# PeihaoChen/RSPNet

Hardware: AMD Instinct MI355X
Metric: clips/sec pretext step (c3d 16x112x112, B=32/GPU) (higher is better)
Workload: dtype f32

## Files before the change

### include/rspnet_hip.h

```cpp
#ifndef RSPNET_HIP_H
#define RSPNET_HIP_H

#include <stddef.h>
#include <stdint.h>

#ifdef __cplusplus
extern "C" {
#endif

#define RSP_OK 0
#define RSP_EINVAL (-1)
#define RSP_EWORKSPACE (-2)
#define RSP_ELAUNCH (-3)
#define RSP_EUNSUPPORTED (-4)

const char* rsp_strerror(int code);
const char* rsp_last_error(void);
const char* rsp_last_conv_kernel(void);
int rsp_version(void);

typedef struct rsp_conv3d_desc {
  int32_t N, Di, Hi, Wi, Cin;
  int32_t Do, Ho, Wo, Cout;
  int32_t kT, kH, kW;
  int32_t sT, sH, sW;
  int32_t pT, pH, pW;
  int32_t in_ld;
  int32_t out_ld;
} rsp_conv3d_desc;

size_t rsp_conv3d_packed_fwd_elems(const rsp_conv3d_desc* d);
int rsp_conv3d_pack_fwd(const rsp_conv3d_desc* d, const float* w_ref, float* w_packed, void* stream);

int32_t rsp_conv3d_stat_tiles(const rsp_conv3d_desc* d);
size_t rsp_conv3d_fwd_workspace(const rsp_conv3d_desc* d);
int rsp_conv3d_fwd(const rsp_conv3d_desc* d, const float* x, const float* w_packed, const float* bias, float* y,
                   float* stat_partials, void* workspace, size_t workspace_bytes, void* stream);

size_t rsp_conv3d_dgrad_workspace(const rsp_conv3d_desc* d);
int rsp_conv3d_dgrad(const rsp_conv3d_desc* d, const float* dy, const float* w_ref, float* dx, void* workspace,
                     size_t workspace_bytes, void* stream);

size_t rsp_conv3d_packed_dgrad_elems(const rsp_conv3d_desc* d);
int rsp_conv3d_dgrad_packed(const rsp_conv3d_desc* d, const float* dy, const float* w_packed, float* dx, void* workspace,
                            size_t workspace_bytes, void* stream);

typedef struct rsp_pack_job {
  const void* src;
  void* dst;
  int64_t total;
  int32_t kind, Cout_src, Cin_src, kT, kH, kW;
  int32_t transpose, O, C, Kld, nTd, nTh, nTw, k0d, k0h, k0w, kstepd, ksteph, kstepw, ntaps;
  int32_t blocks, reserved;
} rsp_pack_job;
int32_t rsp_conv3d_pack_jobs(const rsp_conv3d_desc* d, int32_t which, int32_t Cout_src, int32_t Cin_src, const float* w_ref,
                             float* w_packed, rsp_pack_job* jobs, int32_t max_jobs);
int rsp_pack_run(const rsp_pack_job* jobs_device, int32_t n_jobs, int32_t max_blocks, void* stream);
void rsp_conv3d_pack_forget(const void* w_packed);

size_t rsp_conv3d_wgrad_workspace(const rsp_conv3d_desc* d);
size_t rsp_conv3d_rowgeom_bytes(const rsp_conv3d_desc* d);
int rsp_conv3d_rowgeom(const rsp_conv3d_desc* d, void* table, void* stream);
int rsp_conv3d_wgrad(const rsp_conv3d_desc* d, const float* x, const float* dy, float* dw_ref, float* dbias, int32_t cout_valid,
                     int32_t cin_valid, const void* rowgeom_table, void* workspace, size_t workspace_bytes, void* stream);

const char* rsp_conv3d_kernel_name(const rsp_conv3d_desc* d, int which);

double rsp_conv3d_executed_fraction(const rsp_conv3d_desc* d, int which);

int rsp_conv3d_set_option(const char* name, int32_t value);

int rsp_fastdiv_check(int d, int n);

typedef struct rsp_bn_ema_job {
  float* running_mean;
  float* running_var;
  const float* batch_stats;
  int32_t C;
  float momentum;
} rsp_bn_ema_job;
size_t rsp_bn_finalize_workspace(int32_t tiles, int32_t C);
int rsp_bn_finalize(const float* stat_partials, int32_t tiles, int32_t C, int32_t c_valid, int32_t stat_ld, int64_t count,
                    const float* conv_bias, const float* gamma, const float* beta, float eps, float momentum, float* running_mean,
                    float* running_var, float* batch_stats_out, float* mean_invstd , float* scale_shift ,
                    void* workspace, size_t workspace_bytes, void* stream);
int rsp_bn_running_update(const rsp_bn_ema_job* jobs_device, int32_t n_jobs, int32_t max_c, void* stream);

typedef struct rsp_pool3d_desc {
  int32_t N, Di, Hi, Wi, C;
  int32_t Do, Ho, Wo;
  int32_t kT, kH, kW, sT, sH, sW, pT, pH, pW;
  int32_t in_ld, out_ld, res_ld;
} rsp_pool3d_desc;

int rsp_bn_act_pool_fwd(const rsp_pool3d_desc* d, const float* y, const float* scale_shift, const float* residual,
                        int relu, const float* gate, float* out, void* stream);

int rsp_bn_act_maxpool_applicable(const rsp_pool3d_desc* d);
int rsp_bn_act_maxpool_fwd(const rsp_pool3d_desc* d, const float* y, const float* scale_shift, int relu, const float* gate, float* out,
                           int32_t* argmax, void* stream);

size_t rsp_bn_bwd_workspace(const rsp_pool3d_desc* d);
int rsp_bn_act_pool_bwd(const rsp_pool3d_desc* d, const float* y, const float* residual, const float* dout,
                        const float* gamma, const float* mean_invstd, const float* scale_shift, int relu, float* dy,
                        float* dres, float* dgamma, float* dbeta, int32_t c_valid, const float* gate, const float* dmean,
                        void* workspace, size_t workspace_bytes, void* stream);

size_t rsp_bn_eval_bwd_workspace(const rsp_pool3d_desc* d);
int rsp_bn_eval_act_pool_bwd(const rsp_pool3d_desc* d, const float* y, const float* residual, const float* dout,
                             const float* mean_invstd, const float* scale_shift, int relu, float* dy, float* dres,
                             float* dgamma, float* dbeta, int32_t c_valid, void* workspace, size_t workspace_bytes,
                             void* stream);

int rsp_maxpool3d_fwd(const rsp_pool3d_desc* d, const float* x, float* out, int32_t* argmax, void* stream);
int rsp_maxpool3d_bwd(const rsp_pool3d_desc* d, const float* dout, const int32_t* argmax, float* dx, void* stream);

size_t rsp_gate_fwd_workspace(int32_t N, int32_t P, int32_t C);
int rsp_gate_fwd(const float* x, int32_t N, int32_t P, int32_t C, int32_t in_ld, const float* w, const float* b,
                 float* out, int32_t out_ld, float* mean, float* gate, void* workspace, size_t workspace_bytes,
                 void* stream);
int rsp_bn_gate_sums(const float* y, int32_t N, int32_t P, int32_t C, int32_t y_ld, const float* scale_shift, int relu,
                     float* act, int32_t act_ld, const float* w, const float* b, float* mean, float* gate, void* workspace,
                     size_t workspace_bytes, void* stream);
int rsp_gate_apply(const float* x, int32_t N, int32_t P, int32_t C, int32_t in_ld, const float* gate, float* out, int32_t out_ld,
                   void* stream);
int rsp_gate_bwd_params(const float* y, const float* scale_shift, int relu, const float* dout, int32_t N, int32_t P, int32_t C,
                        int32_t y_ld, int32_t dout_ld, const float* w, const float* mean, const float* gate, float* dw, float* db,
                        float* dmean, void* workspace, size_t workspace_bytes, void* stream);
size_t rsp_gate_bwd_workspace(int32_t N, int32_t P, int32_t C);
int rsp_gate_bwd(const float* x, const float* dout, int32_t N, int32_t P, int32_t C, int32_t x_ld, int32_t dout_ld,
                 const float* w, const float* mean, const float* gate, float* dx, int32_t dx_ld, float* dw, float* db,
                 void* workspace, size_t workspace_bytes, void* stream);

int rsp_head_fwd(const float* feat, int32_t B, int32_t P, int32_t C, int32_t feat_ld, const float* w1,
                 const float* b1, const float* w2, const float* b2, int32_t dim, float* out1, float* out2,
                 float* pooled, float* raw, void* stream);
size_t rsp_head_bwd_workspace(int32_t B, int32_t dim);
int rsp_head_bwd(const float* dout1, const float* dout2, const float* pooled, const float* raw, const float* w1,
                 const float* w2, int32_t B, int32_t P, int32_t C, int32_t feat_ld, int32_t dim, float* dw1,
                 float* db1, float* dw2, float* db2, float* dfeat, void* workspace, size_t workspace_bytes,
                 void* stream);

int rsp_spatial_mean_fwd(const float* x, int32_t N, int32_t P, int32_t C, int32_t ld, float* mean, void* stream);
int rsp_spatial_mean_bwd(const float* dmean, int32_t N, int32_t P, int32_t C, int32_t ld, float* dx, void* stream);
int rsp_linear_fwd(const float* x, int32_t B, int32_t Cin, const float* w, const float* bias, int32_t Cout, int relu,
                   float* y, void* stream);
size_t rsp_linear_bwd_workspace(int32_t B, int32_t Cout);
int rsp_linear_bwd(const float* x, const float* y, const float* dy, const float* w, int32_t B, int32_t Cin, int32_t Cout,
                   int relu, float* dx, float* dw, float* db, void* workspace, size_t workspace_bytes, void* stream);
int rsp_l2norm_fwd(const float* x, int32_t B, int32_t dim, float* y, void* stream);
int rsp_l2norm_bwd(const float* x, const float* dy, int32_t B, int32_t dim, float* dx, void* stream);

int rsp_logits_fwd(const float* qA, const float* qM, const float* kA, const float* kM, const float* knegA,
                   const float* knegM, const float* queue, int32_t B, int32_t dim, int32_t dim_m, int32_t K, float inv_T,
                   float* logits1, float* logits2, float* lposM, float* lnegM, void* stream);
size_t rsp_logits_bwd_workspace(int32_t B, int32_t dim, int32_t K);
int rsp_logits_bwd(const float* dlogits1, const float* dlogits2, const float* dlposM, const float* dlnegM,
                   const float* kA, const float* kM, const float* knegA, const float* knegM, const float* queue,
                   int32_t B, int32_t dim, int32_t dim_m, int32_t K, float inv_T, float* dqA, float* dqM, void* workspace,
                   size_t workspace_bytes, void* stream);

int rsp_loss_fwd_bwd(const float* logits1, const float* logits2, const float* lposM, const float* lnegM, int32_t B,
                     int32_t K1 , float margin, float A, float M, float* losses, float* dlogits1,
                     float* dlogits2, float* dlposM, float* dlnegM, float* row_scratch , void* stream);

int rsp_queue_enqueue(float* queue, int32_t dim, int32_t K, int32_t ptr, const float* keys, int32_t n, void* stream);
int rsp_queue_enqueue_dev(float* queue, int32_t dim, int32_t K, int64_t* ptr_dev, const float* keys, int32_t n, void* stream);

int rsp_clip_gather(const float* im, int32_t B_in, int32_t C, int32_t T_in, int32_t H, int32_t W, const int32_t* src,
                    const int32_t* step, int32_t B_out, int32_t T_out, int32_t C_out, float* out, void* stream);
int rsp_clip_gather_multi(int32_t n_jobs, const float* const* ims, const int32_t* const* srcs, const int32_t* const* steps,
                          float* const* outs, int32_t B_in, int32_t C, int32_t T_in, int32_t H, int32_t W, int32_t B_out, int32_t T_out,
                          int32_t C_out, void* stream);

int rsp_momentum_update(float* k, const float* q, int64_t n, float m, void* stream);

int rsp_sgd_step(float* p, const float* g, float* buf, int64_t n, float lr, float mu, float wd, float gscale,
                 int first, void* stream);

#define RSP_ELT_RELU_FWD 0
#define RSP_ELT_RELU_BWD 1
#define RSP_ELT_SIGMOID_FWD 2
#define RSP_ELT_SIGMOID_BWD 3
#define RSP_ELT_ADD 4
int rsp_eltwise(int32_t op, const float* a, const float* b , float* y, int64_t n, void* stream);

int rsp_rows_gather(const float* in, const int32_t* idx, int32_t n, int32_t width, float* out, void* stream);

#define RSP_AUG_BRIGHTNESS 0
// ... 83 lines not shown
```

### rspnet_amd/_lib.py

```python
from __future__ import annotations

import ctypes as C
import os
from typing import Optional

_HERE = os.path.dirname(os.path.abspath(__file__))
LIB_PATH = os.environ.get("RSPNET_HIP_LIB") or os.path.join(_HERE, "librspnet_hip.so")

c_f32p = C.c_void_p
c_i32p = C.c_void_p
c_stream = C.c_void_p


class ConvDesc(C.Structure):
    _fields_ = [(n, C.c_int32) for n in (
        "N", "Di", "Hi", "Wi", "Cin", "Do", "Ho", "Wo", "Cout", "kT", "kH", "kW", "sT", "sH", "sW",
        "pT", "pH", "pW", "in_ld", "out_ld")]


class PoolDesc(C.Structure):
    _fields_ = [(n, C.c_int32) for n in (
        "N", "Di", "Hi", "Wi", "C", "Do", "Ho", "Wo", "kT", "kH", "kW", "sT", "sH", "sW", "pT", "pH", "pW",
        "in_ld", "out_ld", "res_ld")]


class PackJob(C.Structure):
    _fields_ = [("src", C.c_void_p), ("dst", C.c_void_p), ("total", C.c_int64)] + [(n, C.c_int32) for n in (
        "kind", "Cout_src", "Cin_src", "kT", "kH", "kW", "transpose", "O", "C", "Kld", "nTd", "nTh", "nTw", "k0d", "k0h", "k0w",
        "kstepd", "ksteph", "kstepw", "ntaps", "blocks", "reserved")]


class BnEmaJob(C.Structure):
    _fields_ = [("running_mean", C.c_void_p), ("running_var", C.c_void_p), ("batch_stats", C.c_void_p), ("C", C.c_int32),
                ("momentum", C.c_float)]


class AugmentClipDesc(C.Structure):
    _fields_ = [("src", C.c_void_p), ("frame_pitch", C.c_int64), ("row_pitch", C.c_int32), ("h", C.c_int32), ("w", C.c_int32),
                ("gray", C.c_int32), ("flip", C.c_int32), ("n_ops", C.c_int32), ("op", C.c_int32 * 4),
                ("factor", C.c_float * 4), ("one_minus", C.c_float * 4)]


class ClsMeters(C.Structure):
    _fields_ = [("val", C.c_float * 3), ("sum", C.c_float * 3), ("count", C.c_int32 * 3)]


class PretextMeters(C.Structure):
    _fields_ = [("val", C.c_float * 8), ("sum", C.c_float * 8), ("count", C.c_int32 * 8)]


class FingerprintJob(C.Structure):
    _fields_ = [("ptr", C.c_void_p), ("words", C.c_int64), ("chunk0", C.c_int64), ("kind", C.c_int32), ("reserved", C.c_int32)]


class FingerprintRec(C.Structure):
    _fields_ = [("hash", C.c_uint64), ("sumsq", C.c_double), ("sum_abs", C.c_double), ("max_abs", C.c_float),
                ("nonfinite", C.c_uint32)]


_PD = C.POINTER(ConvDesc)
_PP = C.POINTER(PoolDesc)
_sz = C.c_size_t
_i32 = C.c_int32
_i64 = C.c_int64
_f = C.c_float
_p = C.c_void_p

SIGNATURES = {
    "rsp_strerror": (C.c_char_p, [C.c_int]),
    "rsp_last_error": (C.c_char_p, []),
    "rsp_last_conv_kernel": (C.c_char_p, []),
    "rsp_version": (C.c_int, []),
    "rsp_conv3d_packed_fwd_elems": (_sz, [_PD]),
    "rsp_conv3d_pack_fwd": (C.c_int, [_PD, _p, _p, _p]),
    "rsp_conv3d_stat_tiles": (_i32, [_PD]),
    "rsp_conv3d_fwd_workspace": (_sz, [_PD]),
    "rsp_conv3d_fwd": (C.c_int, [_PD, _p, _p, _p, _p, _p, _p, _sz, _p]),
    "rsp_conv3d_dgrad_workspace": (_sz, [_PD]),
    "rsp_conv3d_dgrad": (C.c_int, [_PD, _p, _p, _p, _p, _sz, _p]),
    "rsp_conv3d_packed_dgrad_elems": (_sz, [_PD]),
    "rsp_conv3d_dgrad_packed": (C.c_int, [_PD, _p, _p, _p, _p, _sz, _p]),
    "rsp_conv3d_pack_jobs": (_i32, [_PD, _i32, _i32, _i32, _p, _p, _p, _i32]),
    "rsp_pack_run": (C.c_int, [_p, _i32, _i32, _p]),
    "rsp_conv3d_pack_forget": (None, [_p]),
    "rsp_conv3d_wgrad_workspace": (_sz, [_PD]),
    "rsp_conv3d_rowgeom_bytes": (_sz, [_PD]),
    "rsp_conv3d_rowgeom": (C.c_int, [_PD, _p, _p]),
    "rsp_conv3d_wgrad": (C.c_int, [_PD, _p, _p, _p, _p, _i32, _i32, _p, _p, _sz, _p]),
    "rsp_conv3d_kernel_name": (C.c_char_p, [_PD, C.c_int]),
    "rsp_conv3d_executed_fraction": (C.c_double, [_PD, C.c_int]),
    "rsp_conv3d_set_option": (C.c_int, [C.c_char_p, _i32]),
    "rsp_fastdiv_check": (C.c_int, [C.c_int, C.c_int]),
    "rsp_bn_finalize_workspace": (_sz, [_i32, _i32]),
    "rsp_bn_finalize": (C.c_int, [_p, _i32, _i32, _i32, _i32, _i64, _p, _p, _p, _f, _f, _p, _p, _p, _p, _p, _p, _sz, _p]),
    "rsp_bn_running_update": (C.c_int, [_p, _i32, _i32, _p]),
    "rsp_bn_act_pool_fwd": (C.c_int, [_PP, _p, _p, _p, C.c_int, _p, _p, _p]),
    "rsp_bn_act_maxpool_applicable": (C.c_int, [_PP]),
    "rsp_bn_act_maxpool_fwd": (C.c_int, [_PP, _p, _p, C.c_int, _p, _p, _p, _p]),
    "rsp_bn_bwd_workspace": (_sz, [_PP]),
    "rsp_bn_act_pool_bwd": (C.c_int, [_PP, _p, _p, _p, _p, _p, _p, C.c_int, _p, _p, _p, _p, _i32, _p, _p, _p, _sz, _p]),
    "rsp_bn_eval_bwd_workspace": (_sz, [_PP]),
    "rsp_bn_eval_act_pool_bwd": (C.c_int, [_PP, _p, _p, _p, _p, _p, C.c_int, _p, _p, _p, _p, _i32, _p, _sz, _p]),
    "rsp_maxpool3d_fwd": (C.c_int, [_PP, _p, _p, _p, _p]),
    "rsp_maxpool3d_bwd": (C.c_int, [_PP, _p, _p, _p, _p]),
    "rsp_gate_fwd_workspace": (_sz, [_i32, _i32, _i32]),
    "rsp_gate_fwd": (C.c_int, [_p, _i32, _i32, _i32, _i32, _p, _p, _p, _i32, _p, _p, _p, _sz, _p]),
    "rsp_bn_gate_sums": (C.c_int, [_p, _i32, _i32, _i32, _i32, _p, C.c_int, _p, _i32, _p, _p, _p, _p, _p, _sz, _p]),
    "rsp_gate_apply": (C.c_int, [_p, _i32, _i32, _i32, _i32, _p, _p, _i32, _p]),
    "rsp_gate_bwd_params": (C.c_int, [_p, _p, C.c_int, _p, _i32, _i32, _i32, _i32, _i32, _p, _p, _p, _p, _p, _p, _p, _sz, _p]),
    "rsp_gate_bwd_workspace": (_sz, [_i32, _i32, _i32]),
    "rsp_gate_bwd": (C.c_int, [_p, _p, _i32, _i32, _i32, _i32, _i32, _p, _p, _p, _p, _i32, _p, _p, _p, _sz, _p]),
    "rsp_head_fwd": (C.c_int, [_p, _i32, _i32, _i32, _i32, _p, _p, _p, _p, _i32, _p, _p, _p, _p, _p]),
    "rsp_head_bwd_workspace": (_sz, [_i32, _i32]),
    "rsp_head_bwd": (C.c_int, [_p, _p, _p, _p, _p, _p, _i32, _i32, _i32, _i32, _i32, _p, _p, _p, _p, _p, _p, _sz, _p]),
    "rsp_spatial_mean_fwd": (C.c_int, [_p, _i32, _i32, _i32, _i32, _p, _p]),
    "rsp_spatial_mean_bwd": (C.c_int, [_p, _i32, _i32, _i32, _i32, _p, _p]),
    "rsp_linear_fwd": (C.c_int, [_p, _i32, _i32, _p, _p, _i32, C.c_int, _p, _p]),
    "rsp_linear_bwd_workspace": (_sz, [_i32, _i32]),
    "rsp_linear_bwd": (C.c_int, [_p, _p, _p, _p, _i32, _i32, _i32, C.c_int, _p, _p, _p, _p, _sz, _p]),
    "rsp_l2norm_fwd": (C.c_int, [_p, _i32, _i32, _p, _p]),
    "rsp_l2norm_bwd": (C.c_int, [_p, _p, _i32, _i32, _p, _p]),
    "rsp_logits_fwd": (C.c_int, [_p, _p, _p, _p, _p, _p, _p, _i32, _i32, _i32, _i32, _f, _p, _p, _p, _p, _p]),
    "rsp_logits_bwd_workspace": (_sz, [_i32, _i32, _i32]),
    "rsp_logits_bwd": (C.c_int, [_p, _p, _p, _p, _p, _p, _p, _p, _p, _i32, _i32, _i32, _i32, _f, _p, _p, _p, _sz, _p]),
    "rsp_loss_fwd_bwd": (C.c_int, [_p, _p, _p, _p, _i32, _i32, _f, _f, _f, _p, _p, _p, _p, _p, _p, _p]),
    "rsp_queue_enqueue": (C.c_int, [_p, _i32, _i32, _i32, _p, _i32, _p]),
    "rsp_queue_enqueue_dev": (C.c_int, [_p, _i32, _i32, _p, _p, _i32, _p]),
    "rsp_clip_gather": (C.c_int, [_p, _i32, _i32, _i32, _i32, _i32, _p, _p, _i32, _i32, _i32, _p, _p]),
    "rsp_clip_gather_multi": (C.c_int, [_i32, _p, _p, _p, _p, _i32, _i32, _i32, _i32, _i32, _i32, _i32, _i32, _p]),
    "rsp_momentum_update": (C.c_int, [_p, _p, _i64, _f, _p]),
    "rsp_sgd_step": (C.c_int, [_p, _p, _p, _i64, _f, _f, _f, _f, C.c_int, _p]),
    "rsp_rows_gather": (C.c_int, [_p, _p, _i32, _i32, _p, _p]),
    "rsp_eltwise": (C.c_int, [_i32, _p, _p, _p, _i64, _p]),
    "rsp_augment_workspace": (_sz, [_i32, _i32, _i32]),
    "rsp_augment_batch": (C.c_int, [_p, _i32, _i32, _i32, C.POINTER(C.c_float), C.POINTER(C.c_float), C.POINTER(C.c_float), _p, _i64,
                                    _p, _sz, _p]),
    "rsp_cosine_topk_splits": (_i32, [_i32, _i32, _i32]),
    "rsp_cosine_topk_workspace": (_sz, [_i32, _i32, _i32, _i32, _i32]),
    "rsp_cosine_topk": (C.c_int, [_p, _i32, _i32, _p, _i32, _i32, _i32, _i32, _i32, _p, _p, _p, _sz, _p]),
    "rsp_topk_hits": (C.c_int, [_p, _i32, _i32, _p, _p, _i32, C.POINTER(C.c_int32), _i32, _p, _p]),
    "rsp_knn_classify_workspace": (_sz, [_i32, _i32, _i32, _i32, _i32, _i32]),
    "rsp_knn_classify": (C.c_int, [_p, _i32, _i32, _p, _p, _i32, _i32, _p, _i32, _i32, _f, _i32, _i32, _i32, _p, _p, _p, _p, _p, _p,
                                   _p, _sz, _p]),
    "rsp_xent_metrics_workspace": (_sz, [_i32, _i32]),
    "rsp_xent_metrics": (C.c_int, [_p, _i32, _i32, _i32, _i32, _p, _i32, _p, _p, _p, _p, _p, _p, _sz, _p]),
    "rsp_pretext_metrics_workspace": (_sz, [_i32]),
    "rsp_pretext_metrics": (C.c_int, [_p, _p, _p, _p, _i32, _i32, _p, _p, _p, _p, _sz, _p]),
    "rsp_cam_maps_workspace": (_sz, [_i32, _i32]),
    "rsp_cam_maps": (C.c_int, [_p, _i32, _p, _i32, _p, _i32, _i32, _i32, _p, _p, _p, _p, _i32, _i32, _p, _p, _sz, _p]),
    "rsp_cam_overlay": (C.c_int, [_p, _i32, _i32, _i32, _i32, _p, _p, _i32, _i32, _i32, _i32, _p, _p]),
    "rsp_fingerprint_workspace": (_sz, [_i64]),
    "rsp_fingerprint": (C.c_int, [_p, _i32, _i64, _p, _p, _sz, _p]),
}

_lib: Optional[C.CDLL] = None


class RspError(RuntimeError):
    pass


def load(init_gpu: bool = False) -> C.CDLL:
    global _lib
    if init_gpu:
        _init_gpu()
    if _lib is not None:
        return _lib
    if not os.path.exists(LIB_PATH):
        raise RspError(
            f"{LIB_PATH} not found: build it with rspnet_amd/csrc/build.sh (or __graft_entry__.build()). "
            "rspnet_amd has no CPU or eager fallback.")
    try:
        import torch
    except ImportError:
        pass
    lib = C.CDLL(LIB_PATH)
    for name, (res, args) in SIGNATURES.items():
        fn = getattr(lib, name)
        fn.restype = res
        fn.argtypes = args
    _lib = lib
    return lib

# ... 33 lines not shown
```

### rspnet_amd/csrc/bn_pool.hip

```cpp
#include "common.h"

namespace {

__global__ __launch_bounds__(256) void bn_finalize_stage1(const float* __restrict__ part, int tiles, int C, int ld, int S,
                                                          double* __restrict__ out) {
  __shared__ double red[4][64][2];
  const int c = blockIdx.x * 64 + (threadIdx.x & 63);
  const int rl = threadIdx.x >> 6;
  const int per = (tiles + S - 1) / S;
  const int t0 = blockIdx.y * per, t1 = min(tiles, t0 + per);
  double s = 0.0, ss = 0.0;
  if (c < C)
    for (int t = t0 + rl; t < t1; t += 4) {
      const float2 v = *reinterpret_cast<const float2*>(part + ((long long)t * ld + c) * 2);
      s += (double)v.x;
      ss += (double)v.y;
    }
  red[rl][threadIdx.x & 63][0] = s;
  red[rl][threadIdx.x & 63][1] = ss;
  __syncthreads();
  if (rl == 0 && c < C) {
    const int l = threadIdx.x;
    out[((long long)blockIdx.y * C + c) * 2 + 0] = red[0][l][0] + red[1][l][0] + red[2][l][0] + red[3][l][0];
    out[((long long)blockIdx.y * C + c) * 2 + 1] = red[0][l][1] + red[1][l][1] + red[2][l][1] + red[3][l][1];
// ... 256 lines not shown
        const long long base = (((long long)n * d.Di + od * d.sT) * d.Hi + oh * d.sH) * d.Wi + ow * d.sW;
        float v[NW][VEC], r[NW][VEC], g[VEC], best[VEC];
#pragma unroll
        for (int w = 0; w < NW; ++w) {
          load_vec<VEC>(p.y + (base + off[w]) * d.in_ld + c, v[w]);
          if (p.res) load_vec<VEC>(p.res + (base + off[w]) * d.res_ld + c, r[w]);
        }
        if (p.gate) load_vec<VEC>(p.gate + (long long)n * d.C + c, g);
#pragma unroll
        for (int e = 0; e < VEC; ++e) best[e] = -INFINITY;
#pragma unroll
        for (int w = 0; w < NW; ++w)
#pragma unroll
          for (int e = 0; e < VEC; ++e) {
            float z = fmaf(v[w][e], sc[e], sh[e]);
            if (p.res) z += r[w][e];
            if (p.relu) z = rsp_relu(z);
            if (p.gate) z *= g[e];
            best[e] = rsp_max_nan(best[e], z);
          }
        store_vec<VEC>(p.out + o * d.out_ld + c, best);
      }
    }
    return;
  }
  for (long long o = (long long)blockIdx.x * p.ppi + pl; o < p.npos; o += (long long)gridDim.x * p.ppi) {
    float best[VEC];
    if (unit) {
      float v[VEC], r[VEC];
      load_vec<VEC>(p.y + o * d.in_ld + c, v);
      if (p.res) load_vec<VEC>(p.res + o * d.res_ld + c, r);
#pragma unroll
      for (int e = 0; e < VEC; ++e) {
        float z = fmaf(v[e], sc[e], sh[e]);
        if (p.res) z += r[e];
        best[e] = p.relu ? rsp_relu(z) : z;
      }
      if (p.gate) {
        const int n = fastdiv(fastdiv(fastdiv((int)o, p.dWo), p.dHo), p.dDo);
        float g[VEC];
        load_vec<VEC>(p.gate + (long long)n * d.C + c, g);
#pragma unroll
        for (int e = 0; e < VEC; ++e) best[e] *= g[e];
      }
    } else {
      const int op = (int)o;
      const int q1 = fastdiv(op, p.dWo), ow = op - q1 * d.Wo;
      const int q2 = fastdiv(q1, p.dHo), oh = q1 - q2 * d.Ho;
      const int n = fastdiv(q2, p.dDo), od = q2 - n * d.Do;
      float g[VEC];
      if (p.gate) load_vec<VEC>(p.gate + (long long)n * d.C + c, g);
#pragma unroll
      for (int e = 0; e < VEC; ++e) best[e] = -INFINITY;
      for (int kt = 0; kt < d.kT; ++kt) {
        const int id = od * d.sT - d.pT + kt;
        if ((unsigned)id >= (unsigned)d.Di) continue;
        for (int kh = 0; kh < d.kH; ++kh) {
          const int ih = oh * d.sH - d.pH + kh;
          if ((unsigned)ih >= (unsigned)d.Hi) continue;
          for (int kw = 0; kw < d.kW; ++kw) {
            const int iw = ow * d.sW - d.pW + kw;
            if ((unsigned)iw >= (unsigned)d.Wi) continue;
            const long long pos = (((long long)n * d.Di + id) * d.Hi + ih) * d.Wi + iw;
            float v[VEC];
            load_vec<VEC>(p.y + pos * d.in_ld + c, v);
            float r[VEC];
            if (p.res) load_vec<VEC>(p.res + pos * d.res_ld + c, r);
#pragma unroll
            for (int e = 0; e < VEC; ++e) {
              float z = fmaf(v[e], sc[e], sh[e]);
              if (p.res) z += r[e];
              if (p.relu) z = rsp_relu(z);
              if (p.gate) z *= g[e];
              best[e] = rsp_max_nan(best[e], z);
            }
          }
        }
      }
    }
    store_vec<VEC>(p.out + o * d.out_ld + c, best);
  }
}

struct BwdParams {
  rsp_pool3d_desc d;
  const float* __restrict__ y;
  const float* __restrict__ res;
  const float* __restrict__ dout;
  const float* __restrict__ gamma;
  const float* __restrict__ mi;
  const float* __restrict__ ss;
  const double* __restrict__ sums;
  float* __restrict__ partial;
  float* __restrict__ dy;
  float* __restrict__ dres;
  int relu;
  int cg;
  int nblocks;
  long long count;
  int cgc, ppi;
  long long npos;
  FastDiv dcgc, dWo, dHo, dDo;
  int Cv;
  const float* __restrict__ gate;
  const float* __restrict__ dmean;
  float invP;
};

template <int VEC>
__device__ __forceinline__ void gated_grad(const BwdParams& p, int n, int c, float (&g)[VEC]) {
  float gt[VEC], dm[VEC];
  load_vec<VEC>(p.gate + (long long)n * p.d.C + c, gt);
  load_vec<VEC>(p.dmean + (long long)n * p.d.C + c, dm);
#pragma unroll
  for (int e = 0; e < VEC; ++e) g[e] = fmaf(g[e], gt[e], dm[e] * p.invP);
}

template <int VEC>
__device__ __forceinline__ void load_gamma(const BwdParams& p, int c, float (&gam)[VEC]) {
  if (p.gamma && p.Cv == p.d.C) {
    load_vec<VEC>(p.gamma + c, gam);
  } else {
#pragma unroll
    for (int e = 0; e < VEC; ++e) gam[e] = c + e < p.Cv ? (p.gamma ? p.gamma[c + e] : 1.f) : 0.f;
  }
}

template <int VEC>
__device__ __forceinline__ void zval(const BwdParams& p, long long pos, int c, const float (&sc)[VEC],
                                     const float (&sh)[VEC], float (&yv)[VEC], float (&z)[VEC]) {
  load_vec<VEC>(p.y + pos * p.d.in_ld + c, yv);
  float r[VEC];
  if (p.res) load_vec<VEC>(p.res + pos * p.d.res_ld + c, r);
#pragma unroll
  for (int e = 0; e < VEC; ++e) {
    z[e] = fmaf(yv[e], sc[e], sh[e]);
    if (p.res) z[e] += r[e];
  }
}

template <int VEC, int MODE>
__global__ __launch_bounds__(256) void bn_bwd_reduce_kernel(const BwdParams p) {
  const rsp_pool3d_desc& d = p.d;
  __shared__ float red[256][2 * VEC];
  const int cg0 = blockIdx.y * 256;
  const int cgc = min(p.cg - cg0, 256);
  const int ppi = p.ppi;
  const int t = threadIdx.x;
  const int pl = fastdiv(t, p.dcgc);
  const int cgi = cg0 + (t - pl * p.cgc);
  const bool active = pl < ppi && (t - pl * p.cgc) < cgc;
  const int c = cgi * VEC;
  float s1[VEC], s2[VEC];
#pragma unroll
  for (int e = 0; e < VEC; ++e) s1[e] = s2[e] = 0.f;
  if (active) {
    float sc[VEC], sh[VEC], mean[VEC], invstd[VEC];
    load_vec<VEC>(p.ss + c, sc);
    load_vec<VEC>(p.ss + d.C + c, sh);
    load_vec<VEC>(p.mi + c, mean);
    load_vec<VEC>(p.mi + d.C + c, invstd);
    const long long npos = (long long)d.N * d.Do * d.Ho * d.Wo;
    long long op = (long long)blockIdx.x * ppi + pl;
    long long stride = (long long)gridDim.x * ppi;
    if constexpr (MODE == 1) {
      const long long step = ppi;
      stride *= 4;
      op = (long long)blockIdx.x * ppi * 4 + pl;
      for (; op + 3 * step < npos; op += stride) {
        float yv[4][VEC], r[4][VEC], g[4][VEC];
#pragma unroll
        for (int u = 0; u < 4; ++u) {
          load_vec<VEC>(p.y + (op + u * step) * d.in_ld + c, yv[u]);
          if (p.res) load_vec<VEC>(p.res + (op + u * step) * d.res_ld + c, r[u]);
          load_vec<VEC>(p.dout + (op + u * step) * d.out_ld + c, g[u]);
        }
#pragma unroll
        for (int u = 0; u < 4; ++u)
#pragma unroll
          for (int e = 0; e < VEC; ++e) {
            float z = fmaf(yv[u][e], sc[e], sh[e]);
            if (p.res) z += r[u][e];
            const float zz = p.relu ? rsp_relu(z) : z;
            const float dz = (p.relu && rsp_relu_blocks(zz)) ? 0.f : g[u][e];
            s1[e] += dz;
            s2[e] = fmaf(dz, (yv[u][e] - mean[e]) * invstd[e], s2[e]);
          }
      }
      stride = step;
    }
    long long op_end = MODE == 1 ? min(npos, op + 4 * (long long)ppi) : npos;
    if constexpr (MODE == 2 || MODE == 3) {
      {
        constexpr int NW = MODE == 2 ? 4 : 8;
        long long off[NW];
        window_offsets<NW>(d, off);
        for (; op < npos; op += stride) {
          const int q1 = fastdiv((int)op, p.dWo), ow = (int)op - q1 * d.Wo;
          const int q2 = fastdiv(q1, p.dHo), oh = q1 - q2 * d.Ho;
          const int n = fastdiv(q2, p.dDo), od = q2 - n * d.Do;
          const long long base = (((long long)n * d.Di + od * d.sT) * d.Hi + oh * d.sH) * d.Wi + ow * d.sW;
          float yv[NW][VEC], r[NW][VEC], g[VEC], best[VEC], by[VEC];
#pragma unroll
          for (int w = 0; w < NW; ++w) {
            load_vec<VEC>(p.y + (base + off[w]) * d.in_ld + c, yv[w]);
            if (p.res) load_vec<VEC>(p.res + (base + off[w]) * d.res_ld + c, r[w]);
          }
          load_vec<VEC>(p.dout + op * d.out_ld + c, g);
#pragma unroll
          for (int e = 0; e < VEC; ++e) { best[e] = -INFINITY; by[e] = 0.f; }
#pragma unroll
          for (int w = 0; w < NW; ++w)
#pragma unroll
            for (int e = 0; e < VEC; ++e) {
              float z = fmaf(yv[w][e], sc[e], sh[e]);
              if (p.res) z += r[w][e];
              const float zz = p.relu ? rsp_relu(z) : z;
              if (rsp_max_takes(zz, best[e])) { best[e] = zz; by[e] = yv[w][e]; }
            }
#pragma unroll
          for (int e = 0; e < VEC; ++e) {
            const float dz = (p.relu && rsp_relu_blocks(best[e])) ? 0.f : g[e];
            s1[e] += dz;
            s2[e] = fmaf(dz, (by[e] - mean[e]) * invstd[e], s2[e]);
          }
        }
      }
      op_end = 0;
    }
    for (; op < op_end; op += stride) {
      const int q1 = fastdiv((int)op, p.dWo), ow = (int)op - q1 * d.Wo;
      const int q2 = fastdiv(q1, p.dHo), oh = q1 - q2 * d.Ho;
      const int n = fastdiv(q2, p.dDo), od = q2 - n * d.Do;
      float best[VEC], by[VEC];
#pragma unroll
      for (int e = 0; e < VEC; ++e) { best[e] = -INFINITY; by[e] = 0.f; }
      for (int kt = 0; kt < d.kT; ++kt) {
        const int id = od * d.sT - d.pT + kt;
        if ((unsigned)id >= (unsigned)d.Di) continue;
        for (int kh = 0; kh < d.kH; ++kh) {
          const int ih = oh * d.sH - d.pH + kh;
          if ((unsigned)ih >= (unsigned)d.Hi) continue;
          for (int kw = 0; kw < d.kW; ++kw) {
            const int iw = ow * d.sW - d.pW + kw;
            if ((unsigned)iw >= (unsigned)d.Wi) continue;
            const long long pos = (((long long)n * d.Di + id) * d.Hi + ih) * d.Wi + iw;
            float yv[VEC], z[VEC];
            zval<VEC>(p, pos, c, sc, sh, yv, z);
#pragma unroll
            for (int e = 0; e < VEC; ++e) {
              const float zz = p.relu ? rsp_relu(z[e]) : z[e];
              if (rsp_max_takes(zz, best[e])) { best[e] = zz; by[e] = yv[e]; }
            }
          }
        }
      }
      float g[VEC];
      load_vec<VEC>(p.dout + op * d.out_ld + c, g);
      if (p.gate) gated_grad<VEC>(p, n, c, g);
#pragma unroll
      for (int e = 0; e < VEC; ++e) {
        const float dz = (p.relu && rsp_relu_blocks(best[e])) ? 0.f : g[e];
        s1[e] += dz;
        s2[e] = fmaf(dz, (by[e] - mean[e]) * invstd[e], s2[e]);
      }
    }
  }
#pragma unroll
  for (int e = 0; e < VEC; ++e) { red[t][e] = s1[e]; red[t][VEC + e] = s2[e]; }
  __syncthreads();
  if (t < cgc) {
    float a1[VEC], a2[VEC];
#pragma unroll
    for (int e = 0; e < VEC; ++e) a1[e] = a2[e] = 0.f;
    for (int l = 0; l < ppi; ++l)
#pragma unroll
      for (int e = 0; e < VEC; ++e) { a1[e] += red[l * cgc + t][e]; a2[e] += red[l * cgc + t][VEC + e]; }
    float* o = p.partial + ((long long)blockIdx.x * d.C + (cg0 + t) * VEC) * 2;
#pragma unroll
    for (int e = 0; e < VEC; ++e) { o[2 * e] = a1[e]; o[2 * e + 1] = a2[e]; }
  }
}

__global__ __launch_bounds__(1024) void bn_bwd_finalize_kernel(const float* __restrict__ partial, int nblocks, int C, int Cv,
                                                               double* __restrict__ sums, float* __restrict__ dgamma,
                                                               float* __restrict__ dbeta) {
  const int c = blockIdx.x * FIN_CH + (threadIdx.x & (FIN_CH - 1));
  double a, b;
  if (!fin_sum_partials(partial, nblocks, C, C, a, b)) return;
  sums[2 * c] = a;
  sums[2 * c + 1] = b;
  if (dbeta && c < Cv) dbeta[c] = (float)a;
  if (dgamma && c < Cv) dgamma[c] = (float)b;
}

template <int VEC>
__global__ __launch_bounds__(256) void bn_bwd_apply_kernel(const BwdParams p) {
  const rsp_pool3d_desc& d = p.d;
  const long long total = (long long)d.N * d.Di * d.Hi * d.Wi * p.cg;
  const double invn = 1.0 / (double)p.count;
  for (long long idx = blockIdx.x * 256ll + threadIdx.x; idx < total; idx += 256ll * gridDim.x) {
    const int cgi = (int)(idx % p.cg);
    long long q = idx / p.cg;
    const long long pos = q;
    const int iw = (int)(q % d.Wi); q /= d.Wi;
    const int ih = (int)(q % d.Hi); q /= d.Hi;
    const int id = (int)(q % d.Di);
    const int n = (int)(q / d.Di);
    const int c = cgi * VEC;
    float sc[VEC], sh[VEC], mean[VEC], invstd[VEC], gam[VEC];
    load_vec<VEC>(p.ss + c, sc);
    load_vec<VEC>(p.ss + d.C + c, sh);
    load_vec<VEC>(p.mi + c, mean);
    load_vec<VEC>(p.mi + d.C + c, invstd);
    load_gamma<VEC>(p, c, gam);
    float yv[VEC], z[VEC], dz[VEC];
    zval<VEC>(p, pos, c, sc, sh, yv, z);
#pragma unroll
    for (int e = 0; e < VEC; ++e) dz[e] = 0.f;
    const int od = id / d.sT, oh = ih / d.sH, ow = iw / d.sW;
    if (od < d.Do && oh < d.Ho && ow < d.Wo) {
      bool win[VEC];
      float mine[VEC];
#pragma unroll
      for (int e = 0; e < VEC; ++e) { mine[e] = p.relu ? rsp_relu(z[e]) : z[e]; win[e] = true; }
      const int my = ((id - od * d.sT) * d.kH + (ih - oh * d.sH)) * d.kW + (iw - ow * d.sW);
      if (d.kT * d.kH * d.kW > 1) {
        for (int kt = 0; kt < d.kT; ++kt)
          for (int kh = 0; kh < d.kH; ++kh)
            for (int kw = 0; kw < d.kW; ++kw) {
              const int o = (kt * d.kH + kh) * d.kW + kw;
              if (o == my) continue;
              const long long pp = (((long long)n * d.Di + od * d.sT + kt) * d.Hi + oh * d.sH + kh) * d.Wi + ow * d.sW + kw;
              float y2[VEC], z2[VEC];
              zval<VEC>(p, pp, c, sc, sh, y2, z2);
#pragma unroll
              for (int e = 0; e < VEC; ++e) {
                const float v = p.relu ? rsp_relu(z2[e]) : z2[e];
                if (rsp_max_displaced(o < my, v, mine[e])) win[e] = false;
              }
            }
      }
      const long long op = (((long long)n * d.Do + od) * d.Ho + oh) * d.Wo + ow;
      float g[VEC];
      load_vec<VEC>(p.dout + op * d.out_ld + c, g);
#pragma unroll
      for (int e = 0; e < VEC; ++e) dz[e] = (win[e] && !(p.relu && rsp_relu_blocks(mine[e]))) ? g[e] : 0.f;
    }
// ... 420 lines not shown
  const bool tile = d->kT == d->sT && d->kH == d->sH && d->kW == d->sW && !(d->pT | d->pH | d->pW);
  return tile && nwin == 4 ? 2 : (tile && nwin == 8 ? 3 : 0);
}

#define RSP_BN_LAUNCH_V(K, V, mode, grid, stream, p)                                                   \
  do {                                                                                                 \
    switch (mode) {                                                                                    \
      case 1: hipLaunchKernelGGL((K<V, 1>), grid, dim3(256), 0, stream, p); break;                     \
      case 2: hipLaunchKernelGGL((K<V, 2>), grid, dim3(256), 0, stream, p); break;                     \
      case 3: hipLaunchKernelGGL((K<V, 3>), grid, dim3(256), 0, stream, p); break;                     \
      default: hipLaunchKernelGGL((K<V, 0>), grid, dim3(256), 0, stream, p); break;                    \
    }                                                                                                  \
  } while (0)
#define RSP_BN_LAUNCH(K, vec, mode, grid, stream, p)                                                   \
  do {                                                                                                 \
    if (vec) RSP_BN_LAUNCH_V(K, 4, mode, grid, stream, p);                                             \
    else RSP_BN_LAUNCH_V(K, 1, mode, grid, stream, p);                                                 \
  } while (0)

int grid_for(long long total) {
  long long b = (total + 255) / 256;
  return (int)(b > 8192 ? 8192 : (b < 1 ? 1 : b));
}

int reduce_blocks(const rsp_pool3d_desc* d, int cg) {
  const int cgc = cg < 256 ? cg : 256;
  const int ppi = 256 / cgc;
  const long long npos = (long long)d->N * d->Do * d->Ho * d->Wo;
  long long b = (npos + (long long)ppi * 8 - 1) / ((long long)ppi * 8);
  return (int)(b > 2048 ? 2048 : (b < 1 ? 1 : b));
}

}

extern "C" {

static int finalize_slices(int tiles) { return tiles >= 8192 ? 256 : (tiles >= 4096 ? 64 : (tiles >= 64 ? 16 : 1)); }

size_t rsp_bn_finalize_workspace(int32_t tiles, int32_t C) {
  const int S = finalize_slices(tiles);
  return (size_t)S * C * 2 * sizeof(double);
}

__global__ __launch_bounds__(256) void bn_ema_kernel(const rsp_bn_ema_job* __restrict__ jobs) {
  const rsp_bn_ema_job j = jobs[blockIdx.y];
  const int c = blockIdx.x * 256 + threadIdx.x;
  if (c >= j.C) return;
  j.running_mean[c] = (1.f - j.momentum) * j.running_mean[c] + j.momentum * j.batch_stats[c];
  j.running_var[c] = (1.f - j.momentum) * j.running_var[c] + j.momentum * j.batch_stats[j.C + c];
}

int rsp_bn_running_update(const rsp_bn_ema_job* jobs_device, int32_t n_jobs, int32_t max_c, void* stream) {
  RSP_REQUIRE(jobs_device && n_jobs > 0 && n_jobs <= 65535 && max_c > 0, "rsp_bn_running_update: bad argument");
  hipLaunchKernelGGL(bn_ema_kernel, dim3(rsp_cdiv(max_c, 256), n_jobs), dim3(256), 0, (hipStream_t)stream, jobs_device);
  return rsp_check_launch("bn_ema_kernel");
}

int rsp_bn_finalize(const float* stat_partials, int32_t tiles, int32_t C, int32_t c_valid, int32_t stat_ld, int64_t count,
                    const float* conv_bias, const float* gamma, const float* beta, float eps, float momentum, float* running_mean,
                    float* running_var, float* batch_stats_out, float* mean_invstd, float* scale_shift, void* workspace,
                    size_t workspace_bytes, void* stream) {
  RSP_REQUIRE(stat_partials && mean_invstd && scale_shift && workspace, "rsp_bn_finalize: null pointer");
  RSP_REQUIRE(tiles > 0 && C > 0 && count > 0 && stat_ld >= C && c_valid > 0 && c_valid <= C, "rsp_bn_finalize: bad size");
  const int S = finalize_slices(tiles);
  if (workspace_bytes < (size_t)S * C * 2 * sizeof(double)) {
    rsp_set_error("rsp_bn_finalize: workspace too small");
    return RSP_EWORKSPACE;
  }
  hipStream_t s = (hipStream_t)stream;
  if (tiles <= 2048) {
    hipLaunchKernelGGL(bn_finalize_one_kernel, dim3(rsp_cdiv(C, FIN_CH)), dim3(1024), 0, s, stat_partials, tiles, C, c_valid, stat_ld, (long long)count,
                       conv_bias, gamma, beta, eps, momentum, running_mean, running_var, mean_invstd, scale_shift, batch_stats_out);
    return rsp_check_launch("bn_finalize_one_kernel");
  }
  double* part = reinterpret_cast<double*>(workspace);
  hipLaunchKernelGGL(bn_finalize_stage1, dim3(rsp_cdiv(C, 64), S), dim3(256), 0, s, stat_partials, tiles, C, stat_ld, S, part);
  int rc = rsp_check_launch("bn_finalize_stage1");
  if (rc != RSP_OK) return rc;
  hipLaunchKernelGGL(bn_finalize_stage2, dim3(rsp_cdiv(C, 64)), dim3(1024), 0, s, part, S, C, c_valid, (long long)count, conv_bias,
                     gamma, beta, eps, momentum, running_mean, running_var, mean_invstd, scale_shift, batch_stats_out);
  return rsp_check_launch("bn_finalize_stage2");
}

int rsp_bn_act_pool_fwd(const rsp_pool3d_desc* d, const float* y, const float* scale_shift, const float* residual,
                        int relu, const float* gate, float* out, void* stream) {
  RSP_REQUIRE(pool_ok(d, false), "rsp_bn_act_pool_fwd: bad descriptor");
  RSP_REQUIRE(y && scale_shift && out, "rsp_bn_act_pool_fwd: null pointer");
  if (!residual && (d->kT != d->sT || d->kH != d->sH || d->kW != d->sW || d->pT || d->pH || d->pW) &&
      rsp_bn_act_maxpool_applicable(d) && rsp_aligned16(y) && rsp_aligned16(out) && rsp_aligned16(scale_shift) &&
      (!gate || rsp_aligned16(gate)))
    return rsp_bn_act_maxpool_fwd(d, y, scale_shift, relu, gate, out, nullptr, stream);
  PoolParams p;
  p.d = *d; p.y = y; p.ss = scale_shift; p.res = residual; p.gate = gate; p.out = out; p.relu = relu;
  const bool vec = d->C % 4 == 0 && d->in_ld % 4 == 0 && d->out_ld % 4 == 0 && rsp_aligned16(y) && rsp_aligned16(out) &&
                   rsp_aligned16(scale_shift) && (!residual || (d->res_ld % 4 == 0 && rsp_aligned16(residual))) &&
                   (!gate || rsp_aligned16(gate));
  p.cg = vec ? d->C / 4 : d->C;
  const Layout L = make_layout(d, p.cg, 4);
  RSP_REQUIRE(L.npos < (1ll << 31), "rsp_bn_act_pool_fwd: more than 2^31 - 1 output positions");
  set_layout(p, L);
  RSP_BN_LAUNCH(bn_act_pool_fwd_kernel, vec, bn_mode(d, gate != nullptr), L.grid, (hipStream_t)stream, p);
  return rsp_check_launch("bn_act_pool_fwd_kernel");
}

size_t rsp_bn_bwd_workspace(const rsp_pool3d_desc* d) {
  if (!pool_ok(d, true)) return 0;
  return rsp_align_up((size_t)2048 * d->C * 2 * sizeof(float), 256) + (size_t)d->C * 2 * sizeof(double);
}

int rsp_bn_act_pool_bwd(const rsp_pool3d_desc* d, const float* y, const float* residual, const float* dout,
                        const float* gamma, const float* mean_invstd, const float* scale_shift, int relu, float* dy,
                        float* dres, float* dgamma, float* dbeta, int32_t c_valid, const float* gate, const float* dmean,
                        void* workspace, size_t workspace_bytes, void* stream) {
  RSP_REQUIRE(pool_ok(d, true), "rsp_bn_act_pool_bwd: needs disjoint windows (kernel == stride, no padding)");
  RSP_REQUIRE(!gate || (dmean && d->kT * d->kH * d->kW == 1 && d->sT * d->sH * d->sW == 1 && !residual),
              "rsp_bn_act_pool_bwd: a gated unit has a unit window, no residual, and needs dmean");
  RSP_REQUIRE(c_valid > 0 && c_valid <= d->C, "rsp_bn_act_pool_bwd: bad valid channel count");
  RSP_REQUIRE(y && dout && mean_invstd && scale_shift && dy && workspace, "rsp_bn_act_pool_bwd: null pointer");
  if (workspace_bytes < rsp_bn_bwd_workspace(d)) {
    rsp_set_error("rsp_bn_act_pool_bwd: workspace too small");
    return RSP_EWORKSPACE;
  }
  hipStream_t s = (hipStream_t)stream;
  BwdParams p;
  memset(&p, 0, sizeof p);
  p.d = *d; p.y = y; p.res = residual; p.dout = dout; p.gamma = gamma; p.mi = mean_invstd; p.ss = scale_shift;
  p.dy = dy; p.dres = dres; p.relu = relu;
  p.Cv = c_valid;
  p.gate = gate; p.dmean = dmean;
  p.invP = 1.f / (float)((long long)d->Di * d->Hi * d->Wi);
  p.count = (long long)d->N * d->Di * d->Hi * d->Wi;
  const bool vec = d->C % 4 == 0 && d->in_ld % 4 == 0 && d->out_ld % 4 == 0 && rsp_aligned16(y) && rsp_aligned16(dout) &&
                   rsp_aligned16(dy) && rsp_aligned16(scale_shift) && rsp_aligned16(mean_invstd) &&
                   (!gamma || c_valid != d->C || rsp_aligned16(gamma)) &&
                   (!residual || (d->res_ld % 4 == 0 && rsp_aligned16(residual) && (!dres || rsp_aligned16(dres)))) &&
                   (!gate || (rsp_aligned16(gate) && rsp_aligned16(dmean)));
  p.cg = vec ? d->C / 4 : d->C;
  p.partial = reinterpret_cast<float*>(workspace);
  double* sums = reinterpret_cast<double*>(reinterpret_cast<unsigned char*>(workspace) +
                                           rsp_align_up((size_t)2048 * d->C * 2 * sizeof(float), 256));
  p.sums = sums;
  const Layout L = make_layout(d, p.cg, 4);
  RSP_REQUIRE(L.npos < (1ll << 31), "rsp_bn_act_pool_bwd: more than 2^31 - 1 output positions");
  set_layout(p, L);
  p.nblocks = reduce_blocks(d, p.cg);
  dim3 rgrid(p.nblocks, rsp_cdiv(p.cg, 256));
  const int mode = bn_mode(d, gate != nullptr);
  RSP_BN_LAUNCH(bn_bwd_reduce_kernel, vec, mode, rgrid, s, p);
  int rc = rsp_check_launch("bn_bwd_reduce_kernel");
  if (rc != RSP_OK) return rc;
  hipLaunchKernelGGL(bn_bwd_finalize_kernel, dim3(rsp_cdiv(d->C, FIN_CH)), dim3(1024), 0, s, p.partial, p.nblocks, d->C, c_valid, sums,
                     dgamma, dbeta);
  rc = rsp_check_launch("bn_bwd_finalize_kernel");
  if (rc != RSP_OK) return rc;
  const bool exact = d->Di % d->sT == 0 && d->Hi % d->sH == 0 && d->Wi % d->sW == 0 && d->kT * d->kH * d->kW <= 8;
  if (exact) {
    RSP_BN_LAUNCH(bn_bwd_apply_win_kernel, vec, mode, L.grid, s, p);
    return rsp_check_launch("bn_bwd_apply_win_kernel");
  }
  const long long total = (long long)d->N * d->Di * d->Hi * d->Wi * p.cg;
  if (vec) hipLaunchKernelGGL(bn_bwd_apply_kernel<4>, dim3(grid_for(total)), dim3(256), 0, s, p);
  else hipLaunchKernelGGL(bn_bwd_apply_kernel<1>, dim3(grid_for(total)), dim3(256), 0, s, p);
  return rsp_check_launch("bn_bwd_apply_kernel");
}

static int eval_bwd_mode(const rsp_pool3d_desc* d) {
  const int m = bn_mode(d, false);
  if (m == 1) return 1;
  const bool exact = d->Di % d->sT == 0 && d->Hi % d->sH == 0 && d->Wi % d->sW == 0;
  return exact ? m : 0;
}

static long long eval_bwd_npos(const rsp_pool3d_desc* d, int mode) {
  if (mode != 0) return (long long)d->N * d->Do * d->Ho * d->Wo;
  return (long long)d->N * rsp_cdiv(d->Di, d->sT) * rsp_cdiv(d->Hi, d->sH) * rsp_cdiv(d->Wi, d->sW);
}

size_t rsp_bn_eval_bwd_workspace(const rsp_pool3d_desc* d) {
  if (!pool_ok(d, true)) return 0;
  const long long npos = eval_bwd_npos(d, eval_bwd_mode(d));
  const long long rows = npos < EVAL_BWD_MAX_BLOCKS ? npos : EVAL_BWD_MAX_BLOCKS;
  return (size_t)rows * d->C * 2 * sizeof(float);
}

#define RSP_BN_EVAL_LAUNCH_S(V, M, grid, stream, p)                                                                       \
  do {                                                                                                                    \
    if (sums) hipLaunchKernelGGL((bn_eval_bwd_kernel<V, M, true>), grid, dim3(256), 0, stream, p);                        \
    else hipLaunchKernelGGL((bn_eval_bwd_kernel<V, M, false>), grid, dim3(256), 0, stream, p);                            \
  } while (0)
#define RSP_BN_EVAL_LAUNCH_V(V, mode, grid, stream, p)                                                                    \
  do {                                                                                                                    \
    switch (mode) {                                                                                                       \
      case 1: RSP_BN_EVAL_LAUNCH_S(V, 1, grid, stream, p); break;                                                         \
      case 2: RSP_BN_EVAL_LAUNCH_S(V, 2, grid, stream, p); break;                                                         \
      case 3: RSP_BN_EVAL_LAUNCH_S(V, 3, grid, stream, p); break;                                                         \
      default: RSP_BN_EVAL_LAUNCH_S(V, 0, grid, stream, p); break;                                                        \
    }                                                                                                                     \
  } while (0)

int rsp_bn_eval_act_pool_bwd(const rsp_pool3d_desc* d, const float* y, const float* residual, const float* dout,
                             const float* mean_invstd, const float* scale_shift, int relu, float* dy, float* dres,
                             float* dgamma, float* dbeta, int32_t c_valid, void* workspace, size_t workspace_bytes,
                             void* stream) {
  RSP_REQUIRE(pool_ok(d, true), "rsp_bn_eval_act_pool_bwd: needs disjoint windows (kernel == stride, no padding)");
  RSP_REQUIRE(c_valid > 0 && c_valid <= d->C, "rsp_bn_eval_act_pool_bwd: bad valid channel count");
  RSP_REQUIRE(y && dout && scale_shift && dy, "rsp_bn_eval_act_pool_bwd: null pointer");
  RSP_REQUIRE(!dres || residual, "rsp_bn_eval_act_pool_bwd: dres without a residual");
  RSP_REQUIRE(d->res_ld >= d->C || !residual, "rsp_bn_eval_act_pool_bwd: bad residual pitch");
  const bool sums = dgamma || dbeta;
  RSP_REQUIRE(!sums || (mean_invstd && workspace), "rsp_bn_eval_act_pool_bwd: parameter gradients need mean_invstd and a workspace");
  if (sums && workspace_bytes < rsp_bn_eval_bwd_workspace(d)) {
    rsp_set_error("rsp_bn_eval_act_pool_bwd: workspace too small");
    return RSP_EWORKSPACE;
  }
  hipStream_t s = (hipStream_t)stream;
  EvalBwdParams p;
  memset(&p, 0, sizeof p);
  p.d = *d; p.y = y; p.res = residual; p.dout = dout; p.mi = mean_invstd; p.ss = scale_shift;
  p.partial = sums ? reinterpret_cast<float*>(workspace) : nullptr;
  p.dy = dy; p.dres = dres; p.relu = relu; p.Cv = c_valid;
  const bool vec = d->C % 4 == 0 && d->in_ld % 4 == 0 && d->out_ld % 4 == 0 && rsp_aligned16(y) && rsp_aligned16(dout) &&
                   rsp_aligned16(dy) && rsp_aligned16(scale_shift) && (!sums || rsp_aligned16(mean_invstd)) &&
                   (!residual || (d->res_ld % 4 == 0 && rsp_aligned16(residual) && (!dres || rsp_aligned16(dres))));
  p.cg = vec ? d->C / 4 : d->C;
  const int mode = eval_bwd_mode(d);
  p.npos = eval_bwd_npos(d, mode);
  RSP_REQUIRE(p.npos < (1ll << 31), "rsp_bn_eval_act_pool_bwd: more than 2^31 - 1 positions");
  p.cgc = p.cg < 256 ? p.cg : 256;
  p.ppi = 256 / p.cgc;
  p.dcgc = fastdiv_make(p.cgc);
  p.De = rsp_cdiv(d->Di, d->sT); p.He = rsp_cdiv(d->Hi, d->sH); p.We = rsp_cdiv(d->Wi, d->sW);
  if (mode == 0) { p.dW = fastdiv_make(p.We); p.dH = fastdiv_make(p.He); p.dD = fastdiv_make(p.De); }
  else { p.dW = fastdiv_make(d->Wo); p.dH = fastdiv_make(d->Ho); p.dD = fastdiv_make(d->Do); }
  long long b = (p.npos + (long long)p.ppi * 16 - 1) / ((long long)p.ppi * 16);
  b = b > EVAL_BWD_MAX_BLOCKS ? EVAL_BWD_MAX_BLOCKS : (b < 1 ? 1 : b);
  const dim3 grid((unsigned)b, (unsigned)rsp_cdiv(p.cg, 256));
  if (vec) RSP_BN_EVAL_LAUNCH_V(4, mode, grid, s, p);
  else RSP_BN_EVAL_LAUNCH_V(1, mode, grid, s, p);
  int rc = rsp_check_launch("bn_eval_bwd_kernel");
  if (rc != RSP_OK || !sums) return rc;
  hipLaunchKernelGGL(bn_eval_bwd_finalize_kernel, dim3(rsp_cdiv(d->C, FIN_CH)), dim3(1024), 0, s, p.partial, (int)b, d->C, c_valid,
                     dgamma, dbeta);
  return rsp_check_launch("bn_eval_bwd_finalize_kernel");
}

}
// ... 1 lines not shown
```

### rspnet_amd/csrc/conv_igemm.hip

```cpp
#include "common.h"
#include <algorithm>
#include <type_traits>
#include "conv_stem.h"

namespace {

constexpr int BK = 32;
constexpr int LDK = BK + 4;
constexpr int MAX_TAPS = 343;

__device__ __attribute__((aligned(64))) float g_zero[16];

const float* igemm_zero_page() {
  static const float* cache[64] = {nullptr};
  int dev = 0;
  if (hipGetDevice(&dev) != hipSuccess || dev < 0 || dev >= 64) dev = 0;
  if (!cache[dev]) {
    void* z = nullptr;
    if (hipGetSymbolAddress(&z, HIP_SYMBOL(g_zero)) != hipSuccess || !z) return nullptr;
    cache[dev] = reinterpret_cast<const float*>(z);
  }
  return cache[dev];
}

// ... 2325 lines not shown
  if (mp.split) {
    mp.ms = plan_multi_split(nm, Ms, tl, nc, cols);
    if (mp.ms.bytes > ws_bytes) mp.split = false;
  }
  if (!((tiles_all >= 512 && tiles_all <= 4096) || mp.split)) return mp;
  mp.n = nm;
  const bool square = bn == 128 || bn == 64;
  mp.l.family = K_MULTI;
  mp.l.bm = 128; mp.l.bn = bn; mp.l.waves_m = square ? 2 : 4; mp.l.waves_n = square ? 2 : 1; mp.l.vec = 4; mp.l.minw = 2;
  mp.l.cols = cols;
  mp.l.partial_bytes = mp.split ? mp.ms.bytes : 0;
  return mp;
}

}

bool rsp_conv_desc_ok(const rsp_conv3d_desc* d) {
  if (!d) return false;
  if (d->N <= 0 || d->Cin <= 0 || d->Cout <= 0) return false;
  if (d->kT * d->kH * d->kW > MAX_TAPS || d->kT <= 0 || d->kH <= 0 || d->kW <= 0) return false;
  if (d->sT <= 0 || d->sH <= 0 || d->sW <= 0 || d->pT < 0 || d->pH < 0 || d->pW < 0) return false;
  if (d->Do != (d->Di + 2 * d->pT - d->kT) / d->sT + 1) return false;
  if (d->Ho != (d->Hi + 2 * d->pH - d->kH) / d->sH + 1) return false;
  if (d->Wo != (d->Wi + 2 * d->pW - d->kW) / d->sW + 1) return false;
  if (d->Do <= 0 || d->Ho <= 0 || d->Wo <= 0) return false;
  if (d->in_ld < d->Cin || d->out_ld < d->Cout) return false;
  return (long long)d->N * d->Do * d->Ho * d->Wo < (1ll << 31);
}

extern "C" {


size_t rsp_conv3d_packed_fwd_elems(const rsp_conv3d_desc* d) {
  if (!desc_ok(d)) return 0;
  if (rsp_stem_applicable(d)) return rsp_stem_packed_elems(d);
  const size_t K = (size_t)d->kT * d->kH * d->kW * d->Cin;
  return (size_t)d->Cout * rsp_align_up(K, 4);
}

int rsp_conv3d_pack_fwd(const rsp_conv3d_desc* d, const float* w_ref, float* w_packed, void* stream) {
  RSP_REQUIRE(desc_ok(d), "rsp_conv3d_pack_fwd: bad descriptor");
  RSP_REQUIRE(w_ref && w_packed, "rsp_conv3d_pack_fwd: null pointer");
  if (rsp_stem_applicable(d)) return rsp_stem_pack(d, w_ref, w_packed, (hipStream_t)stream);
  PackParams p;
  p.w = w_ref; p.out = w_packed;
  p.Cout = d->Cout; p.Cin = d->Cin; p.kT = d->kT; p.kH = d->kH; p.kW = d->kW;
  p.transpose = 0; p.O = d->Cout; p.C = d->Cin;
  p.Kld = (int)rsp_align_up((size_t)d->kT * d->kH * d->kW * d->Cin, 4);
  p.nTd = d->kT; p.nTh = d->kH; p.nTw = d->kW;
  p.k0d = p.k0h = p.k0w = 0;
  p.kstepd = p.ksteph = p.kstepw = 1;
  const long long total = (long long)p.O * p.Kld;
  const int blocks = (int)((total + 255) / 256 > 4096 ? 4096 : (total + 255) / 256);
  hipLaunchKernelGGL(pack_weight_kernel, dim3(blocks), dim3(256), 0, (hipStream_t)stream, p);
  return rsp_check_launch("pack_weight_kernel");
}

int32_t rsp_conv3d_stat_tiles(const rsp_conv3d_desc* d) {
  if (!desc_ok(d)) return 0;
  if (rsp_stem_applicable(d)) return rsp_stem_tiles(d);
  return rsp_cdiv((long long)d->N * d->Do * d->Ho * d->Wo, 128);
}

size_t rsp_conv3d_fwd_workspace(const rsp_conv3d_desc* d) {
  if (!desc_ok(d)) return 0;
  if (rsp_stem_applicable(d)) return 0;
  IgemmParams p;
  fill_fwd_params(d, ALIGNED, ALIGNED, nullptr, ALIGNED, nullptr, p);
  return igemm_partial_bytes(p);
}

int rsp_conv3d_fwd(const rsp_conv3d_desc* d, const float* x, const float* w_packed, const float* bias, float* y,
                   float* stat_partials, void* workspace, size_t workspace_bytes, void* stream) {
  RSP_REQUIRE(desc_ok(d), "rsp_conv3d_fwd: bad descriptor");
  RSP_REQUIRE(x && w_packed && y, "rsp_conv3d_fwd: null pointer");
  RSP_REQUIRE(rsp_aligned16(w_packed), "rsp_conv3d_fwd: packed weight must be 16-byte aligned");
  rsp_note_reset();
  if (rsp_stem_applicable(d)) return rsp_stem_fwd(d, x, w_packed, bias, y, stat_partials, (hipStream_t)stream);
  IgemmParams p;
  const bool vec4 = fill_fwd_params(d, x, w_packed, bias, y, stat_partials, p);
  return run_igemm(p, vec4, workspace, workspace_bytes, (hipStream_t)stream);
}

double rsp_conv3d_executed_fraction(const rsp_conv3d_desc* d, int which) {
  if (!desc_ok(d)) return 1.0;
  if (which == 2) return rsp_wgrad_executed_fraction(d);
  if (which == 0) {
    if (rsp_stem_applicable(d)) return 1.0;
    IgemmParams p;
    const bool vec4 = fill_fwd_params(d, ALIGNED, ALIGNED, nullptr, ALIGNED, nullptr, p);
    return igemm_live_fraction(p, vec4, plan_conv(p, vec4, 0, SIZE_MAX).l[0]);
  }
  IgemmParams cls[64];
  bool cvec[64], in_multi[64] = {false};
  const int ncls = dgrad_classes(d, ALIGNED, ALIGNED, ALIGNED, cls, cvec);
  const MultiPlan mp = plan_multi(cls, cvec, ncls, multi_split_ok(d, ALIGNED), SIZE_MAX);
  for (int j = 0; j < mp.n; ++j) in_multi[mp.cls[j]] = true;
  double live = 0.0, tot = 0.0;
  for (int i = 0; i < ncls; ++i) {
    const IgemmParams& p = cls[i];
    const double wgt = (double)p.M * p.K;
    live += wgt * igemm_live_fraction(p, cvec[i], in_multi[i] ? mp.l : plan_conv(p, cvec[i], 0, SIZE_MAX).l[0]);
    tot += wgt;
  }
  return tot > 0 ? live / tot : 1.0;
}

int rsp_fastdiv_check(int d, int n) {
  const FastDiv f = fastdiv_make(d);
  return f.mul ? (int)((unsigned)(((unsigned long long)(unsigned)n * f.mul) >> 32) >> f.shr) : n;
}

const char* rsp_conv3d_kernel_name(const rsp_conv3d_desc* d, int which) {
  if (!desc_ok(d)) return "invalid";
  if (which == 2) return rsp_wgrad_kernel_name(d);
  if (which == 0 && rsp_stem_applicable(d)) return rsp_stem_kernel_name(d);
  static thread_local char names[64][64];
  static thread_local int n_names = 0;
  LaunchPlan l;
  if (which == 0) {
    IgemmParams p;
    const bool vec4 = fill_fwd_params(d, ALIGNED, ALIGNED, nullptr, ALIGNED, nullptr, p);
    l = plan_conv(p, vec4, out_span_bytes(p), SIZE_MAX).l[0];
  } else {
    IgemmParams cls[64];
    bool cvec[64];
    const int ncls = dgrad_classes(d, ALIGNED, ALIGNED, ALIGNED, cls, cvec);
    const MultiPlan mp = plan_multi(cls, cvec, ncls, multi_split_ok(d, ALIGNED), SIZE_MAX);
    if (d->sT * d->sH * d->sW > 1) cls[0].nTd = cls[0].nTh = cls[0].nTw = 1;
    l = mp.n ? mp.l : plan_conv(cls[0], cvec[0], out_span_bytes(cls[0]), SIZE_MAX).l[0];
  }
  char name[64];
  if (l.family == K_PERSIST || l.family == K_PERSIST_FOLD)
    snprintf(name, sizeof name, kernel_format(l.family), l.bm, l.bn, l.waves_m, l.waves_n, l.ks ? "true" : "false", l.minw);
  else
    snprintf(name, sizeof name, kernel_format(l.family), l.bm, l.bn, l.waves_m, l.waves_n, l.vec, l.minw);
  for (int i = 0; i < n_names; ++i)
    if (!strcmp(names[i], name)) return names[i];
  if (n_names == 64) n_names = 0;
  return strcpy(names[n_names++], name);
}

size_t rsp_conv3d_dgrad_workspace(const rsp_conv3d_desc* d) {
  if (!desc_ok(d)) return 0;
  IgemmParams cls[64];
  bool cvec[64];
  const int ncls = dgrad_classes(d, ALIGNED, ALIGNED, ALIGNED, cls, cvec);
  for (int i = 0; i < ncls; ++i) cvec[i] = true;
  size_t part = plan_multi(cls, cvec, ncls, true, SIZE_MAX).l.partial_bytes;
  for (int i = 0; i < ncls; ++i) {
    const size_t b = igemm_partial_bytes(cls[i]);
    part = b > part ? b : part;
  }
  return dgrad_wpack_bytes(d) + part;
}


static void dgrad_pack_params(const rsp_conv3d_desc* d, const DgradClass& g, const float* w_ref, float* out, PackParams& pk) {
  pk.w = w_ref; pk.out = out;
  pk.Cout = d->Cout; pk.Cin = d->Cin; pk.kT = d->kT; pk.kH = d->kH; pk.kW = d->kW;
  pk.transpose = 1; pk.O = d->Cin; pk.C = d->Cout;
  pk.Kld = (int)rsp_align_up((size_t)g.nt * g.nh * g.nw * d->Cout, 4);
  pk.nTd = g.nt; pk.nTh = g.nh; pk.nTw = g.nw;
  pk.k0d = g.k0t; pk.k0h = g.k0h; pk.k0w = g.k0w;
  pk.kstepd = d->sT; pk.ksteph = d->sH; pk.kstepw = d->sW;
}
// ... 217 lines not shown
```

### rspnet_amd/csrc/conv_stem.h

```cpp
#pragma once
#include "common.h"

bool rsp_conv_desc_ok(const rsp_conv3d_desc* d);
bool rsp_stem_applicable(const rsp_conv3d_desc* d);
int rsp_stem_tiles(const rsp_conv3d_desc* d);
size_t rsp_stem_packed_elems(const rsp_conv3d_desc* d);
int rsp_stem_pack(const rsp_conv3d_desc* d, const float* w_ref, float* w_packed, hipStream_t s);
int rsp_stem_fwd(const rsp_conv3d_desc* d, const float* x, const float* w_packed, const float* bias, float* y,
                 float* stat_partials, hipStream_t s);
const char* rsp_stem_kernel_name(const rsp_conv3d_desc* d);
void rsp_stem_note_packed(const void* w_packed, bool three_channels);
void rsp_stem_forget_packed(const void* w_packed);
const char* rsp_wgrad_kernel_name(const rsp_conv3d_desc* d);
double rsp_wgrad_executed_fraction(const rsp_conv3d_desc* d);
```

### rspnet_amd/csrc/conv_stem.hip

```cpp
#include "conv_stem.h"

#include <mutex>
#include <unordered_map>

namespace {

struct StemParams {
  const float* __restrict__ x;
  const float* __restrict__ w;
  const float* __restrict__ bias;
  float* __restrict__ y;
  float* __restrict__ stat;
  int N, Di, Hi, Wi, Do, Ho, Wo;
  int kT, kH, kW, sT, sH, sW, pT, pH, pW;
  int Cout, out_ld;
  int tw_shift;
  int HT, WT, WTh, WTL;
  int npix, npix_r;
  int FR;
  int ntaps, nchunks;
  int tiles_h, tiles_w, tiles;
  unsigned x_bytes, w_bytes;
  int wide;
};

struct StemBias {
  floatx4 w[2];
  float n[2];
};

__device__ __forceinline__ StemBias stem_bias(const float* __restrict__ bias, int Cout, bool wide, int lane) {
  StemBias b;
#pragma unroll
  for (int j = 0; j < 2; ++j) {
    b.w[j] = floatx4{0.f, 0.f, 0.f, 0.f};
    b.n[j] = 0.f;
    const int cw = 32 * j + 4 * (lane & 7), cn = 32 * j + (lane & 31);
    if (bias && wide && cw < Cout) b.w[j] = *reinterpret_cast<const floatx4*>(bias + cw);
    if (bias && !wide && cn < Cout) b.n[j] = bias[cn];
  }
  asm volatile("" : "+v"(b.w[0]), "+v"(b.w[1]), "+v"(b.n[0]), "+v"(b.n[1]));
  return b;
}

__device__ __forceinline__ void stem_store_wide(const StemParams& p, const floatx16 (&acc)[2], float* stage ,
                                                const long long* rowaddr , int wave, int lane, const StemBias& b) {
  const int l32 = lane & 31, h = lane >> 5;
  const int q = lane & 7, rbase = lane >> 3;
#pragma unroll
  for (int j = 0; j < 2; ++j) {
    const int col = 32 * j + 4 * q;
#pragma unroll
    for (int r = 0; r < 2; ++r) {
#pragma unroll
      for (int e = 0; e < 8; ++e) stage[((e >> 2) * 8 + h * 4 + (e & 3)) * 32 + l32] = acc[j][8 * r + e];
#pragma unroll
      for (int i = 0; i < 2; ++i) {
        const int rl = rbase + 8 * i;
        const floatx4 v = *reinterpret_cast<const floatx4*>(stage + rl * 32 + 4 * q);
        const long long addr = rowaddr[wave * 32 + 16 * r + rl];
        if (addr >= 0 && col < p.Cout) *reinterpret_cast<floatx4*>(p.y + addr + col) = v + b.w[j];
      }
    }
  }
}

template <int G, int NS>
__global__ __launch_bounds__(256, 2) void stem_kernel(const StemParams p) {
  constexpr int TCH = 2 * G;
  constexpr int BU = TCH * 64;
  constexpr int BI = (BU + 255) / 256;
  typedef __attribute__((address_space(3))) void* lptr_t;
  extern __shared__ __attribute__((aligned(16))) unsigned char smem_raw[];
  float* halo = reinterpret_cast<float*>(smem_raw);
  float* Bs = halo + p.FR * p.npix_r * 4;
  int* taptab = reinterpret_cast<int*>(Bs + 2 * BU * 4);
  long long* rowaddr = reinterpret_cast<long long*>(taptab + p.nchunks * TCH);

  const int t = threadIdx.x;
  const int lane = t & 63;
  const int wave = __builtin_amdgcn_readfirstlane(t >> 6);
  const int l32 = lane & 31, h = lane >> 5;

  const int tile = rsp_xcd_remap(blockIdx.x, gridDim.x);
  const int wb = tile % p.tiles_w;
  int q0 = tile / p.tiles_w;
  const int hb = q0 % p.tiles_h;
  q0 /= p.tiles_h;
  const int to = q0 % p.Do;
  const int n = q0 / p.Do;
  const int TW = 1 << p.tw_shift, TH = 128 >> p.tw_shift;
  const int h0 = hb * TH, w0 = wb * TW;
  const StemBias bias = stem_bias(p.bias, p.Cout, p.wide != 0, lane);

  const int khw = p.kH * p.kW;
  for (int i = t; i < p.nchunks * TCH; i += 256) {
    int off = 0;
    if (i < p.ntaps) {
      const int kw = i % p.kW, r = i / p.kW;
      const int kh = r % p.kH, kt = r / p.kH;
      const int col = p.sW == 2 ? (kw & 1) * p.WTh + (kw >> 1) : kw;
      off = (((kt % p.FR) * p.npix_r) + kh * p.WTL + col) * 16;
    }
    taptab[i] = off;
  }

  unsigned hrel[4];
#pragma unroll
  for (int i = 0; i < 4; ++i) {
    const int q = i * 256 + t;
    unsigned r = 0xffffffffu;
    if (q < p.npix) {
      const int hyy = q / p.WTL, cc = q - hyy * p.WTL;
      const int wxp = p.sW == 2 ? (cc < p.WTh ? 2 * cc : 2 * (cc - p.WTh) + 1) : cc;
      const int hi = h0 * p.sH - p.pH + hyy, wi = w0 * p.sW - p.pW + wxp;
      if (wxp < p.WT && (unsigned)hi < (unsigned)p.Hi && (unsigned)wi < (unsigned)p.Wi) r = (unsigned)((hi * p.Wi + wi) * 16);
    }
    hrel[i] = r;
  }

  __amdgpu_buffer_rsrc_t rsrc_x = __builtin_amdgcn_make_buffer_rsrc(const_cast<float*>(p.x), 0, (int)p.x_bytes, 0x00020000);
  __amdgpu_buffer_rsrc_t rsrc_w = __builtin_amdgcn_make_buffer_rsrc(const_cast<float*>(p.w), 0, (int)p.w_bytes, 0x00020000);

  auto load_frame = [&](int f) {
    const int ti = to * p.sT - p.pT + f;
    const bool okf = (unsigned)ti < (unsigned)p.Di;
    const unsigned fbase = (unsigned)(((long long)(n * p.Di + (okf ? ti : 0)) * p.Hi * p.Wi) * 16);
    const int slot = f % p.FR;
#pragma unroll
    for (int i = 0; i < 4; ++i) {
      if (i * 256 + wave * 64 < p.npix_r) {
        const unsigned off = (okf & (hrel[i] != 0xffffffffu)) ? fbase + hrel[i] : 0xffffffffu;
        float* dst = halo + (slot * p.npix_r + i * 256 + wave * 64) * 4;
        __builtin_amdgcn_raw_ptr_buffer_load_lds(rsrc_x, (lptr_t)dst, 16, off, 0, 0, 0);
      }
    }
  };
  auto load_weights = [&](int c, int buf) {
#pragma unroll
    for (int i = 0; i < BI; ++i) {
      if (i * 256 + wave * 64 < BU) {
        const unsigned off = ((unsigned)c * BU + i * 256 + t) * 16u;
        float* dst = Bs + (buf * BU + i * 256 + wave * 64) * 4;
        __builtin_amdgcn_raw_ptr_buffer_load_lds(rsrc_w, (lptr_t)dst, 16, off, 0, 0, 0);
      }
// ... 15 lines not shown

  floatx16 acc[2];
#pragma unroll
  for (int j = 0; j < 2; ++j)
#pragma unroll
    for (int e = 0; e < 16; ++e) acc[j][e] = 0.f;

  int buf = 0;
  for (int c = 0; c < p.nchunks; ++c) {
    const bool more = c + 1 < p.nchunks;
    floatx4 af[G], bf[G][2];
#pragma unroll
    for (int g = 0; g < G; ++g) af[g] = *reinterpret_cast<const floatx4*>(arow + toff[g]);
    const float* bb = Bs + buf * BU * 4 + (h * 64 + l32) * 4;
#pragma unroll
    for (int g = 0; g < G; ++g)
#pragma unroll
      for (int j = 0; j < 2; ++j) bf[g][j] = *reinterpret_cast<const floatx4*>(bb + (2 * g * 64 + 32 * j) * 4);
    int toffn[G];
#pragma unroll
    for (int g = 0; g < G; ++g) toffn[g] = more ? taptab[(c + 1) * TCH + 2 * g + h] : 0;
    if (more) {
      load_weights(c + 1, buf ^ 1);
      const int fh = frame_hi(c + 1);
      while (loaded < fh) load_frame(++loaded);
    }
#pragma unroll
    for (int g = 0; g < G; ++g)
#pragma unroll
      for (int s = 0; s < NS; ++s)
#pragma unroll
        for (int j = 0; j < 2; ++j) acc[j] = __builtin_amdgcn_mfma_f32_32x32x2f32(af[g][s], bf[g][j][s], acc[j], 0, 0, 0);
    __builtin_amdgcn_sched_barrier(0);
    __syncthreads();
    buf ^= 1;
#pragma unroll
    for (int g = 0; g < G; ++g) toff[g] = toffn[g];
  }

  if (t < 128) {
    const int ry = t >> p.tw_shift, rx = t & (TW - 1);
    const int ho = h0 + ry, wo = w0 + rx;
    rowaddr[t] = (ho < p.Ho && wo < p.Wo) ? ((((long long)n * p.Do + to) * p.Ho + ho) * p.Wo + wo) * p.out_ld : -1;
  }
  __syncthreads();
  float* red = Bs;
  if (p.wide) stem_store_wide(p, acc, Bs + 512 + wave * 512, rowaddr, wave, lane, bias);
#pragma unroll
  for (int j = 0; j < 2; ++j) {
    const int col = 32 * j + l32;
    const float bv = bias.n[j];
    float s = 0.f, ss = 0.f;
#pragma unroll
    for (int e = 0; e < 16; ++e) {
      const long long addr = rowaddr[wave * 32 + (e >> 2) * 8 + h * 4 + (e & 3)];
      const float v = addr >= 0 ? acc[j][e] : 0.f;
      if (!p.wide && addr >= 0 && col < p.Cout) p.y[addr + col] = v + bv;
      s += v;
      ss = fmaf(v, v, ss);
    }
    s += __shfl_xor(s, 32);
    ss += __shfl_xor(ss, 32);
    if (h == 0) {
      red[(wave * 64 + col) * 2 + 0] = s;
      red[(wave * 64 + col) * 2 + 1] = ss;
    }
  }
  if (p.stat) {
    __syncthreads();
    if (t < 64 && t < p.Cout) {
      float s = 0.f, ss = 0.f;
#pragma unroll
      for (int w = 0; w < 4; ++w) {
        s += red[(w * 64 + t) * 2 + 0];
        ss += red[(w * 64 + t) * 2 + 1];
      }
      float* o = p.stat + ((long long)tile * p.Cout + t) * 2;
      o[0] = s;
      o[1] = ss;
    }
  }
}

template <int G, bool WIDE, int NS>
__global__ __launch_bounds__(256, 2) void stem_resident_kernel(const StemParams p) {
  constexpr int TCH = 2 * G;
  constexpr int BU = TCH * 64;
  constexpr int BI = (BU + 255) / 256;
  typedef __attribute__((address_space(3))) void* lptr_t;
  extern __shared__ __attribute__((aligned(16))) unsigned char smem_raw[];
  const int hsz = p.FR * p.npix_r * 4;
  float* halo = reinterpret_cast<float*>(smem_raw);
  float* Bs = halo + 2 * hsz;
  int* taptab = reinterpret_cast<int*>(Bs + p.nchunks * BU * 4);
  long long* rowaddr = reinterpret_cast<long long*>(taptab + p.nchunks * TCH);
  float* red = reinterpret_cast<float*>(rowaddr + 128);

  const int t = threadIdx.x;
  const int lane = t & 63;
  const int wave = __builtin_amdgcn_readfirstlane(t >> 6);
  const int l32 = lane & 31, h = lane >> 5;
  const int TW = 1 << p.tw_shift, TH = 128 >> p.tw_shift;

  for (int i = t; i < p.nchunks * TCH; i += 256) {
    int off = 0;
    if (i < p.ntaps) {
      const int kw = i % p.kW, r = i / p.kW;
      const int kh = r % p.kH, kt = r / p.kH;
      const int col = p.sW == 2 ? (kw & 1) * p.WTh + (kw >> 1) : kw;
      off = ((kt * p.npix_r) + kh * p.WTL + col) * 16;
    }
    taptab[i] = off;
  }
  __amdgpu_buffer_rsrc_t rsrc_x = __builtin_amdgcn_make_buffer_rsrc(const_cast<float*>(p.x), 0, (int)p.x_bytes, 0x00020000);
  __amdgpu_buffer_rsrc_t rsrc_w = __builtin_amdgcn_make_buffer_rsrc(const_cast<float*>(p.w), 0, (int)p.w_bytes, 0x00020000);
  for (int c = 0; c < p.nchunks; ++c) {
#pragma unroll
    for (int i = 0; i < BI; ++i) {
      if (i * 256 + wave * 64 < BU) {
        const unsigned off = ((unsigned)c * BU + i * 256 + t) * 16u;
        float* dst = Bs + (c * BU + i * 256 + wave * 64) * 4;
        __builtin_amdgcn_raw_ptr_buffer_load_lds(rsrc_w, (lptr_t)dst, 16, off, 0, 0, 0);
      }
    }
  }
  int hyy[4], wxp[4];
#pragma unroll
  for (int i = 0; i < 4; ++i) {
    const int q = i * 256 + t;
    hyy[i] = -(1 << 20);
    wxp[i] = 0;
    if (q < p.npix) {
      const int r = q / p.WTL, cc = q - r * p.WTL;
      const int wx_ = p.sW == 2 ? (cc < p.WTh ? 2 * cc : 2 * (cc - p.WTh) + 1) : cc;
      if (wx_ < p.WT) {
        hyy[i] = r;
        wxp[i] = wx_;
      }
    }
  }
  auto issue_halo = [&](int tile, int buf) {
    const int wb = tile % p.tiles_w;
    int q0 = tile / p.tiles_w;
    const int hb = q0 % p.tiles_h;
    q0 /= p.tiles_h;
    const int to = q0 % p.Do, n = q0 / p.Do;
    const int hi0 = hb * TH * p.sH - p.pH, wi0 = wb * TW * p.sW - p.pW;
    unsigned hrel[4];
#pragma unroll
    for (int i = 0; i < 4; ++i) {
      const int hi = hi0 + hyy[i], wi = wi0 + wxp[i];
      hrel[i] = ((unsigned)hi < (unsigned)p.Hi && (unsigned)wi < (unsigned)p.Wi) ? (unsigned)((hi * p.Wi + wi) * 16) : 0xffffffffu;
    }
    for (int f = 0; f < p.kT; ++f) {
      const int ti = to * p.sT - p.pT + f;
      const bool okf = (unsigned)ti < (unsigned)p.Di;
      const unsigned fbase = (unsigned)(((long long)(n * p.Di + (okf ? ti : 0)) * p.Hi * p.Wi) * 16);
#pragma unroll
      for (int i = 0; i < 4; ++i) {
        if (i * 256 + wave * 64 < p.npix_r) {
          const unsigned off = (okf & (hrel[i] != 0xffffffffu)) ? fbase + hrel[i] : 0xffffffffu;
          float* dst = halo + buf * hsz + (f * p.npix_r + i * 256 + wave * 64) * 4;
          __builtin_amdgcn_raw_ptr_buffer_load_lds(rsrc_x, (lptr_t)dst, 16, off, 0, 0, 0);
        }
      }
    }
  };

  const int m = wave * 32 + l32;
  const int rowoff = (((m >> p.tw_shift) * p.sH) * p.WTL + (m & (TW - 1))) * 16;
  const StemBias bias = stem_bias(p.bias, p.Cout, WIDE, lane);

  int cur = 0;
  if ((int)blockIdx.x < p.tiles) issue_halo(blockIdx.x, 0);
  for (int tile = blockIdx.x; tile < p.tiles; tile += gridDim.x) {
    __syncthreads();
    const int next = tile + gridDim.x;
    const char* arow = reinterpret_cast<const char*>(halo + cur * hsz) + rowoff;
    floatx16 acc[2];
#pragma unroll
    for (int j = 0; j < 2; ++j)
#pragma unroll
      for (int e = 0; e < 16; ++e) acc[j][e] = 0.f;
    for (int c = 0; c < p.nchunks; ++c) {
      floatx4 af[G], bf[G][2];
#pragma unroll
      for (int g = 0; g < G; ++g) af[g] = *reinterpret_cast<const floatx4*>(arow + taptab[c * TCH + 2 * g + h]);
      const float* bb = Bs + c * BU * 4 + (h * 64 + l32) * 4;
#pragma unroll
      for (int g = 0; g < G; ++g)
#pragma unroll
        for (int j = 0; j < 2; ++j) bf[g][j] = *reinterpret_cast<const floatx4*>(bb + (2 * g * 64 + 32 * j) * 4);
      if (c == p.nchunks - 1 && next < p.tiles) issue_halo(next, cur ^ 1);
#pragma unroll
      for (int g = 0; g < G; ++g)
#pragma unroll
        for (int s = 0; s < NS; ++s)
#pragma unroll
          for (int j = 0; j < 2; ++j) acc[j] = __builtin_amdgcn_mfma_f32_32x32x2f32(af[g][s], bf[g][j][s], acc[j], 0, 0, 0);
    }
    const int wb = tile % p.tiles_w;
    int q0 = tile / p.tiles_w;
    const int hb = q0 % p.tiles_h;
    q0 /= p.tiles_h;
    const int to = q0 % p.Do, n = q0 / p.Do;
    if (t < 128) {
      const int ho = hb * TH + (t >> p.tw_shift), wo = wb * TW + (t & (TW - 1));
      rowaddr[t] = (ho < p.Ho && wo < p.Wo) ? ((((long long)n * p.Do + to) * p.Ho + ho) * p.Wo + wo) * p.out_ld : -1;
    }
    __syncthreads();
    if (WIDE) stem_store_wide(p, acc, halo + cur * hsz + wave * 512, rowaddr, wave, lane, bias);
#pragma unroll
    for (int j = 0; j < 2; ++j) {
      const int col = 32 * j + l32;
      const float bv = bias.n[j];
      float s = 0.f, ss = 0.f;
#pragma unroll
      for (int e = 0; e < 16; ++e) {
        const long long addr = rowaddr[wave * 32 + (e >> 2) * 8 + h * 4 + (e & 3)];
        const float v = addr >= 0 ? acc[j][e] : 0.f;
        if (!WIDE && addr >= 0 && col < p.Cout) p.y[addr + col] = v + bv;
        s += v;
        ss = fmaf(v, v, ss);
      }
      s += __shfl_xor(s, 32);
      ss += __shfl_xor(ss, 32);
      if (h == 0) {
        red[(wave * 64 + col) * 2 + 0] = s;
        red[(wave * 64 + col) * 2 + 1] = ss;
      }
    }
    if (p.stat) {
      __syncthreads();
      if (t < 64 && t < p.Cout) {
        float s = 0.f, ss = 0.f;
#pragma unroll
        for (int w = 0; w < 4; ++w) {
          s += red[(w * 64 + t) * 2 + 0];
          ss += red[(w * 64 + t) * 2 + 1];
        }
        float* o = p.stat + ((long long)tile * p.Cout + t) * 2;
        o[0] = s;
        o[1] = ss;
      }
    }
    cur ^= 1;
  }
}

__global__ void stem_pack_kernel(const float* __restrict__ w, float* __restrict__ out, int Cout, int kT, int kH, int kW,
                                 int ntaps, long long total) {
  for (long long i = blockIdx.x * (long long)blockDim.x + threadIdx.x; i < total; i += (long long)gridDim.x * blockDim.x) {
    const int ci = (int)(i & 3), n = (int)((i >> 2) & 63), tap = (int)(i >> 8);
    float v = 0.f;
    if (tap < ntaps && n < Cout) {
      const int kw = tap % kW, r = tap / kW;
      const int kh = r % kH, kt = r / kH;
      v = w[((((long long)n * 4 + ci) * kT + kt) * kH + kh) * kW + kw];
    }
    out[i] = v;
  }
}

struct StemPlan {
  bool ok;
  int G, TCH, nchunks, tw_shift, HT, WT, WTh, WTL, npix, npix_r, FR, tiles_h, tiles_w;
  bool resident;
  bool wide_ok;
  long long tiles;
  size_t lds;
};

StemPlan stem_plan(const rsp_conv3d_desc* d) {
  StemPlan s;
  memset(&s, 0, sizeof s);
  if (d->Cin != 4 || d->in_ld != 4 || d->Cout > 64 || d->out_ld < d->Cout) return s;
  if (d->sW < 1 || d->sW > 2 || d->sH < 1 || d->sH > 2) return s;
  const int ntaps = d->kT * d->kH * d->kW;
  if (ntaps > 343) return s;
  if ((unsigned long long)d->N * d->Di * d->Hi * d->Wi * 16ull >= 0xF0000000ull) return s;
  const long long waste16 = (long long)rsp_cdiv(d->Ho, 8) * 8 * rsp_cdiv(d->Wo, 16) * 16;
  const long long waste8 = (long long)rsp_cdiv(d->Ho, 16) * 16 * rsp_cdiv(d->Wo, 8) * 8;
  s.tw_shift = waste8 < waste16 ? 3 : 4;
  const long long covered = waste8 < waste16 ? waste8 : waste16;
  if (ntaps > 64 && covered * 100 > (long long)d->Ho * d->Wo * 104) return s;
  const int TW = 1 << s.tw_shift, TH = 128 >> s.tw_shift;
  s.HT = (TH - 1) * d->sH + d->kH;
  s.WT = (TW - 1) * d->sW + d->kW;
  s.WTh = (s.WT + 1) / 2;
  s.WTL = d->sW == 2 ? 2 * s.WTh : s.WT;
  s.npix = s.HT * s.WTL;
  if (s.npix > 1024) return s;
  s.npix_r = (s.npix + 63) / 64 * 64;
  s.FR = d->kT < 3 ? d->kT : 3;
  int best = 0, best_pad = 1 << 30;
  const int cand[3] = {8, 7, 5};
  for (int i = 0; i < 3; ++i) {
    const int tch = 2 * cand[i];
    if (d->kT > 3 && d->kH * d->kW < 2 * tch) continue;
    const int pad = rsp_cdiv(ntaps, tch) * tch;
    if (pad < best_pad) {
      best_pad = pad;
      best = cand[i];
    }
// ... 17 lines not shown
  return s;
}

std::mutex g_three_mu;
std::unordered_map<const void*, bool> g_three;

bool stem_three_channels(const void* w_packed) {
  std::lock_guard<std::mutex> lk(g_three_mu);
  auto it = g_three.find(w_packed);
  return it != g_three.end() && it->second;
}

template <int G, int NS>
int launch_stem(const StemParams& p, const StemPlan& pl, hipStream_t s) {
  static bool attr_set = false;
  if (!attr_set) {
    (void)hipFuncSetAttribute(reinterpret_cast<const void*>(&stem_kernel<G, NS>), hipFuncAttributeMaxDynamicSharedMemorySize,
                              150 * 1024);
    attr_set = true;
  }
  if (pl.resident) {
    static bool attr_set_r = false;
    if (!attr_set_r) {
      (void)hipFuncSetAttribute(reinterpret_cast<const void*>(&stem_resident_kernel<G, true, NS>),
                                hipFuncAttributeMaxDynamicSharedMemorySize, 80 * 1024);
      (void)hipFuncSetAttribute(reinterpret_cast<const void*>(&stem_resident_kernel<G, false, NS>),
                                hipFuncAttributeMaxDynamicSharedMemorySize, 80 * 1024);
      attr_set_r = true;
    }
    long long per_cu = (160 * 1024) / (long long)pl.lds;
    per_cu = per_cu > 3 ? 3 : per_cu;
    const long long grid = pl.tiles < 256 * per_cu ? pl.tiles : 256 * per_cu;
    rsp_note_kernel(p.wide ? "stem_resident_kernel<%d, true, %d>" : "stem_resident_kernel<%d, false, %d>", G, NS);
    if (p.wide) hipLaunchKernelGGL((stem_resident_kernel<G, true, NS>), dim3((unsigned)grid), dim3(256), pl.lds, s, p);
    else hipLaunchKernelGGL((stem_resident_kernel<G, false, NS>), dim3((unsigned)grid), dim3(256), pl.lds, s, p);
    return rsp_check_launch("stem_resident_kernel");
  }
  rsp_note_kernel("stem_kernel<%d, %d>", G, NS);
  hipLaunchKernelGGL((stem_kernel<G, NS>), dim3((unsigned)pl.tiles), dim3(256), pl.lds, s, p);
  return rsp_check_launch("stem_kernel");
}

}

bool rsp_stem_applicable(const rsp_conv3d_desc* d) { return stem_plan(d).ok; }

int rsp_stem_tiles(const rsp_conv3d_desc* d) { return (int)stem_plan(d).tiles; }

const char* rsp_stem_kernel_name(const rsp_conv3d_desc* d) {
  const StemPlan pl = stem_plan(d);
  if (pl.resident && pl.wide_ok)
    return pl.G == 8 ? "stem_resident_kernel<8, true, 3>" : (pl.G == 7 ? "stem_resident_kernel<7, true, 3>" : "stem_resident_kernel<5, true, 3>");
  if (pl.resident)
    return pl.G == 8 ? "stem_resident_kernel<8, false, 3>" : (pl.G == 7 ? "stem_resident_kernel<7, false, 3>" : "stem_resident_kernel<5, false, 3>");
  return pl.G == 8 ? "stem_kernel<8, 3>" : (pl.G == 7 ? "stem_kernel<7, 3>" : "stem_kernel<5, 3>");
}

void rsp_stem_note_packed(const void* w_packed, bool three_channels) {
  std::lock_guard<std::mutex> lk(g_three_mu);
  if (three_channels) g_three[w_packed] = true;
  else g_three.erase(w_packed);
}

void rsp_stem_forget_packed(const void* w_packed) {
  std::lock_guard<std::mutex> lk(g_three_mu);
  g_three.erase(w_packed);
}

size_t rsp_stem_packed_elems(const rsp_conv3d_desc* d) {
  const StemPlan pl = stem_plan(d);
  return (size_t)pl.nchunks * pl.TCH * 256;
}

int rsp_stem_pack(const rsp_conv3d_desc* d, const float* w_ref, float* w_packed, hipStream_t s) {
  const StemPlan pl = stem_plan(d);
  const long long total = (long long)pl.nchunks * pl.TCH * 256;
  const int blocks = (int)((total + 255) / 256 > 2048 ? 2048 : (total + 255) / 256);
  rsp_stem_note_packed(w_packed, false);
  hipLaunchKernelGGL(stem_pack_kernel, dim3(blocks), dim3(256), 0, s, w_ref, w_packed, d->Cout, d->kT, d->kH, d->kW,
                     d->kT * d->kH * d->kW, total);
  return rsp_check_launch("stem_pack_kernel");
}

int rsp_stem_fwd(const rsp_conv3d_desc* d, const float* x, const float* w_packed, const float* bias, float* y,
                 float* stat_partials, hipStream_t s) {
  const StemPlan pl = stem_plan(d);
  RSP_REQUIRE(pl.ok, "rsp_stem_fwd: descriptor not on the stem path");
  RSP_REQUIRE(rsp_aligned16(x) && rsp_aligned16(w_packed), "rsp_conv3d_fwd: 4-channel input and packed weight must be 16-byte aligned");
  StemParams p;
  memset(&p, 0, sizeof p);
  p.x = x; p.w = w_packed; p.bias = bias; p.y = y; p.stat = stat_partials;
  p.N = d->N; p.Di = d->Di; p.Hi = d->Hi; p.Wi = d->Wi; p.Do = d->Do; p.Ho = d->Ho; p.Wo = d->Wo;
  p.kT = d->kT; p.kH = d->kH; p.kW = d->kW; p.sT = d->sT; p.sH = d->sH; p.sW = d->sW;
  p.pT = d->pT; p.pH = d->pH; p.pW = d->pW;
  p.Cout = d->Cout; p.out_ld = d->out_ld;
  p.tw_shift = pl.tw_shift;
  p.HT = pl.HT; p.WT = pl.WT; p.WTh = pl.WTh; p.WTL = pl.WTL;
  p.npix = pl.npix; p.npix_r = pl.npix_r; p.FR = pl.FR;
  p.ntaps = d->kT * d->kH * d->kW; p.nchunks = pl.nchunks;
  p.tiles_h = pl.tiles_h; p.tiles_w = pl.tiles_w; p.tiles = (int)pl.tiles;
  p.wide = pl.wide_ok && rsp_aligned16(y) && (!bias || rsp_aligned16(bias));
  p.x_bytes = (unsigned)((unsigned long long)d->N * d->Di * d->Hi * d->Wi * 16ull);
  p.w_bytes = (unsigned)((size_t)pl.nchunks * pl.TCH * 1024);
  if (stem_three_channels(w_packed)) {
    switch (pl.G) {
      case 8: return launch_stem<8, 3>(p, pl, s);
      case 7: return launch_stem<7, 3>(p, pl, s);
      default: return launch_stem<5, 3>(p, pl, s);
    }
  }
  switch (pl.G) {
    case 8: return launch_stem<8, 4>(p, pl, s);
    case 7: return launch_stem<7, 4>(p, pl, s);
    default: return launch_stem<5, 4>(p, pl, s);
  }
}
```

### rspnet_amd/engine.py

```python
from __future__ import annotations

import contextlib
import os
from dataclasses import dataclass, field
from typing import Dict, List, NamedTuple, Optional, Tuple, Union

import torch
from torch import nn

from . import ops as _ops
from .ops import ConvGeom, PoolGeom

Triple = Tuple[int, int, int]


@dataclass
class ConvBN:
    conv: nn.Module
    bn: nn.Module
    src: int
    dst: int
    k: Triple
    s: Triple = (1, 1, 1)
    p: Triple = (0, 0, 0)
    relu: bool = True
    pool: Optional[Tuple[Triple, Triple]] = None
    residual: Optional[int] = None
    into: Optional[Tuple[int, int, int]] = None
    branch: int = 0
    virtual_w: bool = False
    cout_pad: int = 0


@dataclass
class ConvBNGroup:
    members: List[ConvBN]
    cat: Optional["_CatConv"] = field(default=None, repr=False, compare=False)


@dataclass
class ConvBias:
    conv: nn.Module
    src: int
    dst: int
    k: Triple
    s: Triple = (1, 1, 1)
    p: Triple = (0, 0, 0)
    relu: bool = False


@dataclass
class Pool:
    src: int
    dst: int
    k: Triple
    s: Triple
    p: Triple = (0, 0, 0)
    branch: int = 0


@dataclass
class Gate:
    conv: nn.Module
    src: int
    dst: int
    into: Optional[Tuple[int, int, int]] = None
    branch: int = 0


@dataclass
class Plan:
    nodes: List[object]
    input_slot: int = 0
    output_slot: int = 0
    gate_fusion: Optional[dict] = field(default=None, repr=False, compare=False)
    pool_fusion: Optional[dict] = field(default=None, repr=False, compare=False)


@dataclass
class _Saved:
    x: torch.Tensor
    y: torch.Tensor
    mi: torch.Tensor
    ss: torch.Tensor
    cg: ConvGeom
    pg: PoolGeom
    res: Optional[torch.Tensor] = None
    eval_mode: bool = False
    gate: Optional["_SavedGate"] = None


_SavedVStem = NamedTuple("_SavedVStem", [("x_e", torch.Tensor), ("x_o", torch.Tensor), ("y", torch.Tensor), ("mi", torch.Tensor),
                                         ("ss", torch.Tensor), ("cg", ConvGeom), ("pg", PoolGeom), ("vs", "VirtualStem")])
_SavedMember = NamedTuple("_SavedMember", [("off", int), ("C", int), ("mi", torch.Tensor), ("ss", torch.Tensor), ("pg", PoolGeom)])
_SavedGroup = NamedTuple("_SavedGroup", [("x", torch.Tensor), ("y", torch.Tensor), ("cg", ConvGeom), ("per", List[_SavedMember])])
_SavedPool = NamedTuple("_SavedPool", [("pg", PoolGeom), ("idx", torch.Tensor)])
_SavedGate = NamedTuple("_SavedGate", [("at", int), ("x", Optional[torch.Tensor]), ("mean", torch.Tensor), ("gate", torch.Tensor)])
_SavedConvBias = NamedTuple("_SavedConvBias", [("x", torch.Tensor), ("y", torch.Tensor), ("cg", ConvGeom)])
SavedState = Union[_Saved, _SavedVStem, _SavedGroup, _SavedPool, _SavedGate, _SavedConvBias]


@dataclass
class ForwardCtx:
    saved: Dict[Union[int, Tuple[int, int]], SavedState] = field(default_factory=dict)
    feat_shape: Optional[Tuple[int, ...]] = None
    packed: Optional["PackedWeights"] = None
    head: object = None


class PackedWeights:

    def __init__(self):
        self._entries = []
        self._index = {}
        self._sets = []
        self._ptrs = []
        self._dirty = True
        self._virtual = {}

    def invalidate(self):
        self._dirty = True

    def refresh_now(self):
        if self._dirty and self._entries:
            self._refresh()

    def _refresh(self):
        be = _ops.backend()
        for vs in self._virtual.values():
            vs.refresh()
        ptrs = [c.weight.data_ptr() for _, _, c in self._entries]
        if len(self._sets) > 1 or ptrs != self._ptrs:
            self._sets = [be.pack_set([(g, which, c.weight.data) for g, which, c in self._entries])] if self._entries else []
            self._index = {(id(c), which, be.pack_signature(g, which, c.weight.data)): (0, i)
                           for i, (g, which, c) in enumerate(self._entries)}
            self._ptrs = ptrs
        for ps in self._sets:
            ps.run()
        self._dirty = False

    def _lookup(self, conv, cg: ConvGeom, which: int):
        if self._dirty:
            self._refresh()
        key = (id(conv), which, _ops.backend().pack_signature(cg, which, conv.weight.data))
        at = self._index.get(key)
        if at is None:
            ps = _ops.backend().pack_set([(cg, which, conv.weight.data)])
            ps.run()
            self._sets.append(ps)
            self._entries.append((cg, which, conv))
            self._ptrs.append(conv.weight.data_ptr())
            at = self._index[key] = (len(self._sets) - 1, 0)
        return self._sets[at[0]].packed[at[1]]

    def get(self, conv, cg: ConvGeom):
        return self._lookup(conv, cg, 0)

    def get_dgrad(self, conv, cg: ConvGeom):
        return self._lookup(conv, cg, 1)

    def virtual_stem(self, node) -> "VirtualStem":
        vs = self._virtual.get(id(node.conv))
        if vs is None or vs.device != node.conv.weight.device:
            vs = self._virtual[id(node.conv)] = VirtualStem(node)
        return vs


class _CatConv:
    weight: torch.Tensor = None


def _adjacent_cat(ts):
    t0 = ts[0]
    if not all(t.is_contiguous() and t.shape[1:] == t0.shape[1:] and t.dtype == t0.dtype for t in ts):
        return None
    end = t0.data_ptr() + t0.numel() * t0.element_size()
    for t in ts[1:]:
        if t.data_ptr() != end or t.untyped_storage().data_ptr() != t0.untyped_storage().data_ptr():
            return None
        end += t.numel() * t.element_size()
    shape = (sum(t.shape[0] for t in ts),) + tuple(t0.shape[1:])
    stride = tuple(t0.stride())
    return torch.as_strided(t0, shape, stride, t0.storage_offset())


INPUT_CHANNEL_PAD = 4
GATE_BWD_FUSED = not os.environ.get("RSP_NO_GATE_BWD_FUSION")


class VirtualStem:

    def __init__(self, node):
        self.conv = node.conv
        w = node.conv.weight
        Cout, cin, kT, kH, kW = w.shape
        assert cin == 3 and kW == 7 and node.s[2] == 2 and node.p[2] == 3
        self.holders, self.idx, self.src, self.dst = [], [], [], []
        co = torch.arange(Cout).view(Cout, 1, 1, 1, 1)
        c4 = torch.arange(4).view(1, 4, 1, 1, 1)
        kt = torch.arange(kT).view(1, 1, kT, 1, 1)
        kh = torch.arange(kH).view(1, 1, 1, kH, 1)
        j = torch.arange(6).view(1, 1, 1, 1, 6)
        for off in (3, 1):
            r = 4 * j + c4 - off
            valid = ((r >= 0) & (r < 21)).expand(Cout, 4, kT, kH, 6)
            real = ((((co * 3 + r % 3) * kT + kt) * kH + kh) * 7 + torch.div(r, 3, rounding_mode="floor")).expand(Cout, 4, kT, kH, 6)
            idx = torch.where(valid, real, torch.full_like(real, w.numel())).reshape(-1)
            flat_valid = valid.reshape(-1).nonzero().view(-1)
            self.idx.append(idx.to(w.device))
            self.src.append(flat_valid.to(w.device))
            self.dst.append(real.reshape(-1)[flat_valid].to(w.device))
            h = _CatConv()
            h.weight = torch.zeros((Cout, 4, kT, kH, 6), dtype=w.dtype, device=w.device)
            self.holders.append(h)
        self.device = w.device
        self.refresh()

    enabled = not os.environ.get("RSP_NO_VIRTUAL_STEM")

    @staticmethod
    def applies(node, xin) -> bool:
        w = node.conv.weight
        W = xin.shape[3]
        return (VirtualStem.enabled and node.virtual_w and w.shape[1] == 3 and xin.shape[4] == 4 and w.shape[4] == 7 and node.s[2] == 2 and node.p[2] == 3
                and (3 * W) % 4 == 0 and W % 2 == 0 and getattr(node.conv, "bias", None) is None and node.residual is None
                and node.into is None)

    def refresh(self):
        w = self.conv.weight
        ext = torch.cat([w.data.reshape(-1), w.data.new_zeros(1)])
        for h, idx in zip(self.holders, self.idx):
            torch.index_select(ext, 0, idx, out=h.weight.view(-1))

    def pack_rows(self, xin):
        N, D, H, W, _ = xin.shape
        Wp = 3 * W // 4 + 5
        flat = torch.zeros(N * D * H * Wp * 4 + 8, dtype=xin.dtype, device=xin.device)
        xv = flat[:N * D * H * Wp * 4].view(N, D, H, Wp, 4)
        xv.view(N, D, H, Wp * 4)[..., 12:12 + 3 * W].view(N, D, H, W, 3).copy_(xin[..., :3])
        return xv, torch.as_strided(flat, (N, D, H, Wp, 4), xv.stride(), 8)


class BranchStreams:
    _streams: Dict[Tuple, "torch.cuda.Stream"] = {}
    origin = None
    SMALL_WGRAD_FLOPS = float(os.environ.get("RSP_WGRAD_ASIDE_GFLOP", "50")) * 1e9

    MID_WGRAD_FLOPS = float(os.environ.get("RSP_WGRAD_MID_GFLOP", "400")) * 1e9
    MID_WGRAD_BYTES = float(os.environ.get("RSP_WGRAD_MID_MB", "450")) * 1e6
    EAGER_TASKS = not os.environ.get("RSP_NO_EAGER_OVERLAP")
    RUN_AHEAD = bool(int(os.environ.get("RSP_TASK_RUN_AHEAD", "1")))
    AHEAD_MAX_FLOPS = float(os.environ.get("RSP_TASK_AHEAD_MAX_GFLOP", "100")) * 1e9
    deferred = None

    def __init__(self, x: torch.Tensor):
        self.dev = x.device
        self.on = bool(x.is_cuda and _ops.backend().name == "hip" and BranchStreams.origin is not None
                       and torch.cuda.is_current_stream_capturing()
                       and torch.cuda.current_stream(self.dev).cuda_stream == BranchStreams.origin)
        self.origin_h = BranchStreams.origin
        self.fork_branches = self.on and bool(os.environ.get("RSP_BRANCH_FORKS"))
        if (not self.on and BranchStreams.EAGER_TASKS and x.is_cuda and _ops.backend().name == "hip"
                and not torch.cuda.is_current_stream_capturing()):
            self.on = True
            self.origin_h = torch.cuda.current_stream(self.dev).cuda_stream
        self.active: Dict[int, "torch.cuda.Stream"] = {}
        self.task = None

    def _get(self, key):
        key = (self.dev.index if self.dev.index is not None else torch.cuda.current_device(), key)
# ... 93 lines not shown
            if n.residual is not None or n.pool or n.into is not None or n.cout_pad or n.virtual_w or n.dst == plan.output_slot:
                continue
            if readers.get(n.dst) != [i + 1]:
                continue
            pi = None
            if i + 2 < len(plan.nodes):
                q = plan.nodes[i + 2]
                if (isinstance(q, Pool) and g.into is None and q.src == g.dst and q.branch == n.branch and readers.get(g.dst) == [i + 2]
                        and g.dst != plan.output_slot):
                    pi = i + 2
            table[i] = (i + 1, pi)
    plan.gate_fusion = table
    return table


GATE_POOL_APART = bool(os.environ.get("RSP_NO_GATE_POOL_KEEP"))


def _pool_fusion(plan: "Plan"):
    if plan.pool_fusion is not None:
        return plan.pool_fusion
    readers = _readers(plan)
    table = {}
    if not os.environ.get("RSP_NO_POOL_FUSION"):
        gated = _gate_fusion(plan)
        for i, n in enumerate(plan.nodes[:-1]):
            q = plan.nodes[i + 1]
            if not (isinstance(n, ConvBN) and isinstance(q, Pool) and q.src == n.dst and q.branch == n.branch) or i in gated:
                continue
            if n.pool or n.into is not None or n.cout_pad or n.dst == plan.output_slot or readers.get(n.dst) != [i + 1]:
                continue
            table[i] = i + 1
    plan.pool_fusion = table
    return table


def _view(t, into, C):
    return t if into is None else t[..., into[1]:into[1] + C]


def _out_view(slots, into, lead_shape, C, device):
    if into is None:
        return None
    slot, off, total = into
    if slot not in slots:
        slots[slot] = torch.empty(tuple(lead_shape) + (total,), dtype=torch.float32, device=device)
    return _view(slots[slot], into, C)


def _eval_scale_shift(bn, bias) -> torch.Tensor:
    scale = bn.weight.data * torch.rsqrt(bn.running_var + float(bn.eps))
    shift = bn.bias.data - bn.running_mean * scale
    if bias is not None:
        shift = shift + bias.data * scale
    return torch.stack([scale, shift]).contiguous()


def _eval_mean_invstd(bn, bias) -> torch.Tensor:
    mean = bn.running_mean if bias is None else bn.running_mean - bias.data
    return torch.stack([mean, torch.rsqrt(bn.running_var + float(bn.eps))]).contiguous()


EVAL_BACKWARD_MISSING = ("backward through an eval-mode backbone (BatchNorm on running statistics) is not implemented: "
                         "freeze the backbone (only_train_fc) or call model.train()")


def _handler(table, node):
    fn = table.get(type(node))
    if fn is None:
        raise NotImplementedError(f"plan node {type(node).__name__}")
    return fn


class _Forward:

    def __init__(self, plan, x, packed, keep, training, deferred):
        self.be = _ops.backend()
        self.plan, self.packed, self.keep, self.training, self.deferred = plan, packed, keep, training, deferred
        self.slots: Dict[int, torch.Tensor] = {plan.input_slot: x}
        self.ctx = ForwardCtx(packed=packed) if keep else None
        self.pool_fusion = _pool_fusion(plan)
        self.gate_fusion = _gate_fusion(plan) if training else {}
        self.skipped = set()

    def finalize(self, bn, stats, rows, bias_d):
        bso = self.deferred.get(id(bn)) if self.deferred is not None else None
        if bso is not None:
            return self.be.bn_finalize(stats, rows, bias_d, bn.weight.data, bn.bias.data, float(bn.eps), float(bn.momentum), None, None,
                                       batch_stats_out=bso)
        return self.be.bn_finalize(stats, rows, bias_d, bn.weight.data, bn.bias.data, float(bn.eps), float(bn.momentum),
                                   bn.running_mean, bn.running_var)

    def bn_apply(self, node, y, ss, C, dims, xin, key=None):
        be, slots = self.be, self.slots
        pk, ps = node.pool if node.pool else ((1, 1, 1), (1, 1, 1))
        pg = PoolGeom(*dims, C, pk, ps, (0, 0, 0))
        res = slots[node.residual] if node.residual is not None else None
        pi = self.pool_fusion.get(key) if key is not None else None
        if pi is not None:
            pnode = self.plan.nodes[pi]
            pgf = PoolGeom(*dims, C, pnode.k, pnode.s, pnode.p)
            if not self.keep:
                slots[pnode.dst] = be.bn_act_pool_fwd(pgf, y, ss, res, node.relu)
                self.skipped.add(pi)
                return pgf, res
            fused = be.bn_act_maxpool_fwd(pgf, y, ss, node.relu, True) if (res is None and hasattr(be, "bn_act_maxpool_fwd")) else None
            if fused is not None:
                slots[pnode.dst], idx = fused
                self.ctx.saved[pi] = _SavedPool(pgf, idx)
                self.skipped.add(pi)
                return pg, res
        out = _out_view(slots, node.into, (dims[0],) + pg.out_dims, C, xin.device)
        if out is not None:
            be.bn_act_pool_fwd(pg, y, ss, res, node.relu, out=out)
        else:
            slots[node.dst] = be.bn_act_pool_fwd(pg, y, ss, res, node.relu)
        return pg, res

    def convbn_virtual(self, node, key, xin):
        N, D, H, W, _ = xin.shape
        Cp = max(node.cout_pad, node.conv.weight.shape[0])
        vs = self.packed.virtual_stem(node)
        x_e, x_o = vs.pack_rows(xin)
        (kT, kH, _), (sT, sH, _), (pT, pH, _) = node.k, node.s, node.p
        cg = ConvGeom(N, D, H, x_e.shape[3], 4, Cp, (kT, kH, 6), (sT, sH, 3), (pT, pH, 0), Cin_alg=3 * 7 / 6)
        do, ho, g = cg.out_dims
        y = torch.empty((N, do, ho, 2 * g, Cp), dtype=torch.float32, device=xin.device)
        yv = y.view(N, do, ho, g, 2 * Cp)
        parts = []
        for c, xc in enumerate((x_e, x_o)):
            _, st = self.be.conv_fwd(cg, xc, self.packed.get(vs.holders[c], cg), None, True, out=yv[..., c * Cp:(c + 1) * Cp], out_ld=2 * Cp)
            parts.append(st)
        rows = N * do * ho * 2 * g
        mi, ss = self.finalize(node.bn, torch.cat(parts), rows, None)
        pg, _ = self.bn_apply(node, y, ss, Cp, (N, do, ho, 2 * g), xin, key)
        if self.keep:
            self.ctx.saved[key] = _SavedVStem(x_e, x_o, y, mi, ss, cg, pg, vs)

    def convbn(self, node, key):
        be, keep = self.be, self.keep
        xin = self.slots[node.src]
        if self.training and node.virtual_w and VirtualStem.applies(node, xin):
            return self.convbn_virtual(node, key, xin)
        N, D, H, W, Cin = xin.shape
        w = node.conv.weight
        Cout = w.shape[0]
        Cp = max(node.cout_pad, Cout)
        cg = ConvGeom(N, D, H, W, Cin, Cp, node.k, node.s, node.p, Cin_alg=w.shape[1])
        bias = getattr(node.conv, "bias", None)
        bn = node.bn
        bias_d = None if bias is None else bias.data
        if self.training:
            bias_conv = bias_d if (bias_d is None or Cp == Cout) else torch.cat([bias_d, bias_d.new_zeros(Cp - Cout)])
            y, stats = be.conv_fwd(cg, xin, self.packed.get(node.conv, cg), bias_conv, True)
            mi, ss = self.finalize(bn, stats, cg.rows, bias_d)
        else:
            y, _ = be.conv_fwd(cg, xin, self.packed.get(node.conv, cg), None, False)
            ss = _eval_scale_shift(bn, bias)
            mi = _eval_mean_invstd(bn, bias) if keep else None
            if Cp != Cout:
                pad = torch.zeros((2, Cp - Cout), dtype=ss.dtype, device=ss.device)
                ss, mi = (None if v is None else torch.cat([v, pad], dim=1).contiguous() for v in (ss, mi))
        dims = (N,) + cg.out_dims
        gated = self.gate_fusion.get(key)
        if gated is not None:
            return self.bn_gate(node, key, gated, xin, y, mi, ss, cg, dims)
        pg, res = self.bn_apply(node, y, ss, cg.Cout, dims, xin, key)
        if keep:
            self.ctx.saved[key] = _Saved(xin, y, mi, ss, cg, pg, res, eval_mode=not self.training)

    def bn_gate(self, node, key, gated, xin, y, mi, ss, cg, dims):
        be, keep, slots = self.be, self.keep, self.slots
        gi, pi = gated
        gnode = self.plan.nodes[gi]
        pnode = self.plan.nodes[pi] if pi is not None else None
        pg = PoolGeom(*dims, cg.Cout)
        pool = PoolGeom(*dims, cg.Cout, pnode.k, pnode.s, pnode.p) if pnode is not None else None
        keep_act = keep and not GATE_BWD_FUSED
        with_idx = (keep and pool is not None and not keep_act and getattr(be, "gate_pool_keep", False) and not GATE_POOL_APART
                    and be.bn_act_gate_pool_idx_ok(pool, y, ss))
        if keep and not with_idx:
            pnode = pool = None
        out = _out_view(slots, gnode.into, dims, cg.Cout, xin.device)
        gw, gb = gnode.conv.weight.data, gnode.conv.bias.data
        if with_idx:
            o, a, mean, gate, idx = be.bn_act_gate_fwd(pg, y, ss, node.relu, gw, gb, False, pool=pool, out=out, pool_idx=True)
            self.ctx.saved[pi] = _SavedPool(pool, idx)
        else:
            o, a, mean, gate = be.bn_act_gate_fwd(pg, y, ss, node.relu, gw, gb, keep_act, pool=pool, out=out)
        if pnode is not None:
            slots[pnode.dst] = o
            self.skipped.add(pi)
        elif gnode.into is None:
            slots[gnode.dst] = o
        self.skipped.add(gi)
        if keep:
            sg = self.ctx.saved[gi] = _SavedGate(gi, a if keep_act else None, mean, gate)
            self.ctx.saved[key] = _Saved(xin, y, mi, ss, cg, pg, None, gate=None if keep_act else sg)

    def group(self, node, ni):
        ms = node.members
        wcat = _adjacent_cat([m.conv.weight.data for m in ms]) if self.training else None
        if wcat is None:
            for j, m in enumerate(ms):
                self.convbn(m, (ni, j))
            return
        xin = self.slots[ms[0].src]
        N, D, H, W, Cin = xin.shape
        if node.cat is None:
            node.cat = _CatConv()
        node.cat.weight = wcat
        cg = ConvGeom(N, D, H, W, Cin, wcat.shape[0], ms[0].k, ms[0].s, ms[0].p)
        y, stats = self.be.conv_fwd(cg, xin, self.packed.get(node.cat, cg), None, True)
        off, per = 0, []
        for m in ms:
            C = m.conv.weight.shape[0]
            mi, ss = self.finalize(m.bn, stats[:, off:off + C], cg.rows, None)
            pg, _ = self.bn_apply(m, y[..., off:off + C], ss, C, (N,) + cg.out_dims, xin)
            per.append(_SavedMember(off, C, mi, ss, pg))
            off += C
        if self.keep:
            self.ctx.saved[ni] = _SavedGroup(xin, y, cg, per)

    def convbias(self, node, ni):
        xin = self.slots[node.src]
        N, D, H, W, Cin = xin.shape
        cg = ConvGeom(N, D, H, W, Cin, node.conv.weight.shape[0], node.k, node.s, node.p)
        y, _ = self.be.conv_fwd(cg, xin, self.packed.get(node.conv, cg), node.conv.bias.data, False)
        if node.relu:
            y = self.be.eltwise("relu_fwd", y, out=y)
        self.slots[node.dst] = y
        if self.keep:
            self.ctx.saved[ni] = _SavedConvBias(xin, y, cg)

    def pool(self, node, ni):
        xin = self.slots[node.src]
        N, D, H, W, Cc = xin.shape
        pg = PoolGeom(N, D, H, W, Cc, node.k, node.s, node.p)
        self.slots[node.dst], idx = self.be.maxpool_fwd(pg, xin, self.keep)
        if self.keep:
            self.ctx.saved[ni] = _SavedPool(pg, idx)

    def gate(self, node, ni):
        xin = self.slots[node.src]
        out = _out_view(self.slots, node.into, tuple(xin.shape[:4]), xin.shape[4], xin.device)
        o, mean, gate = self.be.gate_fwd(xin, node.conv.weight.data, node.conv.bias.data, out=out)
        if node.into is None:
            self.slots[node.dst] = o
        if self.keep:
            self.ctx.saved[ni] = _SavedGate(ni, xin, mean, gate)

    HANDLERS = {ConvBN: convbn, ConvBNGroup: group, ConvBias: convbias, Pool: pool, Gate: gate}

    def run_node(self, ni, node):
        if ni not in self.skipped:
            _handler(self.HANDLERS, node)(self, node, ni)


def run_forward(plan: Plan, x: torch.Tensor, packed: PackedWeights, keep: bool, training: bool = True,
                deferred: Optional[Dict[int, torch.Tensor]] = None) -> Tuple[torch.Tensor, Optional[ForwardCtx]]:
    fw = _Forward(plan, x, packed, keep, training, deferred)
    branches = BranchStreams(x)
    for ni, node in enumerate(plan.nodes):
        branches.run(node, lambda: fw.run_node(ni, node))
    branches.finish()
    out = fw.slots[plan.output_slot]
    if keep:
        fw.ctx.feat_shape = tuple(out.shape)
    return out, fw.ctx


def run_backward(plan: Plan, ctx: ForwardCtx, dfeat: torch.Tensor, grad_of, after_param_grads=None,
                 want_input_grad: bool = False, packed: Optional[PackedWeights] = None):
    it = run_backward_iter(plan, ctx, dfeat, grad_of, after_param_grads, want_input_grad, packed)
    try:
        while True:
            next(it)
    except StopIteration as done:
        return done.value


class _Backward:

    def __init__(self, plan, ctx, dfeat, grad_of, after_param_grads, want_input_grad, packed):
        self.be = _ops.backend()
        self.plan, self.ctx, self.grad_of, self.hook, self.want_input_grad = plan, ctx, grad_of, after_param_grads, want_input_grad
        self.packed = packed if packed is not None else ctx.packed
        self.dslots: Dict[int, torch.Tensor] = {plan.output_slot: dfeat}
        self.branches = BranchStreams(dfeat)

    def add_grad(self, slot, g):
        if g is None:
            return
        if slot in self.dslots:
            self.dslots[slot] = self.be.eltwise("add", self.dslots[slot].contiguous(), g, out=g)
        else:
            self.dslots[slot] = g

    def take_grad(self, node, C):
        return _view(self.dslots[node.into[0]], node.into, C) if node.into is not None else self.dslots.pop(node.dst)

    def issued(self, ni):
        if self.hook is not None:
            self.hook(ni, self.branches.grads_ready)

    def input_grad(self, src, cg, dy, conv):
        if src != self.plan.input_slot or self.want_input_grad:
            self.add_grad(src, self.be.conv_dgrad_packed(cg, dy, self.packed.get_dgrad(conv, cg)))

    def convbn(self, node, ni, key=None):
        key = ni if key is None else key
        sv = self.ctx.saved.pop(key)
        if isinstance(sv, _SavedVStem):
            return self.convbn_virtual(node, sv, ni)
        if sv.gate is not None:
            return self.convbn_gated(node, sv, ni)
        if sv.eval_mode:
            return self.convbn_eval(node, sv, ni)
        bn, grad_of = node.bn, self.grad_of
        dout = self.take_grad(node, sv.cg.Cout)
        dy, dres = self.be.bn_act_pool_bwd(sv.pg, sv.y, sv.res, dout, bn.weight.data, sv.mi, sv.ss, node.relu,
                                           node.residual is not None, grad_of(bn.weight), grad_of(bn.bias))
        self.convbn_tail(node, sv, ni, dy, dres, True)

    def convbn_virtual(self, node, sv, ni):
        be, grad_of, vs, cg = self.be, self.grad_of, sv.vs, sv.cg
        assert node.src == self.plan.input_slot and not self.want_input_grad, "a virtual-pixel stem reads the clip: no input gradient"
        dout = self.dslots.pop(node.dst)
        bn = node.bn
        dy, _ = be.bn_act_pool_bwd(sv.pg, sv.y, None, dout, bn.weight.data, sv.mi, sv.ss, node.relu, False, grad_of(bn.weight), grad_of(bn.bias))
        gw = grad_of(node.conv.weight)
        if gw is not None:
            N, do, ho, Wo, Cp = dy.shape
            dyv = dy.view(N, do, ho, Wo // 2, 2 * Cp)
            gflat = gw.view(-1)
            gflat.zero_()
            for c, xc in enumerate((sv.x_e, sv.x_o)):
                gv = torch.empty_like(vs.holders[c].weight)
                be.conv_wgrad(cg, xc, dyv[..., c * Cp:(c + 1) * Cp], gv)
                gflat.index_add_(0, vs.dst[c], gv.view(-1).index_select(0, vs.src[c]))
        self.issued(ni)

    def convbn_gated(self, node, sv, ni):
        bn, grad_of, sg = node.bn, self.grad_of, sv.gate
        gnode = self.plan.nodes[sg.at]
        dout = self.take_grad(gnode, sv.cg.Cout)
        dy = self.be.bn_act_gate_bwd(sv.pg, sv.y, dout, bn.weight.data, sv.mi, sv.ss, node.relu, gnode.conv.weight.data, sg.mean, sg.gate,
                                     grad_of(bn.weight), grad_of(bn.bias), grad_of(gnode.conv.weight), grad_of(gnode.conv.bias))
        self.issued(sg.at)
        self.convbn_tail(node, sv, ni, dy, None, True)

    def convbn_eval(self, node, sv, ni):
        be, grad_of = self.be, self.grad_of
        if not hasattr(be, "bn_eval_act_pool_bwd"):
            raise RuntimeError(EVAL_BACKWARD_MISSING)
        bn = node.bn
        dout = self.take_grad(node, sv.cg.Cout)
        bias = getattr(node.conv, "bias", None)
        gbias = grad_of(bias) if bias is not None else None
        dgamma, dbeta = grad_of(bn.weight), grad_of(bn.bias)
        sums = dbeta if (dbeta is not None or gbias is None) else torch.empty_like(bn.bias.data)
        dy, dres = be.bn_eval_act_pool_bwd(sv.pg, sv.y, sv.res, dout, sv.mi, sv.ss, node.relu, node.residual is not None, dgamma, sums)
        if gbias is not None:
            torch.mul(sv.ss[0][:gbias.shape[0]], sums, out=gbias)
        self.convbn_tail(node, sv, ni, dy, dres, False)

    def convbn_tail(self, node, sv, ni, dy, dres, zero_bias):
        be, grad_of = self.be, self.grad_of
        if node.residual is not None:
            self.add_grad(node.residual, dres)
        bias = getattr(node.conv, "bias", None)
        if bias is not None and zero_bias:
            gb = grad_of(bias)
            if gb is not None:
                gb.zero_()
        gw = grad_of(node.conv.weight)
        if (sv.cg.flops < BranchStreams.SMALL_WGRAD_FLOPS or
                (sv.cg.flops < BranchStreams.MID_WGRAD_FLOPS and sv.cg.bytes < BranchStreams.MID_WGRAD_BYTES)):
            self.branches.side_task(lambda: be.conv_wgrad(sv.cg, sv.x, dy, gw), (sv.x, dy), cost=float(sv.cg.flops))
        else:
            be.conv_wgrad(sv.cg, sv.x, dy, gw)
        self.issued(ni)
        self.input_grad(node.src, sv.cg, dy, node.conv)

    def group(self, node, ni):
        sv = self.ctx.saved.pop(ni, None)
        ms = node.members
        if sv is None:
            for j in range(len(ms) - 1, -1, -1):
                self.convbn(ms[j], ni, (ni, j))
            return
        be, grad_of = self.be, self.grad_of
        dy_cat = torch.empty_like(sv.y)
        for m, p in zip(ms, sv.per):
            be.bn_act_pool_bwd(p.pg, sv.y[..., p.off:p.off + p.C], None, self.take_grad(m, p.C), m.bn.weight.data, p.mi, p.ss, m.relu, False,
                               grad_of(m.bn.weight), grad_of(m.bn.bias), dy_out=dy_cat[..., p.off:p.off + p.C])
        gws = [grad_of(m.conv.weight) for m in ms]
        gcat = _adjacent_cat(gws) if all(g is not None for g in gws) else None
        if gcat is not None:
            be.conv_wgrad(sv.cg, sv.x, dy_cat, gcat)
        else:
            tmp = torch.empty_like(node.cat.weight)
            be.conv_wgrad(sv.cg, sv.x, dy_cat, tmp)
            off = 0
            for m, g in zip(ms, gws):
# ... 40 lines not shown
```

### rspnet_amd/ops.py

```python
from __future__ import annotations

import collections
import contextlib
import ctypes as C
import functools
from dataclasses import dataclass
from typing import Optional, Tuple

import torch

from . import _lib


@dataclass(frozen=True)
class ConvGeom:
    N: int
    Di: int
    Hi: int
    Wi: int
    Cin: int
    Cout: int
    k: Tuple[int, int, int]
    s: Tuple[int, int, int]
    p: Tuple[int, int, int]
    Cin_alg: float = 0

    @property
    def out_dims(self):
        return tuple((i + 2 * p - k) // s + 1 for i, k, s, p in zip((self.Di, self.Hi, self.Wi), self.k, self.s, self.p))

    @property
    def rows(self):
        d, h, w = self.out_dims
        return self.N * d * h * w

    @property
    def flops(self):
        return int(2 * self.rows * self.Cout * (self.Cin_alg or self.Cin) * self.k[0] * self.k[1] * self.k[2])

    @property
    def bytes(self):
        taps = self.k[0] * self.k[1] * self.k[2]
        cin = self.Cin_alg or self.Cin
        return int(4 * (self.N * self.Di * self.Hi * self.Wi * cin + self.rows * self.Cout + self.Cout * cin * taps))

    def desc(self, in_ld=None, out_ld=None) -> _lib.ConvDesc:
        do, ho, wo = self.out_dims
        return _lib.ConvDesc(self.N, self.Di, self.Hi, self.Wi, self.Cin, do, ho, wo, self.Cout, *self.k, *self.s, *self.p,
                             in_ld or self.Cin, out_ld or self.Cout)


@dataclass(frozen=True)
class PoolGeom:
    N: int
    Di: int
    Hi: int
    Wi: int
    C: int
    k: Tuple[int, int, int] = (1, 1, 1)
    s: Tuple[int, int, int] = (1, 1, 1)
    p: Tuple[int, int, int] = (0, 0, 0)

    @property
    def out_dims(self):
        return tuple((i + 2 * p - k) // s + 1 for i, k, s, p in zip((self.Di, self.Hi, self.Wi), self.k, self.s, self.p))

    def desc(self, in_ld=None, out_ld=None, res_ld=None) -> _lib.PoolDesc:
        do, ho, wo = self.out_dims
        return _lib.PoolDesc(self.N, self.Di, self.Hi, self.Wi, self.C, do, ho, wo, *self.k, *self.s, *self.p,
                             in_ld or self.C, out_ld or self.C, res_ld or self.C)


@functools.lru_cache(maxsize=4096)
def _conv_plan(g: "ConvGeom", in_ld, out_ld):
    lib = _lib.load()
    d = g.desc(in_ld=in_ld, out_ld=out_ld)
    ref = C.byref(d)
    names = tuple(lib.rsp_conv3d_kernel_name(ref, which).decode() for which in (0, 1, 2))
    return (d, ref, lib.rsp_conv3d_stat_tiles(ref), lib.rsp_conv3d_fwd_workspace(ref), lib.rsp_conv3d_dgrad_workspace(ref),
            lib.rsp_conv3d_wgrad_workspace(ref), g.out_dims, names)


@functools.lru_cache(maxsize=4096)
def executed_fraction(g: "ConvGeom", which: int) -> float:
    d = g.desc()
    return float(_lib.load().rsp_conv3d_executed_fraction(C.byref(d), which))


@functools.lru_cache(maxsize=8192)
def _pack_signature(g: "ConvGeom", which: int, cout_src: int, cin_src: int):
    lib = _lib.load()
    d = g.desc()
    buf = (_lib.PackJob * 64)()
    cnt = lib.rsp_conv3d_pack_jobs(C.byref(d), which, cout_src, cin_src, C.c_void_p(1 << 20), C.c_void_p(1 << 30), buf, 64)
    lib.rsp_conv3d_pack_forget(C.c_void_p(1 << 30))
    if cnt < 0:
        _lib.check(cnt, "rsp_conv3d_pack_jobs")
    n = (lib.rsp_conv3d_packed_dgrad_elems if which else lib.rsp_conv3d_packed_fwd_elems)(C.byref(d))
    return (int(n), bytes(buf)[:cnt * C.sizeof(_lib.PackJob)])


@functools.lru_cache(maxsize=4096)
def _pool_plan(pg: "PoolGeom", in_ld, out_ld, res_ld):
    lib = _lib.load()
    d = pg.desc(in_ld=in_ld, out_ld=out_ld, res_ld=res_ld)
    ref = C.byref(d)
    return d, ref, lib.rsp_bn_bwd_workspace(ref), pg.out_dims


def _ptr(t: Optional[torch.Tensor]):
    return None if t is None else C.c_void_p(t.data_ptr())


_raw_stream = getattr(torch._C, "_cuda_getCurrentRawStream", None)
_get_device = getattr(torch._C, "_cuda_getDevice", None)


def _stream():
    if _raw_stream is not None and _get_device is not None:
        return C.c_void_p(_raw_stream(_get_device()))
    return C.c_void_p(torch.cuda.current_stream().cuda_stream)


def _chk(t: torch.Tensor, name: str, dtype=torch.float32):
    if not t.is_cuda:
        raise _lib.RspError(f"{name}: expected a HIP device tensor (rspnet_amd has no CPU path)")
    if t.dtype != dtype:
        raise _lib.RspError(f"{name}: expected {dtype}, got {t.dtype}")
    if not t.is_contiguous():
        raise _lib.RspError(f"{name}: expected a contiguous tensor")
    return t


def _rows_ld(t: torch.Tensor, name: str) -> int:
    if not t.is_cuda or t.dtype != torch.float32:
        raise _lib.RspError(f"{name}: expected a float32 HIP device tensor (rspnet_amd has no CPU path)")
    if t.is_contiguous():
        return t.shape[-1]
    ld = t.stride(-2)
    exp, ok = ld, t.stride(-1) == 1
    for dim in range(t.dim() - 2, -1, -1):
        ok = ok and (t.stride(dim) == exp or t.shape[dim] == 1)
        exp *= t.shape[dim]
    if not ok:
        raise _lib.RspError(f"{name}: expected a dense NDHWC tensor or a channel slice of one")
    return ld


def _dy_target(y, in_ld: int, dy_out):
    if dy_out is not None:
        if _rows_ld(dy_out, "dy_out") != in_ld or dy_out.shape != y.shape:
            raise _lib.RspError("dy_out: expected the shape and channel pitch of y")
        return dy_out
    if not y.is_contiguous():
        raise _lib.RspError("y is a channel slice: pass dy_out with the same pitch")
    return torch.empty_like(y)


KnnResult = collections.namedtuple("KnnResult", "pred rank hits votes idx dist")


class HipOps:

    name = "hip"

    def __init__(self):
        self.lib = _lib.load(init_gpu=True)
        self._ws = {}
        self._rowgeom = collections.OrderedDict()
        self._rowgeom_bytes = 0
        self._rowgeom_streams = {}
        self.event_log = None
        self.hbm_log = None

    def _ev(self):
        if self.event_log is None:
            return None
        e = torch.cuda.Event(enable_timing=True)
        e.record()
        return e

    def _log(self, kind, g, e0, kernel=""):
        if e0 is not None:
            e1 = torch.cuda.Event(enable_timing=True)
            e1.record()
            which = {"conv_fwd": 0, "conv_dgrad": 1, "conv_wgrad": 2}[kind]
            self.event_log.append((kind, g.flops, e0, e1, kernel, g.bytes, g, g.flops * executed_fraction(g, which)))

    def _log_hbm(self, kind, nbytes, e0):
        if e0 is not None and self.hbm_log is not None:
            e1 = torch.cuda.Event(enable_timing=True)
            e1.record()
            self.hbm_log.append((kind, int(nbytes), e0, e1))

    def _workspace(self, dev, nbytes: int) -> torch.Tensor:
        if torch.cuda.is_current_stream_capturing():
            return torch.empty(max(int(nbytes), 256), dtype=torch.uint8, device=dev)
        key = (dev, _stream().value)
        buf = self._ws.get(key)
        if buf is None or buf.numel() < nbytes:
            if buf is not None:
                buf.record_stream(torch.cuda.current_stream(dev))
            buf = torch.empty(max(int(nbytes), 1 << 20), dtype=torch.uint8, device=dev)
            self._ws[key] = buf
        return buf

    def set_option(self, name: str, value: int) -> int:
        prev = self.lib.rsp_conv3d_set_option(name.encode(), int(value))
        if prev < 0:
            _lib.check(prev, "rsp_conv3d_set_option")
        _conv_plan.cache_clear()
        executed_fraction.cache_clear()
        return prev

    @contextlib.contextmanager
    def options(self, **kw):
        before = {}
        try:
            for name, value in kw.items():
                prev = self.set_option(name, value)
                self.set_option(name, -1)
                unset = self.set_option(name, value)
                before[name] = -1 if prev == unset else prev
            yield self
        finally:
            for name, value in before.items():
                self.set_option(name, value)

    def conv_pack_fwd(self, g: ConvGeom, w_ref: torch.Tensor) -> torch.Tensor:
        _chk(w_ref, "w_ref")
        d = g.desc()
        n = self.lib.rsp_conv3d_packed_fwd_elems(C.byref(d))
        out = torch.empty(n, dtype=torch.float32, device=w_ref.device)
        _lib.check(self.lib.rsp_conv3d_pack_fwd(C.byref(d), _ptr(w_ref), _ptr(out), _stream()), "rsp_conv3d_pack_fwd")
        return out

    def conv_fwd(self, g: ConvGeom, x, w_packed, bias, want_stats: bool, out: Optional[torch.Tensor] = None,
                 out_ld: Optional[int] = None, in_ld: Optional[int] = None):
        _chk(x, "x")
        d, dref, tiles, wsb, _, _, (do, ho, wo), names = _conv_plan(g, in_ld, out_ld)
        if out is None:
            out = torch.empty((g.N, do, ho, wo, g.Cout), dtype=torch.float32, device=x.device)
        stats = None
        if want_stats:
            stats = torch.empty((tiles, g.Cout, 2), dtype=torch.float32, device=x.device)
        ws = self._workspace(x.device, wsb) if wsb else None
        e0 = self._ev()
        _lib.check(self.lib.rsp_conv3d_fwd(dref, _ptr(x), _ptr(w_packed), _ptr(bias), _ptr(out), _ptr(stats),
                                           _ptr(ws), wsb, _stream()), "rsp_conv3d_fwd")
        self._log("conv_fwd", g, e0, names[0])
        return out, stats

    def conv_dgrad(self, g: ConvGeom, dy, w_ref):
        _chk(dy, "dy")
        _chk(w_ref, "w_ref")
        d, dref, _, _, wsb, _, _, names = _conv_plan(g, None, None)
        dx = torch.empty((g.N, g.Di, g.Hi, g.Wi, g.Cin), dtype=torch.float32, device=dy.device)
        ws = self._workspace(dy.device, wsb)
        e0 = self._ev()
        _lib.check(self.lib.rsp_conv3d_dgrad(dref, _ptr(dy), _ptr(w_ref), _ptr(dx), _ptr(ws), wsb, _stream()),
                   "rsp_conv3d_dgrad")
        self._log("conv_dgrad", g, e0, names[1])
        return dx

    def conv_dgrad_packed(self, g: ConvGeom, dy, w_packed):
        _chk(dy, "dy")
        d, dref, _, _, wsb, _, _, names = _conv_plan(g, None, None)
        dx = torch.empty((g.N, g.Di, g.Hi, g.Wi, g.Cin), dtype=torch.float32, device=dy.device)
        ws = self._workspace(dy.device, wsb)
        e0 = self._ev()
        _lib.check(self.lib.rsp_conv3d_dgrad_packed(dref, _ptr(dy), _ptr(_chk(w_packed, "w_packed")), _ptr(dx), _ptr(ws), wsb,
                                                    _stream()), "rsp_conv3d_dgrad_packed")
        self._log("conv_dgrad", g, e0, names[1])
        return dx

    def pack_signature(self, g: ConvGeom, which: int, w_ref):
        return _pack_signature(g, which, int(w_ref.shape[0]), int(w_ref.shape[1]))

    def pack_set(self, entries):
        return PackSet(self, entries)

    def conv_wgrad(self, g: ConvGeom, x, dy, dw_out: torch.Tensor, dbias_out: Optional[torch.Tensor] = None):
        _chk(x, "x")
        _chk(dw_out, "dw_out")
        dy_ld = _rows_ld(dy, "dy")
        d, dref, _, _, _, wsb, _, names = _conv_plan(g, None, None if dy_ld == g.Cout else dy_ld)
        ws = self._workspace(x.device, wsb)
        if dw_out.shape[0] > g.Cout or dw_out.shape[1] > g.Cin or (dbias_out is not None and tuple(dw_out.shape[:2]) != (g.Cout, g.Cin)):
            raise _lib.RspError("conv_wgrad: dw_out has more channels than the geometry, or a bias gradient with padded channels")
        table = self._rowgeom_table(g, d, dref, x.device)
        e0 = self._ev()
        _lib.check(self.lib.rsp_conv3d_wgrad(dref, _ptr(x), _ptr(dy), _ptr(dw_out), _ptr(dbias_out), dw_out.shape[0], dw_out.shape[1],
                                             _ptr(table), _ptr(ws), wsb, _stream()), "rsp_conv3d_wgrad")
        self._log("conv_wgrad", g, e0, names[2])

    ROWGEOM_MAX_TABLES = 128
    ROWGEOM_MAX_BYTES = 2 << 30

    def _rowgeom_table(self, g: ConvGeom, d, dref, dev):
        if max(g.k) > 8:
            return None
        key = (dev, g.N, g.Di, g.Hi, g.Wi, g.k, g.s, g.p, d.in_ld)
        ent = self._rowgeom.get(key)
        capturing = torch.cuda.is_current_stream_capturing()
        here = _stream().value
        if ent is None:
            if capturing:
                return None
            nbytes = int(self.lib.rsp_conv3d_rowgeom_bytes(dref))
            t = torch.empty(nbytes, dtype=torch.uint8, device=dev)
            _lib.check(self.lib.rsp_conv3d_rowgeom(dref, _ptr(t), _stream()), "rsp_conv3d_rowgeom")
            ev = torch.cuda.Event()
            ev.record()
            ent = self._rowgeom[key] = [t, ev, here, False]
            self._rowgeom_bytes += nbytes
            self._rowgeom_evict(dev)
        else:
            self._rowgeom.move_to_end(key)
            if ent[1] is not None and not capturing:
                if ent[1].query():
                    ent[1] = None
                elif here != ent[2]:
                    torch.cuda.current_stream(dev).wait_event(ent[1])
            if capturing:
                ent[3] = True
        if here not in self._rowgeom_streams and not capturing:
            self._rowgeom_streams[here] = torch.cuda.current_stream(dev)
        return ent[0]

    def _rowgeom_evict(self, dev):
        if len(self._rowgeom) <= self.ROWGEOM_MAX_TABLES and self._rowgeom_bytes <= self.ROWGEOM_MAX_BYTES:
            return
        for key in list(self._rowgeom)[:-1]:
            if len(self._rowgeom) <= self.ROWGEOM_MAX_TABLES and self._rowgeom_bytes <= self.ROWGEOM_MAX_BYTES:
                break
            t, _, _, pinned = self._rowgeom[key]
            if pinned:
                continue
            for st in self._rowgeom_streams.values():
                t.record_stream(st)
            self._rowgeom_bytes -= t.numel()
            del self._rowgeom[key]

    def bn_finalize(self, stats, count: int, conv_bias, gamma, beta, eps: float, momentum: float, running_mean,
                    running_var, batch_stats_out=None):
        tiles, Cc, _ = stats.shape
        if stats.is_contiguous():
            _chk(stats, "stats")
            stat_ld = Cc
        else:
            if not stats.is_cuda or stats.dtype != torch.float32 or stats.stride(2) != 1 or stats.stride(1) != 2 or stats.stride(0) % 2:
                raise _lib.RspError("stats: expected [tiles][C][2] float32 partials or a channel slice of them")
            stat_ld = stats.stride(0) // 2
        mi = torch.empty((2, Cc), dtype=torch.float32, device=stats.device)
        ss = torch.empty((2, Cc), dtype=torch.float32, device=stats.device)
        wsb = int(self.lib.rsp_bn_finalize_workspace(tiles, Cc))
        ws = self._workspace(stats.device, wsb)
        c_valid = Cc if gamma is None else int(gamma.shape[0])
        _lib.check(self.lib.rsp_bn_finalize(_ptr(stats), tiles, Cc, c_valid, stat_ld, count, _ptr(conv_bias), _ptr(gamma), _ptr(beta),
                                            eps, momentum, _ptr(running_mean), _ptr(running_var), _ptr(batch_stats_out), _ptr(mi),
                                            _ptr(ss), _ptr(ws), wsb, _stream()), "rsp_bn_finalize")
        return mi, ss

    def bn_ema_set(self, entries):
        return BnEmaSet(self, entries)

    def bn_act_pool_fwd(self, pg: PoolGeom, y, scale_shift, residual, relu: bool, out=None):
        in_ld = _rows_ld(y, "y")
        if out is None:
            do, ho, wo = pg.out_dims
            out = torch.empty((pg.N, do, ho, wo, pg.C), dtype=torch.float32, device=y.device)
        d, dref, _, _ = _pool_plan(pg, in_ld, _rows_ld(out, "out"), None if residual is None else _rows_ld(residual, "residual"))
        e0 = self._ev()
        _lib.check(self.lib.rsp_bn_act_pool_fwd(dref, _ptr(y), _ptr(scale_shift), _ptr(residual), int(relu), None, _ptr(out),
                                                _stream()), "rsp_bn_act_pool_fwd")
        n_in = pg.N * pg.Di * pg.Hi * pg.Wi * pg.C
        self._log_hbm("bn_act_pool_fwd", 4 * (n_in * (1 if residual is None else 2) + out.numel()), e0)
        return out

    def bn_act_maxpool_fwd(self, pg: PoolGeom, y, scale_shift, relu: bool, keep: bool):
        in_ld = _rows_ld(y, "y")
        do, ho, wo = pg.out_dims
        d = pg.desc(in_ld=in_ld)
        if not self.lib.rsp_bn_act_maxpool_applicable(C.byref(d)) or y.data_ptr() % 16 or scale_shift.data_ptr() % 16:
            return None
        out = torch.empty((pg.N, do, ho, wo, pg.C), dtype=torch.float32, device=y.device)
        idx = torch.empty((pg.N, do, ho, wo, pg.C), dtype=torch.int32, device=y.device) if keep else None
        e0 = self._ev()
        _lib.check(self.lib.rsp_bn_act_maxpool_fwd(C.byref(d), _ptr(y), _ptr(scale_shift), int(relu), None, _ptr(out), _ptr(idx),
                                                   _stream()), "rsp_bn_act_maxpool_fwd")
        self._log_hbm("bn_act_pool_fwd", 4 * (pg.N * pg.Di * pg.Hi * pg.Wi * pg.C + out.numel() * (2 if keep else 1)), e0)
        return out, idx

    def bn_act_pool_bwd(self, pg: PoolGeom, y, residual, dout, gamma, mean_invstd, scale_shift, relu: bool,
                        want_dres: bool, dgamma_out, dbeta_out, dy_out=None):
        in_ld = _rows_ld(y, "y")
        d, dref, wsb, _ = _pool_plan(pg, in_ld, _rows_ld(dout, "dout"), None if residual is None else _rows_ld(residual, "residual"))
        dy = _dy_target(y, in_ld, dy_out)
        dres = torch.empty_like(y) if want_dres else None
        ws = self._workspace(y.device, wsb)
        c_valid = pg.C if gamma is None else int(gamma.shape[0])
        e0 = self._ev()
        _lib.check(self.lib.rsp_bn_act_pool_bwd(dref, _ptr(y), _ptr(residual), _ptr(dout), _ptr(gamma),
                                                _ptr(mean_invstd), _ptr(scale_shift), int(relu), _ptr(dy), _ptr(dres),
                                                _ptr(dgamma_out), _ptr(dbeta_out), c_valid, None, None, _ptr(ws), wsb, _stream()),
                   "rsp_bn_act_pool_bwd")
        n_in = y.numel()
        self._log_hbm("bn_bwd(reduce+apply)", 4 * (2 * (n_in * (1 if residual is None else 2) + dout.numel()) + n_in * (2 if want_dres else 1)), e0)
        return dy, dres

    def bn_eval_act_pool_bwd(self, pg: PoolGeom, y, residual, dout, mean_invstd, scale_shift, relu: bool, want_dres: bool,
                             dgamma_out, dbeta_out, dy_out=None):
        in_ld = _rows_ld(y, "y")
        d, dref, _, _ = _pool_plan(pg, in_ld, _rows_ld(dout, "dout"), None if residual is None else _rows_ld(residual, "residual"))
        dy = _dy_target(y, in_ld, dy_out)
        if want_dres and residual is None:
            raise _lib.RspError("want_dres without a residual")
        dres = torch.empty(y.shape, dtype=torch.float32, device=y.device) if want_dres else None
        if want_dres and d.res_ld != pg.C:
            raise _lib.RspError("residual: a residual whose gradient is wanted must be contiguous")
        sums = dgamma_out is not None or dbeta_out is not None
        c_valid = pg.C
        for v in (dgamma_out, dbeta_out):
            if v is not None:
                c_valid = int(v.shape[0])
        wsb = int(self.lib.rsp_bn_eval_bwd_workspace(dref)) if sums else 0
        ws = self._workspace(y.device, wsb) if sums else None
        e0 = self._ev()
        _lib.check(self.lib.rsp_bn_eval_act_pool_bwd(dref, _ptr(y), _ptr(residual), _ptr(dout), _ptr(mean_invstd), _ptr(scale_shift),
                                                     int(relu), _ptr(dy), _ptr(dres), _ptr(dgamma_out), _ptr(dbeta_out), c_valid,
                                                     _ptr(ws), wsb, _stream()), "rsp_bn_eval_act_pool_bwd")
        n_in = y.numel()
        self._log_hbm("bn_eval_bwd(one pass)", 4 * (n_in * (1 if residual is None else 2) + dout.numel() + n_in * (2 if want_dres else 1)), e0)
        return dy, dres

    def maxpool_fwd(self, pg: PoolGeom, x, keep: bool):
        do, ho, wo = pg.out_dims
        out = torch.empty((pg.N, do, ho, wo, pg.C), dtype=torch.float32, device=x.device)
        idx = torch.empty((pg.N, do, ho, wo, pg.C), dtype=torch.int32, device=x.device) if keep else None
        d = pg.desc(in_ld=_rows_ld(x, "x"))
        _lib.check(self.lib.rsp_maxpool3d_fwd(C.byref(d), _ptr(x), _ptr(out), _ptr(idx), _stream()), "rsp_maxpool3d_fwd")
        return out, idx

    def maxpool_bwd(self, pg: PoolGeom, dout, idx):
        dx = torch.empty((pg.N, pg.Di, pg.Hi, pg.Wi, pg.C), dtype=torch.float32, device=dout.device)
        d = pg.desc(out_ld=_rows_ld(dout, "dout"))
        _lib.check(self.lib.rsp_maxpool3d_bwd(C.byref(d), _ptr(dout), _ptr(idx), _ptr(dx), _stream()), "rsp_maxpool3d_bwd")
        return dx

    def gate_fwd(self, x, w, b, out=None):
        _chk(x, "x")
        N, D, H, W, Cc = x.shape
        P = D * H * W
        if out is None:
            out = torch.empty_like(x)
        mean = torch.empty((N, Cc), dtype=torch.float32, device=x.device)
        gate = torch.empty((N, Cc), dtype=torch.float32, device=x.device)
        wsb = self.lib.rsp_gate_fwd_workspace(N, P, Cc)
        ws = self._workspace(x.device, wsb)
        _lib.check(self.lib.rsp_gate_fwd(_ptr(x), N, P, Cc, Cc, _ptr(_chk(w, "w")), _ptr(_chk(b, "b")), _ptr(out),
                                         _rows_ld(out, "out"), _ptr(mean), _ptr(gate), _ptr(ws), wsb, _stream()),
                   "rsp_gate_fwd")
        return out, mean, gate

    gate_pool_keep = True

    def bn_act_gate_fwd(self, pg: PoolGeom, y, scale_shift, relu: bool, w, b, keep_act: bool, pool: Optional[PoolGeom] = None,
                        out=None, pool_idx: bool = False):
        N, P, Cc = pg.N, pg.Di * pg.Hi * pg.Wi, pg.C
        y_ld = _rows_ld(y, "y")
        if keep_act and pool is not None:
            raise _lib.RspError("bn_act_gate_fwd: the pooled form keeps no activation")
        a = torch.empty((N, pg.Di, pg.Hi, pg.Wi, Cc), dtype=torch.float32, device=y.device) if keep_act else None
        mean = torch.empty((N, Cc), dtype=torch.float32, device=y.device)
        gate = torch.empty((N, Cc), dtype=torch.float32, device=y.device)
        wsb = self.lib.rsp_gate_fwd_workspace(N, P, Cc)
        ws = self._workspace(y.device, wsb)
        _lib.check(self.lib.rsp_bn_gate_sums(_ptr(y), N, P, Cc, y_ld, _ptr(scale_shift), int(relu), _ptr(a), Cc, _ptr(_chk(w, "w")),
                                             _ptr(_chk(b, "b")), _ptr(mean), _ptr(gate), _ptr(ws), wsb, _stream()), "rsp_bn_gate_sums")
        og = pool if pool is not None else pg
        if out is None:
            do, ho, wo = og.out_dims
            out = torch.empty((N, do, ho, wo, Cc), dtype=torch.float32, device=y.device)
        if keep_act:
            _lib.check(self.lib.rsp_gate_apply(_ptr(a), N, P, Cc, Cc, _ptr(gate), _ptr(out), _rows_ld(out, "out"), _stream()),
                       "rsp_gate_apply")
        elif pool_idx:
            d, dref, _, _ = _pool_plan(og, y_ld, _rows_ld(out, "out"), None)
            idx = torch.empty(tuple(out.shape), dtype=torch.int32, device=y.device)
            _lib.check(self.lib.rsp_bn_act_maxpool_fwd(dref, _ptr(y), _ptr(scale_shift), int(relu), _ptr(gate), _ptr(out), _ptr(idx),
# ... 488 lines not shown
```

Baseline: 352.1.

## Fuse stem conv with 2x2 pooling via max/min outputs and save pool-selected inputs

Adds a stem conv kernel that writes only the per-window max and min of the pre-BN conv output, plus statistics. A min/max BN+ReLU kernel then produces the pooled activation, choosing max or min by the sign of the BN scale. This avoids writing and rereading the full-resolution stem activation when no backward save is needed. Separately, the fused BN-act-pool forward now stores the selected pre-BN value per pooled position, so the backward reduction reads a pooled-size tensor instead of rescanning full windows. The cost is extra buffers and more special-cased code paths.

```diff
diff --git a/include/rspnet_hip.h b/include/rspnet_hip.h
--- a/include/rspnet_hip.h
+++ b/include/rspnet_hip.h
@@ -36,6 +36,10 @@
 size_t rsp_conv3d_fwd_workspace(const rsp_conv3d_desc* d);
 int rsp_conv3d_fwd(const rsp_conv3d_desc* d, const float* x, const float* w_packed, const float* bias, float* y,
                    float* stat_partials, void* workspace, size_t workspace_bytes, void* stream);
+
+int rsp_conv3d_stem_pooled_applicable(const rsp_conv3d_desc* d);
+int rsp_conv3d_stem_pooled_fwd(const rsp_conv3d_desc* d, const float* x, const float* w_packed, const float* bias, float* y_max,
+                               float* y_min, float* stat_partials, void* stream);
 
 size_t rsp_conv3d_dgrad_workspace(const rsp_conv3d_desc* d);
 int rsp_conv3d_dgrad(const rsp_conv3d_desc* d, const float* dy, const float* w_ref, float* dx, void* workspace,
@@ -105,6 +109,16 @@
                         const float* gamma, const float* mean_invstd, const float* scale_shift, int relu, float* dy,
                         float* dres, float* dgamma, float* dbeta, int32_t c_valid, const float* gate, const float* dmean,
                         void* workspace, size_t workspace_bytes, void* stream);
+
+int rsp_bn_act_pool_sel_applicable(const rsp_pool3d_desc* d);
+int rsp_bn_act_pool_sel_fwd(const rsp_pool3d_desc* d, const float* y, const float* scale_shift, int relu, float* out, float* y_sel,
+                            void* stream);
+int rsp_bn_act_pool_sel_bwd(const rsp_pool3d_desc* d, const float* y, const float* y_sel, const float* dout, const float* gamma,
+                            const float* mean_invstd, const float* scale_shift, int relu, float* dy, float* dgamma, float* dbeta,
+                            int32_t c_valid, void* workspace, size_t workspace_bytes, void* stream);
+
+int rsp_bn_act_minmax_fwd(const float* y_max, const float* y_min, int64_t positions, int32_t C, int32_t out_ld,
+                          const float* scale_shift, int relu, float* out, void* stream);
 
 size_t rsp_bn_eval_bwd_workspace(const rsp_pool3d_desc* d);
 int rsp_bn_eval_act_pool_bwd(const rsp_pool3d_desc* d, const float* y, const float* residual, const float* dout,
diff --git a/rspnet_amd/_lib.py b/rspnet_amd/_lib.py
--- a/rspnet_amd/_lib.py
+++ b/rspnet_amd/_lib.py
@@ -76,6 +76,8 @@
     "rsp_conv3d_stat_tiles": (_i32, [_PD]),
     "rsp_conv3d_fwd_workspace": (_sz, [_PD]),
     "rsp_conv3d_fwd": (C.c_int, [_PD, _p, _p, _p, _p, _p, _p, _sz, _p]),
+    "rsp_conv3d_stem_pooled_applicable": (C.c_int, [_PD]),
+    "rsp_conv3d_stem_pooled_fwd": (C.c_int, [_PD, _p, _p, _p, _p, _p, _p, _p]),
     "rsp_conv3d_dgrad_workspace": (_sz, [_PD]),
     "rsp_conv3d_dgrad": (C.c_int, [_PD, _p, _p, _p, _p, _sz, _p]),
     "rsp_conv3d_packed_dgrad_elems": (_sz, [_PD]),
@@ -99,6 +101,10 @@
     "rsp_bn_act_maxpool_fwd": (C.c_int, [_PP, _p, _p, C.c_int, _p, _p, _p, _p]),
     "rsp_bn_bwd_workspace": (_sz, [_PP]),
     "rsp_bn_act_pool_bwd": (C.c_int, [_PP, _p, _p, _p, _p, _p, _p, C.c_int, _p, _p, _p, _p, _i32, _p, _p, _p, _sz, _p]),
+    "rsp_bn_act_pool_sel_applicable": (C.c_int, [_PP]),
+    "rsp_bn_act_pool_sel_fwd": (C.c_int, [_PP, _p, _p, C.c_int, _p, _p, _p]),
+    "rsp_bn_act_pool_sel_bwd": (C.c_int, [_PP, _p, _p, _p, _p, _p, _p, C.c_int, _p, _p, _p, _i32, _p, _sz, _p]),
+    "rsp_bn_act_minmax_fwd": (C.c_int, [_p, _p, _i64, _i32, _i32, _p, C.c_int, _p, _p]),
     "rsp_bn_eval_bwd_workspace": (_sz, [_PP]),
     "rsp_bn_eval_act_pool_bwd": (C.c_int, [_PP, _p, _p, _p, _p, _p, C.c_int, _p, _p, _p, _p, _i32, _p, _sz, _p]),
     "rsp_maxpool3d_fwd": (C.c_int, [_PP, _p, _p, _p, _p]),
diff --git a/rspnet_amd/csrc/bn_pool.hip b/rspnet_amd/csrc/bn_pool.hip
--- a/rspnet_amd/csrc/bn_pool.hip
+++ b/rspnet_amd/csrc/bn_pool.hip
@@ -362,6 +362,110 @@
   }
 }
 
+template <int VEC, int MODE>
+__global__ __launch_bounds__(256) void bn_act_pool_sel_fwd_kernel(const PoolParams p, float* __restrict__ ysel) {
+  static_assert(MODE == 2 || MODE == 3, "disjoint windows of 4 or 8 positions");
+  const rsp_pool3d_desc& d = p.d;
+  const int t = threadIdx.x;
+  const int pl = fastdiv(t, p.dcgc);
+  const int cgi = blockIdx.y * 256 + (t - pl * p.cgc);
+  if (pl >= p.ppi || cgi >= p.cg) return;
+  const int c = cgi * VEC;
+  float sc[VEC], sh[VEC];
+  load_vec<VEC>(p.ss + c, sc);
+  load_vec<VEC>(p.ss + d.C + c, sh);
+  constexpr int NW = MODE == 2 ? 4 : 8;
+  long long off[NW];
+  window_offsets<NW>(d, off);
+  for (long long o = (long long)blockIdx.x * p.ppi + pl; o < p.npos; o += (long long)gridDim.x * p.ppi) {
+    const int op = (int)o;
+    const int q1 = fastdiv(op, p.dWo), ow = op - q1 * d.Wo;
+    const int q2 = fastdiv(q1, p.dHo), oh = q1 - q2 * d.Ho;
+    const int n = fastdiv(q2, p.dDo), od = q2 - n * d.Do;
+    const long long base = (((long long)n * d.Di + od * d.sT) * d.Hi + oh * d.sH) * d.Wi + ow * d.sW;
+    float v[NW][VEC], best[VEC], top[VEC], by[VEC];
+#pragma unroll
+    for (int w = 0; w < NW; ++w) load_vec<VEC>(p.y + (base + off[w]) * d.in_ld + c, v[w]);
+#pragma unroll
+    for (int e = 0; e < VEC; ++e) { best[e] = -INFINITY; top[e] = -INFINITY; by[e] = 0.f; }
+#pragma unroll
+    for (int w = 0; w < NW; ++w)
+#pragma unroll
+      for (int e = 0; e < VEC; ++e) {
+        float z = fmaf(v[w][e], sc[e], sh[e]);
+        if (p.relu) z = rsp_relu(z);
+        best[e] = rsp_max_nan(best[e], z);
+        if (rsp_max_takes(z, top[e])) { top[e] = z; by[e] = v[w][e]; }
+      }
+    store_vec<VEC>(p.out + o * d.out_ld + c, best);
+    store_vec<VEC>(ysel + o * d.C + c, by);
+  }
+}
+
+struct MinMaxParams {
+  const float* __restrict__ mx;
+  const float* __restrict__ mn;
+  const float* __restrict__ ss;
+  float* __restrict__ out;
+  int C, out_ld, relu, cg, cgc, ppi;
+  long long npos;
+  FastDiv dcgc;
+};
+
+template <int VEC>
+__device__ __forceinline__ void minmax_act(const float (&a)[VEC], const float (&b)[VEC], const float (&sc)[VEC], const float (&sh)[VEC],
+                                           int relu, float (&o)[VEC]) {
+#pragma unroll
+  for (int e = 0; e < VEC; ++e) {
+    float z;
+    if (sc[e] > 0.f) {
+      z = fmaf(a[e], sc[e], sh[e]);
+    } else if (sc[e] < 0.f) {
+      z = fmaf(b[e], sc[e], sh[e]);
+    } else {
+      const float z1 = fmaf(a[e], sc[e], sh[e]), z2 = fmaf(b[e], sc[e], sh[e]);
+      z = z1 != z1 ? z1 : z2;
+    }
+    o[e] = relu ? rsp_relu(z) : z;
+  }
+}
+
+template <int VEC>
+__global__ __launch_bounds__(256) void bn_act_minmax_fwd_kernel(const MinMaxParams p) {
+  const int t = threadIdx.x;
+  const int pl = fastdiv(t, p.dcgc);
+  const int cgi = blockIdx.y * 256 + (t - pl * p.cgc);
+  if (pl >= p.ppi || cgi >= p.cg) return;
+  const int c = cgi * VEC;
+  float sc[VEC], sh[VEC];
+  load_vec<VEC>(p.ss + c, sc);
+  load_vec<VEC>(p.ss + p.C + c, sh);
+  const long long step = p.ppi;
+  const long long stride = (long long)gridDim.x * p.ppi * 4;
+  long long o = (long long)blockIdx.x * p.ppi * 4 + pl;
+  for (; o + 3 * step < p.npos; o += stride) {
+    float a[4][VEC], b[4][VEC];
+#pragma unroll
+    for (int u = 0; u < 4; ++u) {
+      load_vec<VEC>(p.mx + (o + u * step) * p.C + c, a[u]);
+      load_vec<VEC>(p.mn + (o + u * step) * p.C + c, b[u]);
+    }
+#pragma unroll
+    for (int u = 0; u < 4; ++u) {
+      float r[VEC];
+      minmax_act<VEC>(a[u], b[u], sc, sh, p.relu, r);
+      store_vec<VEC>(p.out + (o + u * step) * p.out_ld + c, r);
+    }
+  }
+  for (int u = 0; u < 4 && o < p.npos; ++u, o += step) {
+    float a[VEC], b[VEC], r[VEC];
+    load_vec<VEC>(p.mx + o * p.C + c, a);
+    load_vec<VEC>(p.mn + o * p.C + c, b);
+    minmax_act<VEC>(a, b, sc, sh, p.relu, r);
+    store_vec<VEC>(p.out + o * p.out_ld + c, r);
+  }
+}
+
 struct BwdParams {
   rsp_pool3d_desc d;
   const float* __restrict__ y;
@@ -385,6 +489,7 @@
   const float* __restrict__ gate;
   const float* __restrict__ dmean;
   float invP;
+  const float* __restrict__ ysel;
 };
 
 template <int VEC>
@@ -544,6 +649,73 @@
         s1[e] += dz;
         s2[e] = fmaf(dz, (by[e] - mean[e]) * invstd[e], s2[e]);
       }
+    }
+  }
+#pragma unroll
+  for (int e = 0; e < VEC; ++e) { red[t][e] = s1[e]; red[t][VEC + e] = s2[e]; }
+  __syncthreads();
+  if (t < cgc) {
+    float a1[VEC], a2[VEC];
+#pragma unroll
+    for (int e = 0; e < VEC; ++e) a1[e] = a2[e] = 0.f;
+    for (int l = 0; l < ppi; ++l)
+#pragma unroll
+      for (int e = 0; e < VEC; ++e) { a1[e] += red[l * cgc + t][e]; a2[e] += red[l * cgc + t][VEC + e]; }
+    float* o = p.partial + ((long long)blockIdx.x * d.C + (cg0 + t) * VEC) * 2;
+#pragma unroll
+    for (int e = 0; e < VEC; ++e) { o[2 * e] = a1[e]; o[2 * e + 1] = a2[e]; }
+  }
+}
+
+template <int VEC>
+__global__ __launch_bounds__(256) void bn_bwd_reduce_sel_kernel(const BwdParams p) {
+  const rsp_pool3d_desc& d = p.d;
+  __shared__ float red[256][2 * VEC];
+  const int cg0 = blockIdx.y * 256;
+  const int cgc = min(p.cg - cg0, 256);
+  const int ppi = p.ppi;
+  const int t = threadIdx.x;
+  const int pl = fastdiv(t, p.dcgc);
+  const int cgi = cg0 + (t - pl * p.cgc);
+  const bool active = pl < ppi && (t - pl * p.cgc) < cgc;
+  const int c = cgi * VEC;
+  float s1[VEC], s2[VEC];
+#pragma unroll
+  for (int e = 0; e < VEC; ++e) s1[e] = s2[e] = 0.f;
+  if (active) {
+    float sc[VEC], sh[VEC], mean[VEC], invstd[VEC];
+    load_vec<VEC>(p.ss + c, sc);
+    load_vec<VEC>(p.ss + d.C + c, sh);
+    load_vec<VEC>(p.mi + c, mean);
+    load_vec<VEC>(p.mi + d.C + c, invstd);
+    const long long npos = (long long)d.N * d.Do * d.Ho * d.Wo;
+    const long long stride = (long long)gridDim.x * ppi;
+    long long op = (long long)blockIdx.x * ppi + pl;
+    auto add = [&](const float (&g)[VEC], const float (&by)[VEC]) {
+#pragma unroll
+      for (int e = 0; e < VEC; ++e) {
+        const float z = fmaf(by[e], sc[e], sh[e]);
+        const float best = p.relu ? rsp_relu(z) : z;
+        const float dz = (p.relu && rsp_relu_blocks(best)) ? 0.f : g[e];
+        s1[e] += dz;
+        s2[e] = fmaf(dz, (by[e] - mean[e]) * invstd[e], s2[e]);
+      }
+    };
+    for (; op + 3 * stride < npos; op += 4 * stride) {
+      float g[4][VEC], by[4][VEC];
+#pragma unroll
+      for (int u = 0; u < 4; ++u) {
+        load_vec<VEC>(p.dout + (op + u * stride) * d.out_ld + c, g[u]);
+        load_vec<VEC>(p.ysel + (op + u * stride) * d.C + c, by[u]);
+      }
+#pragma unroll
+      for (int u = 0; u < 4; ++u) add(g[u], by[u]);
+    }
+    for (; op < npos; op += stride) {
+      float g[VEC], by[VEC];
+      load_vec<VEC>(p.dout + op * d.out_ld + c, g);
+      load_vec<VEC>(p.ysel + op * d.C + c, by);
+      add(g, by);
     }
   }
 #pragma unroll
@@ -1130,6 +1302,49 @@
   return rsp_check_launch("bn_finalize_stage2");
 }
 
+int rsp_bn_act_pool_sel_applicable(const rsp_pool3d_desc* d) {
+  if (!pool_ok(d, true)) return 0;
+  const int m = bn_mode(d, false);
+  return (m == 2 || m == 3) && d->C % 4 == 0 && d->in_ld % 4 == 0 && d->out_ld % 4 == 0 ? 1 : 0;
+}
+
+int rsp_bn_act_pool_sel_fwd(const rsp_pool3d_desc* d, const float* y, const float* scale_shift, int relu, float* out, float* y_sel,
+                            void* stream) {
+  RSP_REQUIRE(rsp_bn_act_pool_sel_applicable(d), "rsp_bn_act_pool_sel_fwd: needs disjoint windows of 4 or 8 positions and channel counts / pitches that are multiples of 4");
+  RSP_REQUIRE(y && scale_shift && out && y_sel, "rsp_bn_act_pool_sel_fwd: null pointer");
+  RSP_REQUIRE(rsp_aligned16(y) && rsp_aligned16(out) && rsp_aligned16(scale_shift) && rsp_aligned16(y_sel),
+              "rsp_bn_act_pool_sel_fwd: pointers must be 16-byte aligned");
+  PoolParams p;
+  p.d = *d; p.y = y; p.ss = scale_shift; p.res = nullptr; p.gate = nullptr; p.out = out; p.relu = relu;
+  p.cg = d->C / 4;
+  const Layout L = make_layout(d, p.cg, 4);
+  RSP_REQUIRE(L.npos < (1ll << 31), "rsp_bn_act_pool_sel_fwd: more than 2^31 - 1 output positions");
+  set_layout(p, L);
+  if (bn_mode(d, false) == 2) hipLaunchKernelGGL((bn_act_pool_sel_fwd_kernel<4, 2>), L.grid, dim3(256), 0, (hipStream_t)stream, p, y_sel);
+  else hipLaunchKernelGGL((bn_act_pool_sel_fwd_kernel<4, 3>), L.grid, dim3(256), 0, (hipStream_t)stream, p, y_sel);
+  return rsp_check_launch("bn_act_pool_sel_fwd_kernel");
+}
+
+int rsp_bn_act_minmax_fwd(const float* y_max, const float* y_min, int64_t positions, int32_t C, int32_t out_ld,
+                          const float* scale_shift, int relu, float* out, void* stream) {
+  RSP_REQUIRE(y_max && y_min && scale_shift && out, "rsp_bn_act_minmax_fwd: null pointer");
+  RSP_REQUIRE(positions > 0 && positions < (1ll << 31) && C > 0 && out_ld >= C, "rsp_bn_act_minmax_fwd: bad size");
+  MinMaxParams p;
+  p.mx = y_max; p.mn = y_min; p.ss = scale_shift; p.out = out; p.C = C; p.out_ld = out_ld; p.relu = relu; p.npos = positions;
+  const bool vec = C % 4 == 0 && out_ld % 4 == 0 && rsp_aligned16(y_max) && rsp_aligned16(y_min) && rsp_aligned16(out) &&
+                   rsp_aligned16(scale_shift);
+  p.cg = vec ? C / 4 : C;
+  p.cgc = p.cg < 256 ? p.cg : 256;
+  p.ppi = 256 / p.cgc;
+  p.dcgc = fastdiv_make(p.cgc);
+  long long b = (positions + (long long)p.ppi * 4 - 1) / ((long long)p.ppi * 4);
+  b = b > 16384 ? 16384 : (b < 1 ? 1 : b);
+  const dim3 grid((unsigned)b, (unsigned)rsp_cdiv(p.cg, 256));
+  if (vec) hipLaunchKernelGGL(bn_act_minmax_fwd_kernel<4>, grid, dim3(256), 0, (hipStream_t)stream, p);
+  else hipLaunchKernelGGL(bn_act_minmax_fwd_kernel<1>, grid, dim3(256), 0, (hipStream_t)stream, p);
+  return rsp_check_launch("bn_act_minmax_fwd_kernel");
+}
+
 int rsp_bn_act_pool_fwd(const rsp_pool3d_desc* d, const float* y, const float* scale_shift, const float* residual,
                         int relu, const float* gate, float* out, void* stream) {
   RSP_REQUIRE(pool_ok(d, false), "rsp_bn_act_pool_fwd: bad descriptor");
@@ -1156,10 +1371,10 @@
   return rsp_align_up((size_t)2048 * d->C * 2 * sizeof(float), 256) + (size_t)d->C * 2 * sizeof(double);
 }
 
-int rsp_bn_act_pool_bwd(const rsp_pool3d_desc* d, const float* y, const float* residual, const float* dout,
-                        const float* gamma, const float* mean_invstd, const float* scale_shift, int relu, float* dy,
-                        float* dres, float* dgamma, float* dbeta, int32_t c_valid, const float* gate, const float* dmean,
-                        void* workspace, size_t workspace_bytes, void* stream) {
+static int bn_act_pool_bwd(const rsp_pool3d_desc* d, const float* y, const float* y_sel, const float* residual, const float* dout,
+                           const float* gamma, const float* mean_invstd, const float* scale_shift, int relu, float* dy,
+                           float* dres, float* dgamma, float* dbeta, int32_t c_valid, const float* gate, const float* dmean,
+                           void* workspace, size_t workspace_bytes, void* stream) {
   RSP_REQUIRE(pool_ok(d, true), "rsp_bn_act_pool_bwd: needs disjoint windows (kernel == stride, no padding)");
   RSP_REQUIRE(!gate || (dmean && d->kT * d->kH * d->kW == 1 && d->sT * d->sH * d->sW == 1 && !residual),
               "rsp_bn_act_pool_bwd: a gated unit has a unit window, no residual, and needs dmean");
@@ -1194,7 +1409,14 @@
   p.nblocks = reduce_blocks(d, p.cg);
   dim3 rgrid(p.nblocks, rsp_cdiv(p.cg, 256));
   const int mode = bn_mode(d, gate != nullptr);
-  RSP_BN_LAUNCH(bn_bwd_reduce_kernel, vec, mode, rgrid, s, p);
+  if (y_sel) {
+    RSP_REQUIRE(vec && (mode == 2 || mode == 3) && !residual && rsp_aligned16(y_sel),
+                "rsp_bn_act_pool_sel_bwd: y_sel needs what rsp_bn_act_pool_sel_fwd needs, and no residual");
+    p.ysel = y_sel;
+    hipLaunchKernelGGL(bn_bwd_reduce_sel_kernel<4>, rgrid, dim3(256), 0, s, p);
+  } else {
+    RSP_BN_LAUNCH(bn_bwd_reduce_kernel, vec, mode, rgrid, s, p);
+  }
   int rc = rsp_check_launch("bn_bwd_reduce_kernel");
   if (rc != RSP_OK) return rc;
   hipLaunchKernelGGL(bn_bwd_finalize_kernel, dim3(rsp_cdiv(d->C, FIN_CH)), dim3(1024), 0, s, p.partial, p.nblocks, d->C, c_valid, sums,
@@ -1210,6 +1432,22 @@
   if (vec) hipLaunchKernelGGL(bn_bwd_apply_kernel<4>, dim3(grid_for(total)), dim3(256), 0, s, p);
   else hipLaunchKernelGGL(bn_bwd_apply_kernel<1>, dim3(grid_for(total)), dim3(256), 0, s, p);
   return rsp_check_launch("bn_bwd_apply_kernel");
+}
+
+int rsp_bn_act_pool_bwd(const rsp_pool3d_desc* d, const float* y, const float* residual, const float* dout,
+                        const float* gamma, const float* mean_invstd, const float* scale_shift, int relu, float* dy,
+                        float* dres, float* dgamma, float* dbeta, int32_t c_valid, const float* gate, const float* dmean,
+                        void* workspace, size_t workspace_bytes, void* stream) {
+  return bn_act_pool_bwd(d, y, nullptr, residual, dout, gamma, mean_invstd, scale_shift, relu, dy, dres, dgamma, dbeta, c_valid, gate,
+                         dmean, workspace, workspace_bytes, stream);
+}
+
+int rsp_bn_act_pool_sel_bwd(const rsp_pool3d_desc* d, const float* y, const float* y_sel, const float* dout, const float* gamma,
+                            const float* mean_invstd, const float* scale_shift, int relu, float* dy, float* dgamma, float* dbeta,
+                            int32_t c_valid, void* workspace, size_t workspace_bytes, void* stream) {
+  RSP_REQUIRE(y_sel, "rsp_bn_act_pool_sel_bwd: null pointer");
+  return bn_act_pool_bwd(d, y, y_sel, nullptr, dout, gamma, mean_invstd, scale_shift, relu, dy, nullptr, dgamma, dbeta, c_valid, nullptr,
+                         nullptr, workspace, workspace_bytes, stream);
 }
 
 static int eval_bwd_mode(const rsp_pool3d_desc* d) {
diff --git a/rspnet_amd/csrc/conv_igemm.hip b/rspnet_amd/csrc/conv_igemm.hip
--- a/rspnet_amd/csrc/conv_igemm.hip
+++ b/rspnet_amd/csrc/conv_igemm.hip
@@ -2431,6 +2431,19 @@
   return run_igemm(p, vec4, workspace, workspace_bytes, (hipStream_t)stream);
 }
 
+int rsp_conv3d_stem_pooled_applicable(const rsp_conv3d_desc* d) {
+  return desc_ok(d) && rsp_stem_applicable(d) && rsp_stem_pooled_applicable(d) ? 1 : 0;
+}
+
+int rsp_conv3d_stem_pooled_fwd(const rsp_conv3d_desc* d, const float* x, const float* w_packed, const float* bias, float* y_max,
+                               float* y_min, float* stat_partials, void* stream) {
+  RSP_REQUIRE(desc_ok(d), "rsp_conv3d_stem_pooled_fwd: bad descriptor");
+  RSP_REQUIRE(x && w_packed && y_max && y_min, "rsp_conv3d_stem_pooled_fwd: null pointer");
+  RSP_REQUIRE(rsp_stem_applicable(d), "rsp_conv3d_stem_pooled_fwd: descriptor not covered (rsp_conv3d_stem_pooled_applicable)");
+  rsp_note_reset();
+  return rsp_stem_pooled_fwd(d, x, w_packed, bias, y_max, y_min, stat_partials, (hipStream_t)stream);
+}
+
 double rsp_conv3d_executed_fraction(const rsp_conv3d_desc* d, int which) {
   if (!desc_ok(d)) return 1.0;
   if (which == 2) return rsp_wgrad_executed_fraction(d);
diff --git a/rspnet_amd/csrc/conv_stem.h b/rspnet_amd/csrc/conv_stem.h
--- a/rspnet_amd/csrc/conv_stem.h
+++ b/rspnet_amd/csrc/conv_stem.h
@@ -9,6 +9,9 @@
 int rsp_stem_fwd(const rsp_conv3d_desc* d, const float* x, const float* w_packed, const float* bias, float* y,
                  float* stat_partials, hipStream_t s);
 const char* rsp_stem_kernel_name(const rsp_conv3d_desc* d);
+bool rsp_stem_pooled_applicable(const rsp_conv3d_desc* d);
+int rsp_stem_pooled_fwd(const rsp_conv3d_desc* d, const float* x, const float* w_packed, const float* bias, float* y_max, float* y_min,
+                        float* stat_partials, hipStream_t s);
 void rsp_stem_note_packed(const void* w_packed, bool three_channels);
 void rsp_stem_forget_packed(const void* w_packed);
 const char* rsp_wgrad_kernel_name(const rsp_conv3d_desc* d);
diff --git a/rspnet_amd/csrc/conv_stem.hip b/rspnet_amd/csrc/conv_stem.hip
--- a/rspnet_amd/csrc/conv_stem.hip
+++ b/rspnet_amd/csrc/conv_stem.hip
@@ -22,6 +22,9 @@
   int tiles_h, tiles_w, tiles;
   unsigned x_bytes, w_bytes;
   int wide;
+  float* __restrict__ ymax;
+  float* __restrict__ ymin;
+  int pool_ld;
 };
 
 struct StemBias {
@@ -61,6 +64,38 @@
         const long long addr = rowaddr[wave * 32 + 16 * r + rl];
         if (addr >= 0 && col < p.Cout) *reinterpret_cast<floatx4*>(p.y + addr + col) = v + b.w[j];
       }
+    }
+  }
+}
+
+__device__ __forceinline__ void stem_store_pooled(const StemParams& p, const floatx16 (&acc)[2], float* stage ,
+                                                  int n, int to, int h0, int w0, int wave, int lane, const StemBias& b) {
+  const int l32 = lane & 31, h = lane >> 5;
+  const int q = lane & 15, kr = lane >> 4;
+  long long addr[2];
+#pragma unroll
+  for (int i = 0; i < 2; ++i) {
+    const int ho = h0 + 2 * wave, wo = w0 + 2 * (kr + 4 * i);
+    addr[i] = (ho < p.Ho && wo < p.Wo && 4 * q < p.Cout)
+                  ? ((((long long)n * p.Do + to) * (p.Ho >> 1) + (ho >> 1)) * (p.Wo >> 1) + (wo >> 1)) * p.pool_ld + 4 * q
+                  : -1;
+  }
+#pragma unroll
+  for (int o = 0; o < 2; ++o) {
+#pragma unroll
+    for (int j = 0; j < 2; ++j)
+#pragma unroll
+      for (int e0 = 0; e0 < 8; e0 += 2) {
+        const float v0 = acc[j][e0] + b.n[j], v1 = acc[j][e0 + 1] + b.n[j], v2 = acc[j][e0 + 8] + b.n[j], v3 = acc[j][e0 + 9] + b.n[j];
+        const float r = o == 0 ? __builtin_elementwise_maximum(__builtin_elementwise_maximum(v0, v1), __builtin_elementwise_maximum(v2, v3))
+                               : __builtin_elementwise_minimum(__builtin_elementwise_minimum(v0, v1), __builtin_elementwise_minimum(v2, v3));
+        stage[((e0 >> 2) * 4 + h * 2 + ((e0 & 3) >> 1)) * 64 + 32 * j + l32] = r;
+      }
+    float* dst = o == 0 ? p.ymax : p.ymin;
+#pragma unroll
+    for (int i = 0; i < 2; ++i) {
+      const floatx4 v = *reinterpret_cast<const floatx4*>(stage + (kr + 4 * i) * 64 + 4 * q);
+      if (addr[i] >= 0) *reinterpret_cast<floatx4*>(dst + addr[i]) = v;
     }
   }
 }
@@ -242,7 +277,7 @@
   }
 }
 
-template <int G, bool WIDE, int NS>
+template <int G, bool WIDE, int NS, bool POOL = false>
 __global__ __launch_bounds__(256, 2) void stem_resident_kernel(const StemParams p) {
   constexpr int TCH = 2 * G;
   constexpr int BU = TCH * 64;
@@ -370,6 +405,7 @@
     }
     __syncthreads();
     if (WIDE) stem_store_wide(p, acc, halo + cur * hsz + wave * 512, rowaddr, wave, lane, bias);
+    if (POOL) stem_store_pooled(p, acc, halo + cur * hsz + wave * 512, n, to, hb * TH, wb * TW, wave, lane, bias);
 #pragma unroll
     for (int j = 0; j < 2; ++j) {
       const int col = 32 * j + l32;
@@ -379,7 +415,7 @@
       for (int e = 0; e < 16; ++e) {
         const long long addr = rowaddr[wave * 32 + (e >> 2) * 8 + h * 4 + (e & 3)];
         const float v = addr >= 0 ? acc[j][e] : 0.f;
-        if (!WIDE && addr >= 0 && col < p.Cout) p.y[addr + col] = v + bv;
+        if (!WIDE && !POOL && addr >= 0 && col < p.Cout) p.y[addr + col] = v + bv;
         s += v;
         ss = fmaf(v, v, ss);
       }
@@ -563,14 +599,11 @@
   return rsp_check_launch("stem_pack_kernel");
 }
 
-int rsp_stem_fwd(const rsp_conv3d_desc* d, const float* x, const float* w_packed, const float* bias, float* y,
-                 float* stat_partials, hipStream_t s) {
-  const StemPlan pl = stem_plan(d);
-  RSP_REQUIRE(pl.ok, "rsp_stem_fwd: descriptor not on the stem path");
-  RSP_REQUIRE(rsp_aligned16(x) && rsp_aligned16(w_packed), "rsp_conv3d_fwd: 4-channel input and packed weight must be 16-byte aligned");
+static StemParams stem_params(const rsp_conv3d_desc* d, const StemPlan& pl, const float* x, const float* w_packed, const float* bias,
+                              float* stat_partials) {
   StemParams p;
   memset(&p, 0, sizeof p);
-  p.x = x; p.w = w_packed; p.bias = bias; p.y = y; p.stat = stat_partials;
+  p.x = x; p.w = w_packed; p.bias = bias; p.stat = stat_partials;
   p.N = d->N; p.Di = d->Di; p.Hi = d->Hi; p.Wi = d->Wi; p.Do = d->Do; p.Ho = d->Ho; p.Wo = d->Wo;
   p.kT = d->kT; p.kH = d->kH; p.kW = d->kW; p.sT = d->sT; p.sH = d->sH; p.sW = d->sW;
   p.pT = d->pT; p.pH = d->pH; p.pW = d->pW;
@@ -580,9 +613,19 @@
   p.npix = pl.npix; p.npix_r = pl.npix_r; p.FR = pl.FR;
   p.ntaps = d->kT * d->kH * d->kW; p.nchunks = pl.nchunks;
   p.tiles_h = pl.tiles_h; p.tiles_w = pl.tiles_w; p.tiles = (int)pl.tiles;
-  p.wide = pl.wide_ok && rsp_aligned16(y) && (!bias || rsp_aligned16(bias));
   p.x_bytes = (unsigned)((unsigned long long)d->N * d->Di * d->Hi * d->Wi * 16ull);
   p.w_bytes = (unsigned)((size_t)pl.nchunks * pl.TCH * 1024);
+  return p;
+}
+
+int rsp_stem_fwd(const rsp_conv3d_desc* d, const float* x, const float* w_packed, const float* bias, float* y,
+                 float* stat_partials, hipStream_t s) {
+  const StemPlan pl = stem_plan(d);
+  RSP_REQUIRE(pl.ok, "rsp_stem_fwd: descriptor not on the stem path");
+  RSP_REQUIRE(rsp_aligned16(x) && rsp_aligned16(w_packed), "rsp_conv3d_fwd: 4-channel input and packed weight must be 16-byte aligned");
+  StemParams p = stem_params(d, pl, x, w_packed, bias, stat_partials);
+  p.y = y;
+  p.wide = pl.wide_ok && rsp_aligned16(y) && (!bias || rsp_aligned16(bias));
   if (stem_three_channels(w_packed)) {
     switch (pl.G) {
       case 8: return launch_stem<8, 3>(p, pl, s);
@@ -596,3 +639,38 @@
     default: return launch_stem<5, 4>(p, pl, s);
   }
 }
+
+static bool stem_pooled_ok(const rsp_conv3d_desc* d, const StemPlan& pl) {
+  return pl.ok && pl.resident && pl.wide_ok && pl.tw_shift == 4 && d->Ho % 2 == 0 && d->Wo % 2 == 0 && d->Cout % 4 == 0;
+}
+
+template <int G, int NS>
+static int launch_stem_pooled(const StemParams& p, const StemPlan& pl, hipStream_t s) {
+  long long per_cu = (160 * 1024) / (long long)pl.lds;
+  per_cu = per_cu > 3 ? 3 : per_cu;
+  const long long grid = pl.tiles < 256 * per_cu ? pl.tiles : 256 * per_cu;
+  return rsp_launch_lds<stem_resident_kernel<G, false, NS, true>>(dim3((unsigned)grid), pl.lds, 80 * 1024, s, std::tie(p),
+                                                                  "stem_resident_kernel<%d, false, %d, true>", G, NS);
+}
+
+bool rsp_stem_pooled_applicable(const rsp_conv3d_desc* d) { return stem_pooled_ok(d, stem_plan(d)); }
+
+int rsp_stem_pooled_fwd(const rsp_conv3d_desc* d, const float* x, const float* w_packed, const float* bias, float* y_max, float* y_min,
+                        float* stat_partials, hipStream_t stream) {
+  const StemPlan pl = stem_plan(d);
+  RSP_REQUIRE(stem_pooled_ok(d, pl), "rsp_conv3d_stem_pooled_fwd: descriptor not covered (rsp_conv3d_stem_pooled_applicable)");
+  RSP_REQUIRE(rsp_aligned16(x) && rsp_aligned16(w_packed) && rsp_aligned16(y_max) && rsp_aligned16(y_min),
+              "rsp_conv3d_stem_pooled_fwd: input, packed weight and both outputs must be 16-byte aligned");
+  StemParams p = stem_params(d, pl, x, w_packed, bias, stat_partials);
+  p.ymax = y_max; p.ymin = y_min; p.pool_ld = d->Cout;
+  if (stem_three_channels(w_packed)) {
+    switch (pl.G) {
+      case 7: return launch_stem_pooled<7, 3>(p, pl, stream);
+      default: return launch_stem_pooled<5, 3>(p, pl, stream);
+    }
+  }
+  switch (pl.G) {
+    case 7: return launch_stem_pooled<7, 4>(p, pl, stream);
+    default: return launch_stem_pooled<5, 4>(p, pl, stream);
+  }
+}
diff --git a/rspnet_amd/engine.py b/rspnet_amd/engine.py
--- a/rspnet_amd/engine.py
+++ b/rspnet_amd/engine.py
@@ -88,6 +88,7 @@
     res: Optional[torch.Tensor] = None
     eval_mode: bool = False
     gate: Optional["_SavedGate"] = None
+    y_sel: Optional[torch.Tensor] = None
 
 
 _SavedVStem = NamedTuple("_SavedVStem", [("x_e", torch.Tensor), ("x_o", torch.Tensor), ("y", torch.Tensor), ("mi", torch.Tensor),
@@ -186,6 +187,8 @@
 
 INPUT_CHANNEL_PAD = 4
 GATE_BWD_FUSED = not os.environ.get("RSP_NO_GATE_BWD_FUSION")
+STEM_POOLED = not os.environ.get("RSP_NO_STEM_POOLED")
+BN_BWD_SEL = not os.environ.get("RSP_NO_BN_BWD_SEL")
 
 
 class VirtualStem:
@@ -445,6 +448,7 @@
         self.pool_fusion = _pool_fusion(plan)
         self.gate_fusion = _gate_fusion(plan) if training else {}
         self.skipped = set()
+        self.y_sel = None
 
     def finalize(self, bn, stats, rows, bias_d):
         bso = self.deferred.get(id(bn)) if self.deferred is not None else None
@@ -454,7 +458,7 @@
         return self.be.bn_finalize(stats, rows, bias_d, bn.weight.data, bn.bias.data, float(bn.eps), float(bn.momentum),
                                    bn.running_mean, bn.running_var)
 
-    def bn_apply(self, node, y, ss, C, dims, xin, key=None):
+    def bn_apply(self, node, y, ss, C, dims, xin, key=None, sel=False):
         be, slots = self.be, self.slots
         pk, ps = node.pool if node.pool else ((1, 1, 1), (1, 1, 1))
         pg = PoolGeom(*dims, C, pk, ps, (0, 0, 0))
@@ -477,6 +481,12 @@
         if out is not None:
             be.bn_act_pool_fwd(pg, y, ss, res, node.relu, out=out)
         else:
+            if (sel and self.keep and self.training and BN_BWD_SEL and node.pool and res is None and pi is None
+                    and hasattr(be, "bn_act_pool_sel_fwd")):
+                got = be.bn_act_pool_sel_fwd(pg, y, ss, node.relu)
+                if got is not None:
+                    slots[node.dst], self.y_sel = got
+                    return pg, res
             slots[node.dst] = be.bn_act_pool_fwd(pg, y, ss, res, node.relu)
         return pg, res
 
@@ -513,6 +523,8 @@
         bias = getattr(node.conv, "bias", None)
         bn = node.bn
         bias_d = None if bias is None else bias.data
+        if self.stem_pooled(node, key, xin, cg, bias_d):
+            return
         if self.training:
             bias_conv = bias_d if (bias_d is None or Cp == Cout) else torch.cat([bias_d, bias_d.new_zeros(Cp - Cout)])
             y, stats = be.conv_fwd(cg, xin, self.packed.get(node.conv, cg), bias_conv, True)
@@ -528,9 +540,32 @@
         gated = self.gate_fusion.get(key)
         if gated is not None:
             return self.bn_gate(node, key, gated, xin, y, mi, ss, cg, dims)
-        pg, res = self.bn_apply(node, y, ss, cg.Cout, dims, xin, key)
+        pg, res = self.bn_apply(node, y, ss, cg.Cout, dims, xin, key, sel=True)
         if keep:
-            self.ctx.saved[key] = _Saved(xin, y, mi, ss, cg, pg, res, eval_mode=not self.training)
+            self.ctx.saved[key] = _Saved(xin, y, mi, ss, cg, pg, res, eval_mode=not self.training, y_sel=self.y_sel)
+            self.y_sel = None
+
+    def stem_pooled(self, node, key, xin, cg, bias_d) -> bool:
+        be = self.be
+        if (self.keep or not self.training or not STEM_POOLED or not node.pool or tuple(node.pool[0]) != (1, 2, 2)
+                or tuple(node.pool[1]) != (1, 2, 2) or node.residual is not None or node.cout_pad or node.virtual_w
+                or xin.shape[4] != 4 or cg.Cout > 64 or self.gate_fusion.get(key) is not None or self.pool_fusion.get(key) is not None
+                or not hasattr(be, "stem_pooled_fwd")):
+            return False
+        _, ho, wo = cg.out_dims
+        if ho % 2 or wo % 2:
+            return False
+        got = be.stem_pooled_fwd(cg, xin, self.packed.get(node.conv, cg), bias_d)
+        if got is None:
+            return False
+        ymax, ymin, stats = got
+        _, ss = self.finalize(node.bn, stats, cg.rows, bias_d)
+        out = _out_view(self.slots, node.into, ymax.shape[:4], cg.Cout, xin.device)
+        if out is not None:
+            be.bn_act_minmax_fwd(ymax, ymin, ss, node.relu, out=out)
+        else:
+            self.slots[node.dst] = be.bn_act_minmax_fwd(ymax, ymin, ss, node.relu)
+        return True
 
     def bn_gate(self, node, key, gated, xin, y, mi, ss, cg, dims):
         be, keep, slots = self.be, self.keep, self.slots
@@ -682,8 +717,9 @@
             return self.convbn_eval(node, sv, ni)
         bn, grad_of = node.bn, self.grad_of
         dout = self.take_grad(node, sv.cg.Cout)
+        sel = {} if sv.y_sel is None else {"y_sel": sv.y_sel}
         dy, dres = self.be.bn_act_pool_bwd(sv.pg, sv.y, sv.res, dout, bn.weight.data, sv.mi, sv.ss, node.relu,
-                                           node.residual is not None, grad_of(bn.weight), grad_of(bn.bias))
+                                           node.residual is not None, grad_of(bn.weight), grad_of(bn.bias), **sel)
         self.convbn_tail(node, sv, ni, dy, dres, True)
 
     def convbn_virtual(self, node, sv, ni):
diff --git a/rspnet_amd/ops.py b/rspnet_amd/ops.py
--- a/rspnet_amd/ops.py
+++ b/rspnet_amd/ops.py
@@ -98,6 +98,12 @@
         _lib.check(cnt, "rsp_conv3d_pack_jobs")
     n = (lib.rsp_conv3d_packed_dgrad_elems if which else lib.rsp_conv3d_packed_fwd_elems)(C.byref(d))
     return (int(n), bytes(buf)[:cnt * C.sizeof(_lib.PackJob)])
+
+
+@functools.lru_cache(maxsize=4096)
+def _stem_pooled_ok(g: "ConvGeom") -> bool:
+    d = g.desc()
+    return bool(_lib.load().rsp_conv3d_stem_pooled_applicable(C.byref(d)))
 
 
 @functools.lru_cache(maxsize=4096)
@@ -250,6 +256,32 @@
                                            _ptr(ws), wsb, _stream()), "rsp_conv3d_fwd")
         self._log("conv_fwd", g, e0, names[0])
         return out, stats
+
+    def stem_pooled_fwd(self, g: ConvGeom, x, w_packed, bias):
+        _chk(x, "x")
+        d, dref, tiles, _, _, _, (do, ho, wo), names = _conv_plan(g, None, None)
+        if not _stem_pooled_ok(g) or x.data_ptr() % 16:
+            return None
+        ymax = torch.empty((g.N, do, ho // 2, wo // 2, g.Cout), dtype=torch.float32, device=x.device)
+        ymin = torch.empty_like(ymax)
+        stats = torch.empty((tiles, g.Cout, 2), dtype=torch.float32, device=x.device)
+        e0 = self._ev()
+        _lib.check(self.lib.rsp_conv3d_stem_pooled_fwd(dref, _ptr(x), _ptr(w_packed), _ptr(bias), _ptr(ymax), _ptr(ymin), _ptr(stats),
+                                                       _stream()), "rsp_conv3d_stem_pooled_fwd")
+        self._log("conv_fwd", g, e0, names[0])
+        return ymax, ymin, stats
+
+    def bn_act_minmax_fwd(self, ymax, ymin, scale_shift, relu: bool, out=None):
+        _chk(ymax, "ymax")
+        _chk(ymin, "ymin")
+        if out is None:
+            out = torch.empty_like(ymax)
+        Cc = ymax.shape[-1]
+        e0 = self._ev()
+        _lib.check(self.lib.rsp_bn_act_minmax_fwd(_ptr(ymax), _ptr(ymin), ymax.numel() // Cc, Cc, _rows_ld(out, "out"), _ptr(scale_shift),
+                                                  int(relu), _ptr(out), _stream()), "rsp_bn_act_minmax_fwd")
+        self._log_hbm("bn_act_pool_fwd", 4 * (2 * ymax.numel() + out.numel()), e0)
+        return out
 
     def conv_dgrad(self, g: ConvGeom, dy, w_ref):
         _chk(dy, "dy")
@@ -378,6 +410,19 @@
         self._log_hbm("bn_act_pool_fwd", 4 * (n_in * (1 if residual is None else 2) + out.numel()), e0)
         return out
 
+    def bn_act_pool_sel_fwd(self, pg: PoolGeom, y, scale_shift, relu: bool):
+        in_ld = _rows_ld(y, "y")
+        d, dref, _, (do, ho, wo) = _pool_plan(pg, in_ld, None, None)
+        if not self.lib.rsp_bn_act_pool_sel_applicable(dref) or y.data_ptr() % 16 or scale_shift.data_ptr() % 16:
+            return None
+        out = torch.empty((pg.N, do, ho, wo, pg.C), dtype=torch.float32, device=y.device)
+        ysel = torch.empty_like(out)
+        e0 = self._ev()
+        _lib.check(self.lib.rsp_bn_act_pool_sel_fwd(dref, _ptr(y), _ptr(scale_shift), int(relu), _ptr(out), _ptr(ysel), _stream()),
+                   "rsp_bn_act_pool_sel_fwd")
+        self._log_hbm("bn_act_pool_fwd", 4 * (pg.N * pg.Di * pg.Hi * pg.Wi * pg.C + 2 * out.numel()), e0)
+        return out, ysel
+
     def bn_act_maxpool_fwd(self, pg: PoolGeom, y, scale_shift, relu: bool, keep: bool):
         in_ld = _rows_ld(y, "y")
         do, ho, wo = pg.out_dims
@@ -393,7 +438,7 @@
         return out, idx
 
     def bn_act_pool_bwd(self, pg: PoolGeom, y, residual, dout, gamma, mean_invstd, scale_shift, relu: bool,
-                        want_dres: bool, dgamma_out, dbeta_out, dy_out=None):
+                        want_dres: bool, dgamma_out, dbeta_out, dy_out=None, y_sel=None):
         in_ld = _rows_ld(y, "y")
         d, dref, wsb, _ = _pool_plan(pg, in_ld, _rows_ld(dout, "dout"), None if residual is None else _rows_ld(residual, "residual"))
         dy = _dy_target(y, in_ld, dy_out)
@@ -401,11 +446,19 @@
         ws = self._workspace(y.device, wsb)
         c_valid = pg.C if gamma is None else int(gamma.shape[0])
         e0 = self._ev()
+        n_in = y.numel()
+        if y_sel is not None:
+            if residual is not None or want_dres:
+                raise _lib.RspError("bn_act_pool_bwd: y_sel with a residual")
+            _lib.check(self.lib.rsp_bn_act_pool_sel_bwd(dref, _ptr(y), _ptr(_chk(y_sel, "y_sel")), _ptr(dout), _ptr(gamma), _ptr(mean_invstd),
+                                                        _ptr(scale_shift), int(relu), _ptr(dy), _ptr(dgamma_out), _ptr(dbeta_out), c_valid,
+                                                        _ptr(ws), wsb, _stream()), "rsp_bn_act_pool_sel_bwd")
+            self._log_hbm("bn_bwd(reduce+apply)", 4 * (y_sel.numel() + 2 * dout.numel() + 2 * n_in), e0)
+            return dy, dres
         _lib.check(self.lib.rsp_bn_act_pool_bwd(dref, _ptr(y), _ptr(residual), _ptr(dout), _ptr(gamma),
                                                 _ptr(mean_invstd), _ptr(scale_shift), int(relu), _ptr(dy), _ptr(dres),
                                                 _ptr(dgamma_out), _ptr(dbeta_out), c_valid, None, None, _ptr(ws), wsb, _stream()),
                    "rsp_bn_act_pool_bwd")
-        n_in = y.numel()
         self._log_hbm("bn_bwd(reduce+apply)", 4 * (2 * (n_in * (1 if residual is None else 2) + dout.numel()) + n_in * (2 if want_dres else 1)), e0)
         return dy, dres
 
```

New measurement: 355.9, median of 6. 1.1% higher.
